# Veason-silverbullet/NNR

Measured on AMD Instinct MI355X. Metric: training impressions/sec on MIND-200k (CNE+SUE, bs=64), higher is better.
Workload: dtype f32

## Files before the change

### include/nnr_hip.h

```cpp
#ifndef NNR_HIP_H
#define NNR_HIP_H
#include <stdint.h>
#include <hip/hip_runtime_api.h>

#ifdef __cplusplus
extern "C" {
#endif

#define NNR_OK 0
#define NNR_ERR_ARG (-1)
#define NNR_ERR_LAUNCH (-2)
#define NNR_ERR_UNSUPPORTED (-3)

int nnr_version(void);

typedef struct nnr_gemm_args {
  const float* A;
  const float* B;
  float* C;
  int M, N, K;
  int lda, ldb, ldc;
  int trans_a, trans_b;
  const int* dyn_dev;
  int dyn_dim;
// ... 17 lines not shown
  int ldres;
  int accumulate;
  int atomic;
  const int* c_idx;
  int split_k;
  const float* rowdot_w;
  float* rowdot_out;
  int batch;
  long strideA, strideB, strideC, stride_aux, stride_res;
  int k_chunk;
  float* colsum_out;
  int tile;
  uint32_t drop_thresh;
  float drop_scale;
  int vec_epi;
  int sched;
  float* slab;
  long slab_floats;
  int slab_mode;
  const float* pre_add;
  int ldpre;
  int gate_bwd;
  const void* B3;
  long b3_stride;
  int ldb3;
} nnr_gemm_args;

int nnr_gemm_f32(const nnr_gemm_args* args, hipStream_t stream);
int nnr_split_bf16x3(const float* w, int rows, int cols, int ld, int ldo, void* out3, long img_stride, hipStream_t stream);

int nnr_seq_plan(uint8_t* mask, const int* ids, int n, int L, const int* perm_in, int* len_out, int* order, int* rank, int* slen,
                 int* bs, int* off, int* row_seq, int* tok, int* prev_f, int* prev_r, hipStream_t stream);

int nnr_seq_plan_pair(uint8_t* mask0, const int* ids0, int n0, uint8_t* mask1, const int* ids1, int n1, int L, const int* perm_in,
                      int* len_out, int* order, int* rank, int* slen, int* bs, int* off, int* row_seq, int* tok, int* prev_f,
                      int* prev_r, hipStream_t stream);

int nnr_cne_pair_map(const int* order_t, const int* order_c, int n0, int n, int* pm_t, int* pm_c, int* tmp, hipStream_t stream);

int nnr_mask_cover(const uint8_t* mask, int n, int L, uint8_t* cover, hipStream_t stream);
int nnr_seq_rowmap(const int* off, const int* rank, const int* len, int n, int L, int* rowmap, hipStream_t stream);

int nnr_lstm_dims(int H, int* UB, int* HP, int* NP);
int nnr_lstm_pack_weights(const float* w_ih_f, const float* w_hh_f, const float* b_ih_f, const float* b_hh_f, const float* w_ih_r,
                          const float* w_hh_r, const float* b_ih_r, const float* b_hh_r, int H, int E, float* w_ihp, float* b_p,
                          float* wf, float* wb, float* w_ihp_t, hipStream_t stream);
int nnr_lstm_unpack_grads(float* dw_ihp, float* db_p, float* dw_hhp, int H, int E, float* dw_ih_f, float* dw_hh_f,
                          float* db_ih_f, float* db_hh_f, float* dw_ih_r, float* dw_hh_r, float* db_ih_r, float* db_hh_r,
                          int accumulate , int zero_src, hipStream_t stream);
typedef struct nnr_lstm_problem {
  const int* bs; const int* off; const int* slen; const int* prev_f; const int* prev_r;
  int n, L;
  float* gates;
  float* cell;
  float* hout;
  float* cn;
  const float* wf;
  const float* wb;
  const float* dh;
  const float* dcn;
  unsigned* sync;
} nnr_lstm_problem;
size_t nnr_lstm_sync_bytes(int n);
size_t nnr_lstm_sync_diag_offset(int n);
int nnr_lstm_set_timeout_counter(unsigned* dev_counter);
int nnr_lstm_fwd(const nnr_lstm_problem* probs, int nprob, int H, hipStream_t stream);
int nnr_lstm_bwd(const nnr_lstm_problem* probs, int nprob, int H, hipStream_t stream);

typedef struct nnr_pool_args {
  const float* x; int ldx; int D; int n; int L;
  int packed;
  const int* off; const int* slen; const int* order;
  const uint8_t* mask; int mask_div;
  const float* score;
  const float* v; int ldv; float scale;
  float* alpha;
  float* out; int ldo; const float* add_in; int ldadd;
  const float* dout; int lddo; const float* dout2; int lddo2;
  float* dx; int lddx; int dx_accumulate;
  float* dscore;
  float* dv; int lddv;
  const float* th; int ldth; int A; const float* w2;
  const float* alpha_b; const float* dout_b; int lddo_b; const float* dscore_b; const float* v_b; int ldv_b; float scale_b;
} nnr_pool_args;
int nnr_attn_pool_fwd(const nnr_pool_args* a, hipStream_t stream);
int nnr_attn_pool_bwd(const nnr_pool_args* a, hipStream_t stream);

int nnr_gate_bwd(const float* dHt, const float* H, const float* G, float* dH, float* dpre, const int* rows_dev, int rows, int cols,
                 hipStream_t stream);
int nnr_packed_seq_sum(const float* x, int D, const int* off, const int* slen, int n, float* out, hipStream_t stream);
int nnr_slot_workspace_floats(int N);
int nnr_tanh_score_bwd(float* th, const float* ds, const float* w2, float* dw2, const int* rows_dev, int rows, int A, float* ws,
                       hipStream_t stream);
int nnr_colsum(const float* x, int ld, const int* rows_dev, int rows, int N, float* out_accum, float* ws, hipStream_t stream);
int nnr_rowdot(const float* x, int ld, const float* w, const int* rows_dev, int rows, int N, float* out,
               hipStream_t stream);
int nnr_small_embed_fwd(const float* table, const int* idx, int n, int dim, float* out, int ldo, float p, uint32_t seed,
                        hipStream_t stream);
int nnr_small_embed_bwd(const int* idx, int n, int dim, const float* dout, int lddo, float* dtable_accum, float p, uint32_t seed,
                        hipStream_t stream);
int nnr_embed_gather(const float* table, const int* idx, long n, const int* n_dev , int dim, float* out,
                     float p, uint32_t seed, hipStream_t stream);
int nnr_embed_scatter(const float* dout, const int* idx, long n, int dim, float* dtable_accum, float p, uint32_t seed,
                      hipStream_t stream);
int nnr_embed_scatter_dyn(const float* dout, const int* idx, long n, const int* n_dev, int dim, float* dtable, float p, uint32_t seed,
                          hipStream_t stream);
size_t nnr_token_sort_workspace_bytes(long cap, int vocab);
int nnr_token_sort(const int* tok, long cap, const int* n_dev, int vocab, unsigned* keys_tmp, int* rows_tmp, unsigned* keys_sorted,
                   int* rows_sorted, void* temp, size_t temp_bytes, hipStream_t stream);
size_t nnr_embed_scatter_sorted_workspace_floats(long cap);
int nnr_embed_scatter_sorted(const float* dout, const unsigned* keys_sorted, const int* rows_sorted, long cap, int vocab, int dim,
                             float* dtable_accum, float p, uint32_t seed, float* partial_ws, hipStream_t stream);
int nnr_transpose2d(const float* in, float* out, long rows, int cols, int accumulate, hipStream_t stream);
typedef struct nnr_transpose_desc { const float* in; float* out; int rows, cols; } nnr_transpose_desc;
int nnr_transpose_batch(const nnr_transpose_desc* descs_dev, int count, hipStream_t stream);
int nnr_add(float* y, const float* x, long n, float alpha, hipStream_t stream);
int nnr_add_atomic(float* y, const float* x, long n, float alpha, hipStream_t stream);
int nnr_add2d(float* y, int ldy, const float* x, int ldx, int rows, int cols, float alpha, int accumulate, hipStream_t stream);
int nnr_expand_rows_fwd(const float* x, float* y, int B, int N, int D, hipStream_t stream);
int nnr_expand_rows_bwd(const float* dy, float* dx, int B, int N, int D, hipStream_t stream);
int nnr_dropout(const float* x, float* y, long n, float p, uint32_t seed, hipStream_t stream);
int nnr_relu_bwd(const float* dy, const float* y, float* dx, long n, hipStream_t stream);
int nnr_gcn_aggregate_fwd(const float* graph, const float* z, const float* bias, const float* resid, float* r_out, float* y, int B, int G,
                          int D, int relu, float p, uint32_t seed, hipStream_t stream);
int nnr_gcn_aggregate_bwd(const float* graph, const float* dy, const float* r, float* ds, float* dx0, float* dz, int B, int G, int D, float p,
                          uint32_t seed, hipStream_t stream);
int nnr_relu_drop_bwd(const float* dy, const float* r, float* ds, float* dx, long n, float p, uint32_t seed, hipStream_t stream);

int nnr_mhsa_fwd(const float* qkv, const uint8_t* mask, int n, int Lq, int heads, int dh, float scale, float* out, float* prob,
                 float drop_p, uint32_t seed, hipStream_t stream);
int nnr_mhsa_bwd(const float* qkv, const uint8_t* mask, const float* prob, const float* dout, int n, int Lq, int heads, int dh,
                 float scale, float* dqkv, float drop_p, uint32_t seed, hipStream_t stream);
int nnr_mhsa_fwd_packed(const float* qkv, const uint8_t* mask, const int* rowmap, int n, int Lq, int heads, int dh, float scale, float* out,
                        float drop_p, uint32_t seed, hipStream_t stream);
int nnr_mhsa_bwd_packed(const float* qkv, const uint8_t* mask, const int* rowmap, const float* dout, int n, int Lq, int heads, int dh, float scale,
                        float* dqkv, float drop_p, uint32_t seed, hipStream_t stream);
int nnr_mhsa_pair_map(const int* off, const int* slen, const int* order, const uint8_t* mask, int n, int L, int* vrowmap, uint8_t* vmask,
                      hipStream_t stream);
int nnr_mhsa_fwd_paired(const float* qkv, const uint8_t* vmask, const int* vrowmap, const int* off, int n, int heads, int dh, float scale,
                        float* out, float drop_p, uint32_t seed, hipStream_t stream);
int nnr_mhsa_bwd_paired(const float* qkv, const uint8_t* vmask, const int* vrowmap, const int* off, const float* dout, int n, int heads, int dh,
                        float scale, float* dqkv, float drop_p, uint32_t seed, hipStream_t stream);

int nnr_sue_x0_fwd(const float* hist, const float* proxy, float* x0, int B, int Hn, int Kc, int D, float p, uint32_t seed,
                   uint8_t* cmask_fix, hipStream_t stream);
int nnr_sue_x0_bwd(const float* dx0, const float* dx0_add, float* dhist, float* dproxy_accum, int B, int Hn, int Kc, int D, float p,
                   uint32_t seed, hipStream_t stream);
int nnr_sue_slice_fwd(const float* gcn, const float* x0, float* gfeat, int B, int Hn, int G, int D, hipStream_t stream);
int nnr_sue_slice_bwd(const float* dgfeat, float* dpad, int B, int Hn, int G, int D, hipStream_t stream);
int nnr_sue_intra_fwd(const float* kf, const float* qc, const float* g, const long* cidx, int B, int N, int Hn, int C, int A, int D,
                      float* alpha, float* feat, hipStream_t stream);
int nnr_sue_intra_bwd(const float* kf, const float* qc, const float* g, const long* cidx, const float* alpha, const float* dfeat, int B,
                      int N, int Hn, int C, int A, int D, float* dg, float* dkf, float* dqc, float* ds_ws ,
                      hipStream_t stream);

int nnr_cand_attn_ws_floats(int B, int N, int H, int A);
int nnr_cand_attn_fwd(const float* P, const float* Q, const float* w2, const float* feat, int ldf, const uint8_t* mask, int B, int N,
                      int H, int A, int D, int act, float* alpha, float* out, hipStream_t stream);
int nnr_cand_attn_bwd(const float* P, const float* Q, const float* w2, const float* feat, int ldf, const uint8_t* mask, const float* alpha,
                      const float* dout, int B, int N, int H, int A, int D, int act, float* dP, float* dQ, float* dfeat,
                      int dfeat_accumulate, float* ws, float* dw2_accum, hipStream_t stream);

int nnr_omap_ws_floats(int B, int N, int H, int D, int K);
int nnr_omap_fwd(const float* hist, int ldf, const float* cand, const uint8_t* mask, const float* W, int B, int N, int H, int D, int K,
                 float* alpha, float* Y, float* beta, float* R, float* gamma, float* out, float* ws, hipStream_t stream);
int nnr_omap_bwd(const float* hist, int ldf, const float* cand, const uint8_t* mask, const float* W, const float* alpha, const float* Y,
                 const float* beta, const float* R, const float* gamma, const float* dout, int B, int N, int H, int D, int K, float* dhist,
                 int dhist_accumulate, float* dcand, float* dW_accum, float* ws, hipStream_t stream);
int nnr_omap_reg_fwd(const float* W, int D, int K, float coef, float* off, float* loss, hipStream_t stream);
int nnr_omap_reg_bwd(const float* W, const float* off, const float* gup, int D, int K, float coef, float* dW_accum, hipStream_t stream);

typedef struct nnr_corpus_tables {
  const int* news_category; const int* news_subCategory;
  const int* title_text; const uint8_t* title_mask; const int* title_entity;
  const int* abstract_text; const uint8_t* abstract_mask; const int* abstract_entity;
  const long* beh_user; const int* beh_history; const uint8_t* beh_history_mask; const int* beh_line;
  const float* graph_table; const uint8_t* cmask_table; const long* cidx_table;
  int T, C, H, G, K1;
} nnr_corpus_tables;
typedef struct nnr_batch_out {
  long* user_id;
  int* u_cat; int* u_sub; int* u_tt; uint8_t* u_tm; int* u_te; int* u_ct; uint8_t* u_cm; int* u_ce;
  uint8_t* u_hmask; float* u_graph; uint8_t* u_cmask; long* u_cidx;
  int* n_cat; int* n_sub; int* n_tt; uint8_t* n_tm; int* n_te; int* n_ct; uint8_t* n_cm; int* n_ce;
} nnr_batch_out;
int nnr_corpus_batch(const nnr_corpus_tables* t, const nnr_batch_out* o, const int* beh_idx, const int* samples, int ld_samples, int B,
                     int S, hipStream_t stream);
int nnr_history_graph(const int* cats, const uint8_t* hmask, int B, int H, int K, int norm, float* graph, uint8_t* cmask, long* cidx,
                      hipStream_t stream);
int nnr_rank_metrics(const float* scores, const uint8_t* labels, const long* offsets, int n_impressions, int* ranks,
                     double* per_impression, hipStream_t stream);

int nnr_logits_loss_fwd(const float* user, const float* cand, int B, int N, int D, float* logits, float* loss, float* dlogits,
                        hipStream_t stream);
int nnr_logits_fwd(const float* user, const float* cand, int B, int N, int D, float* logits, hipStream_t stream);
int nnr_nls_loss(const float* logits, int B, int N, float* loss, float* dlogits, hipStream_t stream);
int nnr_logits_bwd(const float* dlogits, const float* user, const float* cand, int B, int N, int D, float* duser, float* dcand,
                   int dcand_accumulate, hipStream_t stream);
int nnr_layernorm_fwd(const float* u, const float* gamma, const float* beta, float eps, long rows, int D, float* xhat, float* rstd,
                      float* r_out, const float* resid, float* y, float p, uint32_t seed, hipStream_t stream);
int nnr_layernorm_bwd(const float* dv, const float* xhat, const float* rstd, const float* gamma, long rows, int D, float* du,
                      float* dgamma, float* dbeta, hipStream_t stream);
int nnr_sumsq(const float* g, long n, float* out, hipStream_t stream);
int nnr_sumsq_part(const float* g, long n, float* out, const float* add_in, int slot, hipStream_t stream);
int nnr_clip_adam(float* p, const float* g, float* m, float* v, long n, const float* sumsq, float grad_scale, float clip, float lr,
                  float beta1, float beta2, float eps, float weight_decay, int step, hipStream_t stream);

int nnr_adam_skipped_steps(unsigned* host_out, int reset);
int nnr_adam_skipped_peek(unsigned* host_out);

typedef struct nnr_dp_ctx nnr_dp_ctx;
int nnr_dp_unique_id(void* out128);
int nnr_dp_init(const void* uid128, int rank, int world, nnr_dp_ctx** ctx);
int nnr_dp_allreduce(nnr_dp_ctx* ctx, float* flat, size_t n, hipStream_t stream);
int nnr_dp_broadcast(nnr_dp_ctx* ctx, float* flat, size_t n, int root, hipStream_t stream);
int nnr_dp_destroy(nnr_dp_ctx* ctx);
int nnr_dp_emulate_ranks(nnr_dp_ctx* ctx, int ranks);
int nnr_dp_busy(float* buf, long n, int workgroups, int iters, hipStream_t stream);
int nnr_rows_touch(const int* tok, long cap, const int* n_dev, int V, float* flags, hipStream_t stream);
int nnr_rows_compact(const float* flags, int V, int* pos, int* count, hipStream_t stream);
int nnr_rows_pack(const float* dense, const int* pos, int V, int E, float* packed, hipStream_t stream);
int nnr_rows_unpack(const float* packed, const int* pos, int V, int E, float* dense, hipStream_t stream);

int nnr_fusion_rows_fwd(const float* cat_table, const float* sub_table, const int* cat0, const int* sub0, int n0, const int* cat1,
                        const int* sub1, int n1, int cd, int sd, float* out, int ldo, float p, uint32_t seed_cat, uint32_t seed_sub,
                        hipStream_t stream);
int nnr_fusion_rows_bwd(const int* cat0, const int* sub0, int n0, const int* cat1, const int* sub1, int n1, int cd, int sd, const float* dout,
                        int lddo, float* dcat_table_accum, float* dsub_table_accum, float p, uint32_t seed_cat, uint32_t seed_sub,
                        hipStream_t stream);
int nnr_fusion_rows_bwd_det(const int* cat0, const int* sub0, int n0, const int* cat1, const int* sub1, int n1, int cd, int sd, int ncat,
// ... 34 lines not shown
```

### nnr_amd/_lib.py

```python
import ctypes as C
import os
import subprocess

_HERE = os.path.dirname(os.path.abspath(__file__))
LIB_PATH = os.environ.get('NNR_HIP_LIB') or os.path.join(_HERE, 'libnnr_hip.so')
_lib = None

vp, ci, cf, cu32, cl = C.c_void_p, C.c_int, C.c_float, C.c_uint32, C.c_long


class GemmArgs(C.Structure):
    _fields_ = [('A', vp), ('B', vp), ('C', vp), ('M', ci), ('N', ci), ('K', ci), ('lda', ci), ('ldb', ci), ('ldc', ci),
                ('trans_a', ci), ('trans_b', ci), ('dyn_dev', vp), ('dyn_dim', ci), ('a_idx', vp), ('b_idx', vp),
                ('drop_target', ci), ('drop_p', cf), ('drop_seed', cu32), ('drop_cols', ci), ('alpha', cf), ('bias', vp),
                ('rowvec', vp), ('ldrv', ci), ('rowvec_map', vp), ('act', ci), ('aux_out', vp), ('ldaux', ci), ('mul', vp),
                ('ldmul', ci), ('resid', vp), ('ldres', ci), ('accumulate', ci), ('atomic', ci), ('c_idx', vp),
                ('split_k', ci), ('rowdot_w', vp), ('rowdot_out', vp), ('batch', ci), ('strideA', cl), ('strideB', cl),
                ('strideC', cl), ('stride_aux', cl), ('stride_res', cl), ('k_chunk', ci), ('colsum_out', vp), ('tile', ci), ('drop_thresh', cu32),
                ('drop_scale', cf), ('vec_epi', ci), ('sched', ci), ('slab', vp), ('slab_floats', cl), ('slab_mode', ci), ('pre_add', vp), ('ldpre', ci), ('gate_bwd', ci), ('B3', vp), ('b3_stride', cl), ('ldb3', ci)]


class LstmProblem(C.Structure):
    _fields_ = [('bs', vp), ('off', vp), ('slen', vp), ('prev_f', vp), ('prev_r', vp), ('n', ci), ('L', ci), ('gates', vp),
                ('cell', vp), ('hout', vp), ('cn', vp), ('wf', vp), ('wb', vp), ('dh', vp), ('dcn', vp), ('sync', vp)]


class TransposeDesc(C.Structure):
    _fields_ = [('inp', vp), ('out', vp), ('rows', ci), ('cols', ci)]


class CorpusTables(C.Structure):
    _fields_ = [(k, vp) for k in ('news_category', 'news_subCategory', 'title_text', 'title_mask', 'title_entity', 'abstract_text',
                                  'abstract_mask', 'abstract_entity', 'beh_user', 'beh_history', 'beh_history_mask', 'beh_line',
                                  'graph_table', 'cmask_table', 'cidx_table')] + [(k, ci) for k in ('T', 'C', 'H', 'G', 'K1')]


class BatchOut(C.Structure):
    _fields_ = [(k, vp) for k in ('user_id', 'u_cat', 'u_sub', 'u_tt', 'u_tm', 'u_te', 'u_ct', 'u_cm', 'u_ce', 'u_hmask', 'u_graph',
                                  'u_cmask', 'u_cidx', 'n_cat', 'n_sub', 'n_tt', 'n_tm', 'n_te', 'n_ct', 'n_cm', 'n_ce')]


class PoolArgs(C.Structure):
    _fields_ = [('x', vp), ('ldx', ci), ('D', ci), ('n', ci), ('L', ci), ('packed', ci), ('off', vp), ('slen', vp),
                ('order', vp), ('mask', vp), ('mask_div', ci), ('score', vp), ('v', vp), ('ldv', ci), ('scale', cf),
                ('alpha', vp), ('out', vp), ('ldo', ci), ('add_in', vp), ('ldadd', ci), ('dout', vp), ('lddo', ci),
                ('dout2', vp), ('lddo2', ci), ('dx', vp), ('lddx', ci), ('dx_accumulate', ci), ('dscore', vp), ('dv', vp),
                ('lddv', ci), ('th', vp), ('ldth', ci), ('A', ci), ('w2', vp),
                ('alpha_b', vp), ('dout_b', vp), ('lddo_b', ci), ('dscore_b', vp), ('v_b', vp), ('ldv_b', ci), ('scale_b', cf)]


SIGNATURES = {
    'nnr_version': 'i32',
    'nnr_gemm_f32': 'i32 GemmArgs stream',
    'nnr_split_bf16x3': 'i32 ptr i32 i32 i32 i32 ptr i64 stream',
    'nnr_seq_plan': 'i32 ptr ptr i32 i32 ptr ptr ptr ptr ptr ptr ptr ptr ptr ptr ptr stream',
    'nnr_seq_plan_pair': 'i32 ptr ptr i32 ptr ptr i32 i32 ptr ptr ptr ptr ptr ptr ptr ptr ptr ptr ptr stream',
    'nnr_cne_pair_map': 'i32 ptr ptr i32 i32 ptr ptr ptr stream',
    'nnr_mask_cover': 'i32 ptr i32 i32 ptr stream',
    'nnr_seq_rowmap': 'i32 ptr ptr ptr i32 i32 ptr stream',
    'nnr_lstm_dims': 'i32 i32 ptr ptr ptr',
    'nnr_lstm_pack_weights': 'i32 ptr ptr ptr ptr ptr ptr ptr ptr i32 i32 ptr ptr ptr ptr ptr stream',
    'nnr_lstm_unpack_grads': 'i32 ptr ptr ptr i32 i32 ptr ptr ptr ptr ptr ptr ptr ptr i32 i32 stream',
    'nnr_lstm_sync_bytes': 'u64 i32',
    'nnr_lstm_sync_diag_offset': 'u64 i32',
    'nnr_lstm_set_timeout_counter': 'i32 ptr',
    'nnr_lstm_fwd': 'i32 LstmProblem i32 i32 stream',
    'nnr_lstm_bwd': 'i32 LstmProblem i32 i32 stream',
    'nnr_attn_pool_fwd': 'i32 PoolArgs stream',
    'nnr_attn_pool_bwd': 'i32 PoolArgs stream',
    'nnr_gate_bwd': 'i32 ptr ptr ptr ptr ptr ptr i32 i32 stream',
    'nnr_packed_seq_sum': 'i32 ptr i32 ptr ptr i32 ptr stream',
    'nnr_slot_workspace_floats': 'i32 i32',
    'nnr_tanh_score_bwd': 'i32 ptr ptr ptr ptr ptr i32 i32 ptr stream',
    'nnr_colsum': 'i32 ptr i32 ptr i32 i32 ptr ptr stream',
    'nnr_rowdot': 'i32 ptr i32 ptr ptr i32 i32 ptr stream',
    'nnr_small_embed_fwd': 'i32 ptr ptr i32 i32 ptr i32 f32 seed stream',
    'nnr_small_embed_bwd': 'i32 ptr i32 i32 ptr i32 ptr f32 seed stream',
    'nnr_embed_gather': 'i32 ptr ptr i64 ptr i32 ptr f32 seed stream',
    'nnr_embed_scatter': 'i32 ptr ptr i64 i32 ptr f32 seed stream',
    'nnr_embed_scatter_dyn': 'i32 ptr ptr i64 ptr i32 ptr f32 seed stream',
    'nnr_token_sort_workspace_bytes': 'u64 i64 i32',
    'nnr_token_sort': 'i32 ptr i64 ptr i32 ptr ptr ptr ptr ptr u64 stream',
    'nnr_embed_scatter_sorted_workspace_floats': 'u64 i64',
    'nnr_embed_scatter_sorted': 'i32 ptr ptr ptr i64 i32 i32 ptr f32 seed ptr stream',
    'nnr_transpose2d': 'i32 ptr ptr i64 i32 i32 stream',
    'nnr_transpose_batch': 'i32 TransposeDesc i32 stream',
    'nnr_add': 'i32 ptr ptr i64 f32 stream',
    'nnr_add_atomic': 'i32 ptr ptr i64 f32 stream',
    'nnr_add2d': 'i32 ptr i32 ptr i32 i32 i32 f32 i32 stream',
    'nnr_expand_rows_fwd': 'i32 ptr ptr i32 i32 i32 stream',
    'nnr_expand_rows_bwd': 'i32 ptr ptr i32 i32 i32 stream',
    'nnr_dropout': 'i32 ptr ptr i64 f32 seed stream',
    'nnr_relu_bwd': 'i32 ptr ptr ptr i64 stream',
    'nnr_gcn_aggregate_fwd': 'i32 ptr ptr ptr ptr ptr ptr i32 i32 i32 i32 f32 seed stream',
    'nnr_gcn_aggregate_bwd': 'i32 ptr ptr ptr ptr ptr ptr i32 i32 i32 f32 seed stream',
    'nnr_relu_drop_bwd': 'i32 ptr ptr ptr ptr i64 f32 seed stream',
    'nnr_mhsa_fwd': 'i32 ptr ptr i32 i32 i32 i32 f32 ptr ptr f32 seed stream',
    'nnr_mhsa_bwd': 'i32 ptr ptr ptr ptr i32 i32 i32 i32 f32 ptr f32 seed stream',
    'nnr_mhsa_fwd_packed': 'i32 ptr ptr ptr i32 i32 i32 i32 f32 ptr f32 seed stream',
    'nnr_mhsa_bwd_packed': 'i32 ptr ptr ptr ptr i32 i32 i32 i32 f32 ptr f32 seed stream',
    'nnr_mhsa_pair_map': 'i32 ptr ptr ptr ptr i32 i32 ptr ptr stream',
    'nnr_mhsa_fwd_paired': 'i32 ptr ptr ptr ptr i32 i32 i32 f32 ptr f32 seed stream',
    'nnr_mhsa_bwd_paired': 'i32 ptr ptr ptr ptr ptr i32 i32 i32 f32 ptr f32 seed stream',
    'nnr_sue_x0_fwd': 'i32 ptr ptr ptr i32 i32 i32 i32 f32 seed ptr stream',
    'nnr_sue_x0_bwd': 'i32 ptr ptr ptr ptr i32 i32 i32 i32 f32 seed stream',
    'nnr_sue_slice_fwd': 'i32 ptr ptr ptr i32 i32 i32 i32 stream',
    'nnr_sue_slice_bwd': 'i32 ptr ptr i32 i32 i32 i32 stream',
    'nnr_sue_intra_fwd': 'i32 ptr ptr ptr ptr i32 i32 i32 i32 i32 i32 ptr ptr stream',
    'nnr_sue_intra_bwd': 'i32 ptr ptr ptr ptr ptr ptr i32 i32 i32 i32 i32 i32 ptr ptr ptr ptr stream',
    'nnr_cand_attn_ws_floats': 'i32 i32 i32 i32 i32',
    'nnr_cand_attn_fwd': 'i32 ptr ptr ptr ptr i32 ptr i32 i32 i32 i32 i32 i32 ptr ptr stream',
    'nnr_cand_attn_bwd': 'i32 ptr ptr ptr ptr i32 ptr ptr ptr i32 i32 i32 i32 i32 i32 ptr ptr ptr i32 ptr ptr stream',
    'nnr_omap_ws_floats': 'i32 i32 i32 i32 i32 i32',
    'nnr_omap_fwd': 'i32 ptr i32 ptr ptr ptr i32 i32 i32 i32 i32 ptr ptr ptr ptr ptr ptr ptr stream',
    'nnr_omap_bwd': 'i32 ptr i32 ptr ptr ptr ptr ptr ptr ptr ptr ptr i32 i32 i32 i32 i32 ptr i32 ptr ptr ptr stream',
    'nnr_omap_reg_fwd': 'i32 ptr i32 i32 f32 ptr ptr stream',
    'nnr_omap_reg_bwd': 'i32 ptr ptr ptr i32 i32 f32 ptr stream',
    'nnr_corpus_batch': 'i32 CorpusTables BatchOut ptr ptr i32 i32 i32 stream',
    'nnr_history_graph': 'i32 ptr ptr i32 i32 i32 i32 ptr ptr ptr stream',
    'nnr_rank_metrics': 'i32 ptr ptr ptr i32 ptr ptr stream',
    'nnr_logits_loss_fwd': 'i32 ptr ptr i32 i32 i32 ptr ptr ptr stream',
    'nnr_logits_fwd': 'i32 ptr ptr i32 i32 i32 ptr stream',
    'nnr_nls_loss': 'i32 ptr i32 i32 ptr ptr stream',
    'nnr_logits_bwd': 'i32 ptr ptr ptr i32 i32 i32 ptr ptr i32 stream',
    'nnr_layernorm_fwd': 'i32 ptr ptr ptr f32 i64 i32 ptr ptr ptr ptr ptr f32 seed stream',
    'nnr_layernorm_bwd': 'i32 ptr ptr ptr ptr i64 i32 ptr ptr ptr stream',
    'nnr_sumsq': 'i32 ptr i64 ptr stream',
    'nnr_sumsq_part': 'i32 ptr i64 ptr ptr i32 stream',
    'nnr_clip_adam': 'i32 ptr ptr ptr ptr i64 ptr f32 f32 f32 f32 f32 f32 f32 i32 stream',
    'nnr_adam_skipped_steps': 'i32 ptr i32',
    'nnr_adam_skipped_peek': 'i32 ptr',
    'nnr_dp_unique_id': 'i32 ptr',
    'nnr_dp_init': 'i32 ptr i32 i32 handle',
    'nnr_dp_allreduce': 'i32 handle ptr u64 stream',
    'nnr_dp_broadcast': 'i32 handle ptr u64 i32 stream',
    'nnr_dp_destroy': 'i32 handle',
    'nnr_dp_emulate_ranks': 'i32 handle i32',
    'nnr_dp_busy': 'i32 ptr i64 i32 i32 stream',
    'nnr_rows_touch': 'i32 ptr i64 ptr i32 ptr stream',
    'nnr_rows_compact': 'i32 ptr i32 ptr ptr stream',
    'nnr_rows_pack': 'i32 ptr ptr i32 i32 ptr stream',
    'nnr_rows_unpack': 'i32 ptr ptr i32 i32 ptr stream',
    'nnr_fusion_rows_fwd': 'i32 ptr ptr ptr ptr i32 ptr ptr i32 i32 i32 ptr i32 f32 seed seed stream',
    'nnr_fusion_rows_bwd': 'i32 ptr ptr i32 ptr ptr i32 i32 i32 ptr i32 ptr ptr f32 seed seed stream',
    'nnr_fusion_rows_bwd_det': 'i32 ptr ptr i32 ptr ptr i32 i32 i32 i32 i32 ptr i32 ptr ptr f32 seed seed stream',
    'nnr_click_loss': 'i32 ptr ptr i32 i32 i32 ptr ptr ptr ptr ptr ptr stream',
    'nnr_fill_zero': 'i32 ptr u64 stream',
    'nnr_copy_bytes': 'i32 ptr ptr u64 stream',
    'nnr_fill_column_u8': 'i32 ptr i32 i32 i32 i32 stream',
    'nnr_tape_create': 'i32 handle',
    'nnr_tape_destroy': 'i32 handle',
    'nnr_tape_fn_id': 'i32 cstr',
    'nnr_tape_fn_nargs': 'i32 i32',
    'nnr_tape_call': 'i32 handle i32 stream ptr i32 ptr ptr ptr i32 i32 ptr ptr',
    'nnr_tape_wait_stream': 'i32 handle stream stream',
    'nnr_tape_event_record': 'i32 handle u64 stream',
    'nnr_tape_event_wait': 'i32 handle stream u64',
    'nnr_tape_segment': 'i32 handle',
    'nnr_tape_patch': 'i32 handle u64 i32 i32 i64',
    'nnr_tape_finalize': 'i32 handle',
    'nnr_tape_prepare_timing': 'i32 handle i32',
    'nnr_tape_info': 'i32 handle ptr ptr ptr ptr ptr',
    'nnr_tape_replay': 'i32 handle i32 ptr i32 ptr i32 i32',
    'nnr_tape_timings': 'i32 handle i32 ptr i32',
    'nnr_tape_timeline': 'i32 handle i32 ptr ptr ptr i32',
    'nnr_tape_last_error': 'i32 handle ptr ptr cstr i32',
}
SYMBOLS = list(SIGNATURES)
STRUCTS = {'nnr_gemm_args': GemmArgs, 'nnr_lstm_problem': LstmProblem, 'nnr_pool_args': PoolArgs, 'nnr_transpose_desc': TransposeDesc,
           'nnr_corpus_tables': CorpusTables, 'nnr_batch_out': BatchOut}
DEVICE_STRUCTS = {'TransposeDesc'}
_CTYPES = {'i32': ci, 'i64': cl, 'u64': C.c_size_t, 'f32': cf, 'seed': cu32, 'ptr': vp, 'handle': vp, 'cstr': C.c_char_p, 'stream': vp}
_CTYPES.update((c.__name__, vp if c.__name__ in DEVICE_STRUCTS else C.POINTER(c)) for c in STRUCTS.values())


def kinds(name):
    return SIGNATURES[name].split()[1:]


class NnrHipError(RuntimeError):
    pass


def build(force=False):
    if force:
        bdir = os.path.join(_HERE, 'csrc', 'build')
        if os.path.isdir(bdir):
            for f in os.listdir(bdir):
# ... 41 lines not shown
```

### nnr_amd/csrc/gcn.hip

```cpp
#include "common.h"

namespace {

constexpr int GCN_MAXG = 128;

template <int MODE, int MT>
__global__ __launch_bounds__(256) __attribute__((amdgpu_waves_per_eu(3, 8))) void gcn_aggregate_kernel(
    const float* __restrict__ graph, const float* __restrict__ in, const float* __restrict__ bias, const float* __restrict__ aux_in,
    float* __restrict__ out0, float* __restrict__ out1, float* __restrict__ out2, int G, int D, int relu, uint32_t seed, uint32_t thr, float scale) {
  extern __shared__ __attribute__((aligned(16))) float sm[];
  const int ks_n = (G + 3) >> 2, GR = ks_n * 4;
  const int A_LD = GR | 1;
  constexpr int Z_LD = 68;
  float* As = sm;
  float* Zs = sm + ((GR * A_LD + 3) & ~3);
  const int b = blockIdx.y, tid = threadIdx.x, lane = tid & 63, w = tid >> 6;
  const int r16 = lane & 15, kk = lane >> 4;
  const float* A = graph + (long)b * G * G;
  if ((G & 3) == 0) {
    const int g4 = G >> 2;
    for (int i = tid; i < G * g4; i += 256) {
      const int row = i / g4, c = (i - row * g4) * 4;
      const f32x4 v = *reinterpret_cast<const f32x4*>(A + row * G + c);
#pragma unroll
      for (int e = 0; e < 4; ++e) As[row * A_LD + c + e] = v[e];
    }
  } else {
    for (int i = tid; i < GR * A_LD; i += 256) {
      const int row = i / A_LD, col = i - row * A_LD;
      As[i] = (row < G && col < G) ? A[row * G + col] : 0.f;
    }
  }
  const int c0 = blockIdx.x * 64;
  const int c4 = (tid & 15) * 4, rr = tid >> 4;
  const bool cok = c0 + c4 < D;
  const long base = (long)b * G * D;
#pragma unroll
  for (int pass = 0; pass < MT; ++pass) {
    const int row = pass * 16 + rr;
    f32x4 v = {0.f, 0.f, 0.f, 0.f};
    if (row < G && cok) {
      const long idx = base + (long)row * D + c0 + c4;
      v = *reinterpret_cast<const f32x4*>(in + idx);
      if (MODE == 1 && aux_in) {
        if (thr) {
          bool kp[4];
          nnr_keep4(seed, (uint64_t)idx, thr, kp);
#pragma unroll
          for (int e = 0; e < 4; ++e) v[e] = kp[e] ? v[e] * scale : 0.f;
        }
        if (out1) *reinterpret_cast<f32x4*>(out1 + idx) = v;
        const f32x4 rv = *reinterpret_cast<const f32x4*>(aux_in + idx);
#pragma unroll
        for (int e = 0; e < 4; ++e) v[e] = rv[e] > 0.f ? v[e] : 0.f;
        *reinterpret_cast<f32x4*>(out0 + idx) = v;
      }
    }
    if (row < GR) *reinterpret_cast<f32x4*>(&Zs[row * Z_LD + c4]) = v;
  }
  __syncthreads();
  float bf[MT * 4];
#pragma unroll
  for (int ks = 0; ks < MT * 4; ++ks) bf[ks] = ks < ks_n ? Zs[(4 * ks + kk) * Z_LD + w * 16 + r16] : 0.f;
  f32x4 acc[MT];
  int arow[MT];
#pragma unroll
  for (int m = 0; m < MT; ++m) {
    acc[m] = f32x4{0.f, 0.f, 0.f, 0.f};
    arow[m] = min(m * 16 + r16, GR - 1);
  }
#pragma unroll
  for (int ks = 0; ks < MT * 4; ++ks) {
    if (ks < ks_n) {
#pragma unroll
      for (int m = 0; m < MT; ++m) {
        const float a = MODE == 0 ? As[arow[m] * A_LD + 4 * ks + kk] : As[(4 * ks + kk) * A_LD + arow[m]];
        acc[m] = __builtin_amdgcn_mfma_f32_16x16x4f32(a, bf[ks], acc[m], 0, 0, 0);
      }
    }
  }
  __syncthreads();
#pragma unroll
  for (int m = 0; m < MT; ++m)
#pragma unroll
    for (int e = 0; e < 4; ++e)
      if (m * 16 + 4 * kk + e < GR) Zs[(m * 16 + 4 * kk + e) * Z_LD + w * 16 + r16] = acc[m][e];
  __syncthreads();
  if (!cok) return;
  f32x4 bv = {0.f, 0.f, 0.f, 0.f};
  if (MODE == 0 && bias) bv = *reinterpret_cast<const f32x4*>(bias + c0 + c4);
#pragma unroll
  for (int pass = 0; pass < MT; ++pass) {
    const int row = pass * 16 + rr;
    if (row < G) {
      const long idx = base + (long)row * D + c0 + c4;
      f32x4 x = *reinterpret_cast<const f32x4*>(&Zs[row * Z_LD + c4]);
      if (MODE == 0) {
        x += bv;
        if (relu) {
#pragma unroll
          for (int e = 0; e < 4; ++e) x[e] = fmaxf(x[e], 0.f);
        }
        if (out1) *reinterpret_cast<f32x4*>(out1 + idx) = x;
        if (aux_in) x += *reinterpret_cast<const f32x4*>(aux_in + idx);
        if (thr) {
          bool kp[4];
          nnr_keep4(seed, (uint64_t)idx, thr, kp);
#pragma unroll
          for (int e = 0; e < 4; ++e) x[e] = kp[e] ? x[e] * scale : 0.f;
        }
        *reinterpret_cast<f32x4*>(out0 + idx) = x;
      } else {
        *reinterpret_cast<f32x4*>(out2 + idx) = x;
      }
    }
  }
}


}

extern "C" int nnr_gcn_aggregate_fwd(const float* graph, const float* z, const float* bias, const float* resid, float* r_out, float* y, int B,
                                     int G, int D, int relu, float p, uint32_t seed, hipStream_t stream) {
  if (!graph || !z || !y || B <= 0 || G <= 0 || D <= 0) return NNR_ERR_ARG;
  if (G > GCN_MAXG || (D & 3)) return NNR_ERR_UNSUPPORTED;
  const float sc = p > 0.f ? 1.f / (1.f - p) : 1.f;
  const int gp = (G + 15) / 16 * 16, gr = (G + 3) / 4 * 4;
#define GCN_CASE(MT_) case MT_: hipLaunchKernelGGL((gcn_aggregate_kernel<0, MT_>), dim3((D + 63) / 64, B), dim3(256), (size_t)(((gr * (gr | 1) + 3) & ~3) + gr * 68) * sizeof(float), \
                                                   stream, graph, z, bias, resid, y, r_out, nullptr, G, D, relu, seed, nnr_drop_thresh(p), sc); break;
  switch (gp / 16) { GCN_CASE(1) GCN_CASE(2) GCN_CASE(3) GCN_CASE(4) GCN_CASE(5) GCN_CASE(6) GCN_CASE(7) GCN_CASE(8) }
#undef GCN_CASE
  NNR_CHECK_LAUNCH();
  return NNR_OK;
}

extern "C" int nnr_gcn_aggregate_bwd(const float* graph, const float* dy, const float* r, float* ds, float* dx0, float* dz, int B, int G, int D,
                                     float p, uint32_t seed, hipStream_t stream) {
  if (!graph || !dy || !dz || B <= 0 || G <= 0 || D <= 0 || (r && !ds)) return NNR_ERR_ARG;
  if (G > GCN_MAXG || (D & 3)) return NNR_ERR_UNSUPPORTED;
  const float sc = p > 0.f ? 1.f / (1.f - p) : 1.f;
  const int gp = (G + 15) / 16 * 16, gr = (G + 3) / 4 * 4;
#define GCN_CASE(MT_) case MT_: hipLaunchKernelGGL((gcn_aggregate_kernel<1, MT_>), dim3((D + 63) / 64, B), dim3(256), (size_t)(((gr * (gr | 1) + 3) & ~3) + gr * 68) * sizeof(float), \
                                                   stream, graph, dy, nullptr, r, ds, dx0, dz, G, D, 0, seed, nnr_drop_thresh(p), sc); break;
  switch (gp / 16) { GCN_CASE(1) GCN_CASE(2) GCN_CASE(3) GCN_CASE(4) GCN_CASE(5) GCN_CASE(6) GCN_CASE(7) GCN_CASE(8) }
#undef GCN_CASE
  NNR_CHECK_LAUNCH();
  return NNR_OK;
}
```

### nnr_amd/csrc/gemm.hip

```cpp
#include "common.h"
#include <stdlib.h>
#include <type_traits>

namespace {

template <int BK>
__device__ __forceinline__ int swz(int r16) {
  return BK == 16 ? ((4 - (r16 >> 2)) & 3) : BK == 32 ? ((r16 >> 1) & 7) : (r16 & 15);
}

template <int TM, int TN>
__device__ __forceinline__ void gemm_epilogue(const nnr_gemm_args& g, f32x4 (&acc)[TM][TN], float* lds, float* __restrict__ C, int m0,
                                              int n0, int M, int N, int z) {
  constexpr int BN = 16 * TN, E_LD = BN + 4;
  const int tid = threadIdx.x, lane = tid & 63, w = tid >> 6;
  const int r = lane & 15, kk = lane >> 4;
  const uint32_t dthr = g.drop_thresh;
  const float dscale = g.drop_scale;
  const bool use_atomic = !g.slab_mode && (g.atomic || g.split_k > 1 || g.k_chunk > 0);
  float* aux = g.aux_out;
  const float* res = g.resid;
  const float* mulp = g.mul;
  if (g.batch > 1 && g.split_k <= 1 && g.k_chunk <= 0) {
    if (aux) aux += (long)z * g.stride_aux;
// ... 797 lines not shown
  dim3 grid(nbm * nbn, 1, g.batch > 1 ? g.batch : 1), block(256);
  hipLaunchKernelGGL((gemm_nt_pipe2_kernel<TM, TN, NS, OCC>), grid, block, 0, s, g);
  NNR_CHECK_LAUNCH();
  return NNR_OK;
}

template <int TM, int TN, int BK, int NS, int OCC, int PRIO = 0>
int launch_pipe(const nnr_gemm_args& g0, hipStream_t s) {
  constexpr int BM = 64 * TM, BN = 16 * TN;
  nnr_gemm_args g = g0;
  g.sched = kNtRagged;
  const int nbm = (g.M + BM - 1) / BM, nbn = (g.N + BN - 1) / BN;
  dim3 grid(nbm * nbn, 1, g.batch > 1 ? g.batch : 1), block(256);
  hipLaunchKernelGGL((gemm_nt_pipe_kernel<TM, TN, BK, NS, OCC, PRIO>), grid, block, 0, s, g);
  NNR_CHECK_LAUNCH();
  return NNR_OK;
}

static bool pipe_ok(const nnr_gemm_args& g) {
  auto al = [](const void* p) { return ((uintptr_t)p & 15) == 0; };
  return !g.trans_a && !g.trans_b && !g.b_idx && g.split_k <= 1 && g.k_chunk <= 0 && !g.rowdot_w && !g.colsum_out &&
         (g.drop_target == 0 || g.drop_target == 3 || g.drop_target == 4) && (g.K & 3) == 0 && (g.lda & 3) == 0 && (g.ldb & 3) == 0 &&
         al(g.A) && al(g.B) && (g.batch <= 1 || (((g.strideA | g.strideB) & 3) == 0)) && (g.dyn_dim == 0 || g.dyn_dim == 1);
}

typedef __bf16 bf16x8_t __attribute__((ext_vector_type(8)));
__device__ __forceinline__ void split3_bf16(float x, __bf16& h1, __bf16& h2, __bf16& h3) {
  const unsigned u = __builtin_bit_cast(unsigned, x), mag = u & 0x7fffffffu;
  const bool big = mag >= 0x7f7f8000u, nonfinite = mag >= 0x7f800000u;
  h1 = (__bf16)x;
  if (big) h1 = __builtin_bit_cast(__bf16, (unsigned short)((u >> 16) | (mag > 0x7f800000u ? 0x40u : 0u)));
  const float r1 = nonfinite ? 0.f : x - (float)h1;
  h2 = (__bf16)r1;
  const float r2 = r1 - (float)h2;
  h3 = (__bf16)r2;
}
__global__ void split_bf16x3_kernel(const float* __restrict__ w, int rows, int cols, int ld, int ldo, __bf16* __restrict__ out, long img_stride) {
  const long total = (long)rows * ldo;
  for (long i = blockIdx.x * (long)blockDim.x + threadIdx.x; i < total; i += (long)gridDim.x * blockDim.x) {
    const int r = (int)(i / ldo), c = (int)(i - (long)r * ldo);
    __bf16 a, b, d;
    split3_bf16(c < cols ? w[(long)r * ld + c] : 0.f, a, b, d);
    out[i] = a; out[img_stride + i] = b; out[2 * img_stride + i] = d;
  }
}
__device__ __forceinline__ int bx3_swzA(int r) { return ((r >> 1) & 1) | (((r >> 3) & 1) << 2); }
__device__ __forceinline__ int bx3_swzB(int r) { return (r >> 1) & 3; }

typedef unsigned u32x4_t __attribute__((ext_vector_type(4)));
__device__ __forceinline__ unsigned hi16_pair(float odd, float even) {
  return __builtin_amdgcn_perm(__float_as_uint(odd), __float_as_uint(even), 0x07060302u);
}
__device__ __forceinline__ void split3_trunc8(const f32x4& x0, const f32x4& x1, bf16x8_t& a1, bf16x8_t& a2, bf16x8_t& a3) {
  const float xs[8] = {x0[0], x0[1], x0[2], x0[3], x1[0], x1[1], x1[2], x1[3]};
  unsigned w1[4], w2[4], w3[4];
#pragma unroll
  for (int p = 0; p < 4; ++p) {
    const float xe = xs[2 * p], xo = xs[2 * p + 1];
    const unsigned h1 = hi16_pair(xo, xe);
    const float re = xe - __uint_as_float(h1 << 16), ro = xo - __uint_as_float(h1 & 0xffff0000u);
    const unsigned h2 = hi16_pair(ro, re);
    const float se = re - __uint_as_float(h2 << 16), so = ro - __uint_as_float(h2 & 0xffff0000u);
    w1[p] = h1; w2[p] = h2; w3[p] = hi16_pair(so, se);
  }
  a1 = __builtin_bit_cast(bf16x8_t, u32x4_t{w1[0], w1[1], w1[2], w1[3]});
  a2 = __builtin_bit_cast(bf16x8_t, u32x4_t{w2[0], w2[1], w2[2], w2[3]});
  a3 = __builtin_bit_cast(bf16x8_t, u32x4_t{w3[0], w3[1], w3[2], w3[3]});
}

template <int TM, int TN, int NS>
__global__ __launch_bounds__(256, (NS * (64 * TM * 128 + 3 * 16 * TN * 64) > 80 * 1024 ? 1 : 2)) void gemm_nt_bx3_kernel(nnr_gemm_args g) {
  constexpr int BM = 64 * TM, BN = 16 * TN, BK = 32;
  constexpr int A_BYTES = BM * BK * 4, B_IMG_BYTES = BN * BK * 2, STAGE_BYTES = A_BYTES + 3 * B_IMG_BYTES;
  constexpr int NIA = A_BYTES / 1024, NIB1 = B_IMG_BYTES / 1024;
  static_assert(A_BYTES % 1024 == 0 && B_IMG_BYTES % 1024 == 0 && NIA % 4 == 0, "tile shape");
  constexpr int E_LD = BN + 4;
  constexpr int LDS_BYTES = NS * STAGE_BYTES > 64 * E_LD * 4 ? NS * STAGE_BYTES : 64 * E_LD * 4;
  __shared__ __attribute__((aligned(1024))) unsigned char lds_raw[LDS_BYTES];
  const int tid = threadIdx.x, lane = tid & 63, w = __builtin_amdgcn_readfirstlane(tid >> 6), r = lane & 15, q = lane >> 4;
  int M = g.M;
  if (g.dyn_dim == 1) M = min(M, *g.dyn_dev);
  const int N = g.N, K = g.K;
  const int nbm = (M + BM - 1) / BM, nbn = (N + BN - 1) / BN, nblk = nbm * nbn;
  if ((int)blockIdx.x >= nblk) return;
  int v;
  {
    const int b = blockIdx.x, qq = nblk >> 3, rem = nblk & 7, x = b & 7, slot = b >> 3;
    v = x * qq + min(x, rem) + slot;
  }
  const int bm = v / nbn, bn = v - bm * nbn, m0 = bm * BM, n0 = bn * BN;
  const int S = (K + BK - 1) / BK;
  const unsigned lds_base = (unsigned)(uintptr_t)lds_raw;
  const float* zero = nnr_zero_page;
  asm volatile("" : "+s"(zero));
  constexpr int NA = NIA / 4, NBW = (3 * NIB1 + 3) / 4;
  static_assert(NA <= 8 && NBW <= 8, "tile shape");
  unsigned voffA[8], voffB[8];
  int akc[NA], bkc[NBW];
#pragma unroll
  for (int i = 0; i < 8; ++i) voffA[i] = voffB[i] = 0;
#pragma unroll
  for (int i = 0; i < NA; ++i) {
    const int row = (w + 4 * i) * 8 + lane / 8, c = (lane % 8) ^ bx3_swzA(row & 15);
    akc[i] = 4 * c;
    voffA[i] = (unsigned)(((long)min(row, M - 1 - m0) * g.lda + 4 * c) * 4);
  }
#pragma unroll
  for (int j = 0; j < NBW; ++j) {
    const int idx = min(w + 4 * j, 3 * NIB1 - 1);
    const int img = idx / NIB1, jj = idx - img * NIB1, row = jj * 16 + lane / 4, c = (lane % 4) ^ bx3_swzB(row & 15);
    bkc[j] = 8 * c;
    voffB[j] = (unsigned)(((long)img * g.b3_stride + (long)min(row, N - 1 - n0) * g.ldb3 + 8 * c) * 2);
  }
  const float* Abase = g.A + (long)m0 * g.lda;
  const char* Bbase = reinterpret_cast<const char*>(reinterpret_cast<const __bf16*>(g.B3) + (long)n0 * g.ldb3);
  const bool nb_hi = ((3 * NIB1) % 4 == 0) || (w < (3 * NIB1) % 4);
  const bool ktail = (K % BK) != 0;
  auto issue = [&](int s) __attribute__((always_inline)) {
    const int k0 = s * BK;
    const unsigned sb = lds_base + (unsigned)((s % NS) * STAGE_BYTES) + (unsigned)(w * 1024);
    if (!(ktail && s == S - 1)) {
      lds_dma16_block<NA>(Abase + k0, sb, voffA);
      const float* bb = reinterpret_cast<const float*>(Bbase + 2L * k0);
      if (nb_hi) lds_dma16_block<NBW>(bb, sb + A_BYTES, voffB);
      else if constexpr (NBW > 1) lds_dma16_block<NBW - 1>(bb, sb + A_BYTES, voffB);
      return;
    }
#pragma unroll
    for (int i = 0; i < NA; ++i)
      lds_dma16((k0 + akc[i] < K) ? reinterpret_cast<const float*>(reinterpret_cast<const char*>(Abase + k0) + voffA[i]) : zero, sb + (unsigned)(i * 4096));
#pragma unroll
    for (int j = 0; j < NBW; ++j)
      if (j < NBW - 1 || nb_hi)
        lds_dma16((k0 + bkc[j] < K) ? reinterpret_cast<const float*>(Bbase + 2L * k0 + voffB[j]) : zero, sb + A_BYTES + (unsigned)(j * 4096));
  };
  f32x4 acc_hi[TM][TN], acc_lo[TM][TN];
#pragma unroll
  for (int m = 0; m < TM; ++m)
#pragma unroll
    for (int n = 0; n < TN; ++n) acc_hi[m][n] = acc_lo[m][n] = f32x4{0.f, 0.f, 0.f, 0.f};
#pragma unroll
  for (int s = 0; s < NS - 1; ++s)
    if (s < S) issue(s);
  for (int s = 0; s < S; ++s) {
    if (nb_hi) wait_stages<NA + NBW, NS - 2>(S - 1 - s);
    else wait_stages<NA + NBW - 1, NS - 2>(S - 1 - s);
    __builtin_amdgcn_s_barrier();
    if (s + NS - 1 < S) issue(s + NS - 1);
    const unsigned char* st = lds_raw + (s % NS) * STAGE_BYTES;
    const float* As = reinterpret_cast<const float*>(st);
    const __bf16* Bi = reinterpret_cast<const __bf16*>(st + A_BYTES);
    bf16x8_t bf[3][TN];
#pragma unroll
    for (int img = 0; img < 3; ++img)
#pragma unroll
      for (int n = 0; n < TN; ++n)
        bf[img][n] = *reinterpret_cast<const bf16x8_t*>(Bi + img * (BN * BK) + (n * 16 + r) * BK + ((q ^ bx3_swzB(r)) * 8));
#pragma unroll
    for (int m = 0; m < TM; ++m) {
      const float* arow = As + ((w * TM + m) * 16 + r) * BK;
      const f32x4 x0 = *reinterpret_cast<const f32x4*>(arow + 4 * ((2 * q) ^ bx3_swzA(r)));
      const f32x4 x1 = *reinterpret_cast<const f32x4*>(arow + 4 * ((2 * q + 1) ^ bx3_swzA(r)));
      bf16x8_t a1, a2, a3;
      split3_trunc8(x0, x1, a1, a2, a3);
#pragma unroll
      for (int n = 0; n < TN; ++n) {
        acc_hi[m][n] = __builtin_amdgcn_mfma_f32_16x16x32_bf16(a1, bf[0][n], acc_hi[m][n], 0, 0, 0);
        acc_lo[m][n] = __builtin_amdgcn_mfma_f32_16x16x32_bf16(a3, bf[0][n], acc_lo[m][n], 0, 0, 0);
        acc_lo[m][n] = __builtin_amdgcn_mfma_f32_16x16x32_bf16(a1, bf[2][n], acc_lo[m][n], 0, 0, 0);
        acc_lo[m][n] = __builtin_amdgcn_mfma_f32_16x16x32_bf16(a2, bf[1][n], acc_lo[m][n], 0, 0, 0);
        acc_lo[m][n] = __builtin_amdgcn_mfma_f32_16x16x32_bf16(a2, bf[0][n], acc_lo[m][n], 0, 0, 0);
        acc_lo[m][n] = __builtin_amdgcn_mfma_f32_16x16x32_bf16(a1, bf[1][n], acc_lo[m][n], 0, 0, 0);
      }
    }
  }
#pragma unroll
  for (int m = 0; m < TM; ++m)
#pragma unroll
    for (int n = 0; n < TN; ++n) acc_hi[m][n] += acc_lo[m][n];
  __syncthreads();
  gemm_epilogue<TM, TN>(g, acc_hi, reinterpret_cast<float*>(lds_raw), g.C, m0, n0, M, N, 0);
}

static bool bx3_ok(const nnr_gemm_args& g) {
  auto al = [](const void* p) { return ((uintptr_t)p & 15) == 0; };
  return pipe_ok(g) && !g.a_idx && g.batch <= 1 && g.B3 && al(g.B3) && (g.ldb3 & 7) == 0 && g.ldb3 >= g.K && ((g.b3_stride * 2) & 15) == 0;
}
template <int TM, int TN, int NS>
int launch_bx3(const nnr_gemm_args& g, hipStream_t s) {
  constexpr int BM = 64 * TM, BN = 16 * TN;
  const int nbm = (g.M + BM - 1) / BM, nbn = (g.N + BN - 1) / BN;
  hipLaunchKernelGGL((gemm_nt_bx3_kernel<TM, TN, NS>), dim3(nbm * nbn), dim3(256), 0, s, g);
  NNR_CHECK_LAUNCH();
  return NNR_OK;
}

__device__ __forceinline__ int tn_eff_slices(int split_k, int sched, int K, int nblk, int slots) {
  const int deal_mode = sched & 3;
  const int want_wg = ((sched >> 2) & 63) ? ((sched >> 2) & 63) * 64 : 512;
  const int slice_stages = (sched >> 8) ? (sched >> 8) : 96;
  const int ktiles = (K + 15) / 16;
  const int want = (want_wg + nblk - 1) / nblk;
  int eff = max(1, min(min(split_k, max(want, ktiles / slice_stages)), max(1, ktiles / 12)));
  if (deal_mode != 2) {
    const int W = eff * nblk, wv = W / slots;
    const int target = W < slots ? slots : (((W - wv * slots) * 2 < slots) ? wv * slots : (wv + 1) * slots);
    eff = max(1, min(target / nblk, min(split_k, max(1, ktiles / 12))));
  }
  return eff;
}

template <int TM, int TN, int NS, int OCC, int PRIO = 0>
__global__ __launch_bounds__(256, OCC) void gemm_tn_pipe_kernel(nnr_gemm_args g) {
  if (PRIO == 1) set_prio_dyn((blockIdx.x + gridDim.x * blockIdx.z) >> 8);
  constexpr int BK = 16, BM = 64 * TM, BN = 16 * TN;
  constexpr int PA = BM, PB = BN <= 64 ? 64 : (BN <= 128 ? 128 : 256);
  constexpr int RA = 256 / PA, RB = 256 / PB;
  constexpr int NIA = BK / RA, NIB = BK / RB, NI = NIA + NIB;
  constexpr int NPW = (NI + 3) / 4;
  constexpr int STAGE = BK * (PA + PB);
  constexpr int E_LD = BN + 4;
  constexpr int LDS_FLOATS = (NS * STAGE > 64 * E_LD) ? NS * STAGE : 64 * E_LD;
  static_assert(BN <= 256 && NI % 4 == 0, "tile shape");
  __shared__ __attribute__((aligned(1024))) float lds[LDS_FLOATS];

  const int tid = threadIdx.x, lane = tid & 63, w = __builtin_amdgcn_readfirstlane(tid >> 6);
  const int r = lane & 15, kk = lane >> 4;
  const int M = g.M, N = g.N;
  int K = g.K;
  if (g.dyn_dim == 2) K = min(K, *g.dyn_dev);
  const int nbm = (M + BM - 1) / BM, nbn = (N + BN - 1) / BN;
  const int nblk = nbm * nbn;
  int v, z = 0;
  int kbeg = 0, kend = K;
  if (g.split_k > 1) {
    const int deal_mode = g.sched & 3;
    const int ktiles = (K + BK - 1) / BK;
    const int eff = tn_eff_slices(g.split_k, g.sched, K, nblk, OCC * 256);
    if (deal_mode) {
      const int W = eff * nblk, per = (W + 7) >> 3;
      const int L = blockIdx.x, x = L & 7, slot = L >> 3;
      const int lin = x * per + slot;
      if (slot >= per || lin >= W) return;
      z = lin / nblk;
      v = lin - z * nblk;
    } else {
      z = blockIdx.x / nblk;
      v = blockIdx.x - z * nblk;
      if (z >= eff) return;
    }
    const int per_k = (ktiles + eff - 1) / eff;
    kbeg = z * per_k * BK;
    kend = min(K, kbeg + per_k * BK);
    if (kbeg >= kend) return;
  } else {
    const int b = blockIdx.x, q = nblk >> 3, rem = nblk & 7, x = b & 7, slot = b >> 3;
    v = x * q + min(x, rem) + slot;
  }
  const int bm = v / nbn, bn = v - bm * nbn;
  const int m0 = bm * BM, n0 = bn * BN;
  const float* __restrict__ A = g.A;
  const float* __restrict__ B = g.B;
  const int* __restrict__ bidx = g.b_idx;
  const float* zero = nnr_zero_page;
  asm volatile("" : "+s"(zero));

  long coloff[NPW];
  int krow[NPW];
#pragma unroll
  for (int i = 0; i < NPW; ++i) {
    const int q = w + 4 * i;
    if (q < NIA) {
      const int kl = q * RA + lane / (PA / 4), p4 = lane % (PA / 4);
      const int col = (4 * p4) ^ (16 * ((kl >> 2) & 1));
      krow[i] = kl;
// ... 661 lines not shown
```

### nnr_amd/csrc/misc.hip

```cpp
#include "common.h"

namespace {

constexpr int EW_BLOCKS = 2048;
__host__ __device__ inline int ew_grid(long n, int per_block) {
  long b = (n + per_block - 1) / per_block;
  return (int)(b < 1 ? 1 : (b > EW_BLOCKS ? EW_BLOCKS : b));
}
__device__ __forceinline__ int dyn_rows(const int* dev, int rows) { return dev ? min(rows, *dev) : rows; }

__global__ void gate_bwd_kernel(const float* __restrict__ dHt, const float* __restrict__ H, const float* __restrict__ G,
                                float* __restrict__ dH, float* __restrict__ dpre, const int* rows_dev, int rows, int cols) {
  const long n4 = (long)dyn_rows(rows_dev, rows) * cols / 4;
  for (long i = blockIdx.x * (long)blockDim.x + threadIdx.x; i < n4; i += (long)gridDim.x * blockDim.x) {
    const f32x4 d = reinterpret_cast<const f32x4*>(dHt)[i], h = reinterpret_cast<const f32x4*>(H)[i],
                g = reinterpret_cast<const f32x4*>(G)[i];
    reinterpret_cast<f32x4*>(dH)[i] = d * g;
    reinterpret_cast<f32x4*>(dpre)[i] = d * h * g * (1.f - g);
  }
}

__global__ __launch_bounds__(256) void packed_seq_sum_kernel(const float* __restrict__ x, int D, const int* __restrict__ off,
                                                             const int* __restrict__ slen, int n, float* __restrict__ out) {
  __shared__ f32x4 part[128];
// ... 241 lines not shown
    }
    __syncthreads();
    for (int j = ty; j < 32; j += 8) {
      const int c = c0 + j, r = r0 + tx;
      if (r < d.rows && c < d.cols) d.out[(long)c * d.rows + r] = tile[tx][j];
    }
    __syncthreads();
  }
}

__global__ void add_kernel(float* __restrict__ y, const float* __restrict__ x, long n, float alpha) {
  for (long i = blockIdx.x * (long)blockDim.x + threadIdx.x; i < n; i += (long)gridDim.x * blockDim.x) y[i] += alpha * x[i];
}
__global__ void add_atomic_kernel(float* __restrict__ y, const float* __restrict__ x, long n, float alpha) {
  for (long i = blockIdx.x * (long)blockDim.x + threadIdx.x; i < n; i += (long)gridDim.x * blockDim.x) atomicAdd(&y[i], alpha * x[i]);
}
__global__ void add2d_kernel(float* __restrict__ y, int ldy, const float* __restrict__ x, int ldx, int rows, int cols,
                             float alpha, int accumulate) {
  const long total = (long)rows * cols;
  for (long i = blockIdx.x * (long)blockDim.x + threadIdx.x; i < total; i += (long)gridDim.x * blockDim.x) {
    const int r = i / cols, c = i - (long)r * cols;
    const float v = alpha * x[(long)r * ldx + c];
    float* p = y + (long)r * ldy + c;
    *p = accumulate ? *p + v : v;
  }
}
__global__ void expand_rows_kernel(const float* __restrict__ x, float* __restrict__ y, int B, int N, int D) {
  const long total = (long)B * N * D;
  for (long i = blockIdx.x * (long)blockDim.x + threadIdx.x; i < total; i += (long)gridDim.x * blockDim.x) {
    const long row = i / D;
    const int c = (int)(i - row * D);
    y[i] = x[(row / N) * D + c];
  }
}
__global__ void expand_rows_bwd_kernel(const float* __restrict__ dy, float* __restrict__ dx, int B, int N, int D) {
  const long total = (long)B * D;
  for (long i = blockIdx.x * (long)blockDim.x + threadIdx.x; i < total; i += (long)gridDim.x * blockDim.x) {
    const long b = i / D;
    const int c = (int)(i - b * D);
    const float* p = dy + b * N * D + c;
    float acc = p[0];
    for (int j = 1; j < N; ++j) acc += p[(long)j * D];
    dx[i] = acc;
  }
}

__global__ void sue_x0_kernel(const float* __restrict__ hist, const float* __restrict__ proxy, float* __restrict__ x0, int B,
                              int Hn, int Kc, int D, const float* __restrict__ dx0, const float* __restrict__ dx0_add,
                              float* __restrict__ dhist, float* __restrict__ dproxy, uint8_t* __restrict__ cmask_fix, uint32_t seed,
                              uint32_t thr, float scale) {
  const int G = Hn + Kc;
  const long total = (long)B * G * D;
  if (cmask_fix)
    for (long b = blockIdx.x * (long)blockDim.x + threadIdx.x; b < B; b += (long)gridDim.x * blockDim.x) cmask_fix[b * (Kc + 1) + Kc] = 1;
  for (long i = blockIdx.x * (long)blockDim.x + threadIdx.x; i < total; i += (long)gridDim.x * blockDim.x) {
    const int c = i % D; const long q = i / D; const int j = q % G; const int b = q / G;
    const float up = dx0 ? (dx0_add ? dx0[i] + dx0_add[i] : dx0[i]) : 0.f;
    if (j < Hn) {
      if (x0) x0[i] = hist[((long)b * Hn + j) * D + c];
      if (dhist) dhist[((long)b * Hn + j) * D + c] = up;
    } else {
      const int k = j - Hn;
      if (x0) {
        const float m = nnr_keep(seed, (uint64_t)((long)b * Kc + k) * D + c, thr) ? scale : 0.f;
        x0[i] = proxy[(long)k * D + c] * m;
      }
    }
  }
  if (dproxy) {
    for (long t = blockIdx.x * (long)blockDim.x + threadIdx.x; t < (long)Kc * D; t += (long)gridDim.x * blockDim.x) {
      const int c = t % D, k = t / D;
      float acc = 0.f;
      for (int b = 0; b < B; ++b) {
        const long i = ((long)b * G + Hn + k) * D + c;
        const float up = dx0_add ? dx0[i] + dx0_add[i] : dx0[i];
        const float m = nnr_keep(seed, (uint64_t)((long)b * Kc + k) * D + c, thr) ? scale : 0.f;
        acc += up * m;
      }
      atomicAdd(&dproxy[t], acc);
    }
  }
}

__global__ void sue_slice_kernel(const float* __restrict__ gcn, const float* __restrict__ x0, float* __restrict__ gfeat,
                                 const float* __restrict__ dgfeat, float* __restrict__ dpad, int B, int Hn, int G, int D) {
  const long total = (long)B * G * D;
  for (long i = blockIdx.x * (long)blockDim.x + threadIdx.x; i < total; i += (long)gridDim.x * blockDim.x) {
    const int c = i % D; const long q = i / D; const int j = q % G; const int b = q / G;
    if (gfeat) { if (j < Hn) gfeat[((long)b * Hn + j) * D + c] = gcn[i] + x0[i]; }
    if (dpad) dpad[i] = (j < Hn) ? dgfeat[((long)b * Hn + j) * D + c] : 0.f;
  }
}

__global__ void relu_drop_bwd_kernel(const float* __restrict__ dy, const float* __restrict__ r, float* __restrict__ ds,
                                     float* __restrict__ dx, long n, int cols, uint32_t seed, uint32_t thr, float scale) {
  for (long i = blockIdx.x * (long)blockDim.x + threadIdx.x; i < n; i += (long)gridDim.x * blockDim.x) {
    const float m = nnr_keep(seed, (uint64_t)i, thr) ? scale : 0.f;
    const float g = dy[i] * m;
    ds[i] = (r[i] > 0.f) ? g : 0.f;
    if (dx) dx[i] = g;
  }
}

__global__ void dropout_kernel(const float* __restrict__ x, float* __restrict__ y, long n, uint32_t seed, uint32_t thr,
                               float scale) {
  for (long i = blockIdx.x * (long)blockDim.x + threadIdx.x; i < n; i += (long)gridDim.x * blockDim.x)
    y[i] = nnr_keep(seed, (uint64_t)i, thr) ? x[i] * scale : 0.f;
}

__global__ void relu_bwd_kernel(const float* __restrict__ dy, const float* __restrict__ y, float* __restrict__ dx, long n) {
  for (long i = blockIdx.x * (long)blockDim.x + threadIdx.x; i < n; i += (long)gridDim.x * blockDim.x)
    dx[i] = (y[i] > 0.f) ? dy[i] : 0.f;
}

constexpr int SUE_MAXH = 64, SUE_MAXC = 32;
__device__ __forceinline__ void sue_members(const int* cid, int Hn, int C, int* ccnt, int* cstart, int* order) {
  const int tid = threadIdx.x;
  if (tid < C) {
    int n = 0;
    for (int j = 0; j < Hn; ++j) n += (cid[j] == tid);
    ccnt[tid] = n;
  }
  __syncthreads();
  if (tid == 0) {
    int acc = 0;
    for (int c = 0; c < C; ++c) { cstart[c] = acc; acc += ccnt[c]; }
  }
  __syncthreads();
  if (tid < C) {
    int k = cstart[tid];
    for (int j = 0; j < Hn; ++j) if (cid[j] == tid) order[k++] = j;
  }
  __syncthreads();
}

__device__ __forceinline__ bool sue_xcd_map(int id, int B, int per_user, int* b, int* w) {
  const int x = id & 7, slot = id >> 3;
  *b = (slot / per_user) * 8 + x;
  *w = slot % per_user;
  return *b < B;
}
__global__ __launch_bounds__(256) void sue_intra_fwd_kernel(const float* __restrict__ kf, const float* __restrict__ qc,
                                                            const float* __restrict__ g, const long* __restrict__ cidx,
                                                            int B, int N, int Hn, int C, int A, int D, float inv_scale,
                                                            float* __restrict__ alpha, float* __restrict__ feat) {
  __shared__ float sc[SUE_MAXH], al[SUE_MAXH], cmax[SUE_MAXC], csum[SUE_MAXC];
  __shared__ int cid[SUE_MAXH], order[SUE_MAXH], ccnt[SUE_MAXC], cstart[SUE_MAXC];
  int b, wi;
  if (!sue_xcd_map(blockIdx.x, B, N * ((D + 255) / 256), &b, &wi)) return;
  const int slice = wi / N, bn = b * N + (wi - slice * N);
  const int tid = threadIdx.x, lane = tid & 63, w = tid >> 6;
  for (int j = tid; j < Hn; j += 256) cid[j] = (int)cidx[(long)b * Hn + j];
  const float* q = qc + (long)bn * A;
  for (int j0 = w; j0 < Hn; j0 += 16) {
    float p[4] = {0.f, 0.f, 0.f, 0.f};
    const float* k[4];
#pragma unroll
    for (int u = 0; u < 4; ++u) k[u] = kf + ((long)b * Hn + min(j0 + 4 * u, Hn - 1)) * A;
    for (int x = lane; x < A; x += 64) {
      const float qv = q[x];
      float kv[4];
#pragma unroll
      for (int u = 0; u < 4; ++u) kv[u] = k[u][x];
#pragma unroll
      for (int u = 0; u < 4; ++u) p[u] += kv[u] * qv;
    }
// ... 329 lines not shown
  const float mean = wave_sum(s) / (float)D;
  float q = 0.f;
#pragma unroll
  for (int i = 0; i < LN_MAXPL; ++i) {
    const int c = lane + 64 * i;
    const float d = c < D ? v[i] - mean : 0.f;
    q += d * d;
  }
  const float rstd = 1.f / sqrtf(wave_sum(q) / (float)D + eps);
  if (lane == 0) rstd_out[row] = rstd;
#pragma unroll
  for (int i = 0; i < LN_MAXPL; ++i) {
    const int c = lane + 64 * i;
    if (c < D) {
      const float xh = (v[i] - mean) * rstd;
      const float r = fmaxf(xh * gamma[c] + beta[c], 0.f);
      xhat[row * D + c] = xh;
      r_out[row * D + c] = r;
      float o = r + (resid ? resid[row * D + c] : 0.f);
      if (thr) o = nnr_keep(seed, (uint64_t)(row * D + c), thr) ? o * scale : 0.f;
      y[row * D + c] = o;
    }
  }
}

__global__ __launch_bounds__(256) void ln_bwd_kernel(const float* __restrict__ dv, const float* __restrict__ xhat, const float* __restrict__ rstd,
                                                     const float* __restrict__ gamma, long rows, int D, float* __restrict__ du,
                                                     float* __restrict__ dgamma, float* __restrict__ dbeta) {
  __shared__ float red[2][LN_MAXPL * 64];
  const int lane = threadIdx.x & 63, w = threadIdx.x >> 6;
  for (int i = threadIdx.x; i < 2 * LN_MAXPL * 64; i += 256) (&red[0][0])[i] = 0.f;
  __syncthreads();
  float ag[LN_MAXPL], ab[LN_MAXPL];
#pragma unroll
  for (int i = 0; i < LN_MAXPL; ++i) ag[i] = ab[i] = 0.f;
  for (int k = 0; k < 4; ++k) {
    const long row = (long)blockIdx.x * 16 + w * 4 + k;
    if (row >= rows) break;
    float g[LN_MAXPL], xh[LN_MAXPL];
    float s1 = 0.f, s2 = 0.f;
#pragma unroll
    for (int i = 0; i < LN_MAXPL; ++i) {
      const int c = lane + 64 * i;
      const float d = c < D ? dv[row * D + c] : 0.f;
      xh[i] = c < D ? xhat[row * D + c] : 0.f;
      g[i] = c < D ? d * gamma[c] : 0.f;
      s1 += g[i];
      s2 += g[i] * xh[i];
      ag[i] += d * xh[i];
      ab[i] += d;
    }
    s1 = wave_sum(s1) / (float)D;
    s2 = wave_sum(s2) / (float)D;
    const float rs = rstd[row];
#pragma unroll
    for (int i = 0; i < LN_MAXPL; ++i) {
      const int c = lane + 64 * i;
      if (c < D) du[row * D + c] = rs * (g[i] - s1 - xh[i] * s2);
    }
  }
#pragma unroll
  for (int i = 0; i < LN_MAXPL; ++i) {
    atomicAdd(&red[0][lane + 64 * i], ag[i]);
    atomicAdd(&red[1][lane + 64 * i], ab[i]);
  }
  __syncthreads();
  for (int c = threadIdx.x; c < D; c += 256) {
    atomicAdd(&dgamma[c], red[0][c]);
    atomicAdd(&dbeta[c], red[1][c]);
  }
}

}

#define EW_LAUNCH(kern, n, ...)                                                             \
  do {                                                                                      \
    hipLaunchKernelGGL(kern, dim3(ew_grid((n), 256)), dim3(256), 0, stream, __VA_ARGS__);   \
    NNR_CHECK_LAUNCH();                                                                     \
    return NNR_OK;                                                                          \
  } while (0)

extern "C" int nnr_version(void) { return 1; }

extern "C" int nnr_gate_bwd(const float* dHt, const float* H, const float* G, float* dH, float* dpre, const int* rows_dev,
                            int rows, int cols, hipStream_t stream) {
  if (cols & 3) return NNR_ERR_UNSUPPORTED;
  EW_LAUNCH(gate_bwd_kernel, (long)rows * cols / 4, dHt, H, G, dH, dpre, rows_dev, rows, cols);
}

extern "C" int nnr_packed_seq_sum(const float* x, int D, const int* off, const int* slen, int n, float* out, hipStream_t stream) {
  if (D & 3) return NNR_ERR_UNSUPPORTED;
  hipLaunchKernelGGL(packed_seq_sum_kernel, dim3(n), dim3(256), 0, stream, x, D, off, slen, n, out);
  NNR_CHECK_LAUNCH();
  return NNR_OK;
}

extern "C" int nnr_slot_workspace_floats(int N) { return NNR_SLOTS * N; }

extern "C" int nnr_tanh_score_bwd(float* th, const float* ds, const float* w2, float* dw2, const int* rows_dev, int rows, int A,
                                  float* ws, hipStream_t stream) {
  const int rpb = 64;
  int blocks = (rows + rpb - 1) / rpb;
  if (ws) blocks = blocks > NNR_SLOTS ? NNR_SLOTS : (blocks < 1 ? 1 : blocks);
  hipLaunchKernelGGL(tanh_score_bwd_kernel, dim3(blocks), dim3(256), 0, stream, th, ds, w2, dw2, rows_dev, rows, A, rpb, ws);
  NNR_CHECK_LAUNCH();
  if (ws) {
    hipLaunchKernelGGL(slot_reduce_kernel, dim3((A + 7) / 8), dim3(256), 0, stream, (const float*)ws, blocks, A, dw2);
    NNR_CHECK_LAUNCH();
  }
  return NNR_OK;
}

extern "C" int nnr_rowdot(const float* x, int ld, const float* w, const int* rows_dev, int rows, int N, float* out, hipStream_t stream) {
  if (!x || !w || !out || rows <= 0) return rows <= 0 ? NNR_OK : NNR_ERR_ARG;
  if ((N & 3) || (ld & 3) || ((uintptr_t)x & 15) || ((uintptr_t)w & 15)) return NNR_ERR_UNSUPPORTED;
  const int blocks = (rows + 3) / 4;
  hipLaunchKernelGGL(rowdot_kernel, dim3(blocks > 8192 ? 8192 : blocks), dim3(256), 0, stream, x, ld, w, rows_dev, rows, N, out);
  NNR_CHECK_LAUNCH();
  return NNR_OK;
}

extern "C" int nnr_colsum(const float* x, int ld, const int* rows_dev, int rows, int N, float* out, float* ws, hipStream_t stream) {
  if (rows <= 0 || N <= 0) return NNR_OK;
  int rpb = rows / 512;
  rpb = rpb < 8 ? 8 : (rpb > 128 ? 128 : rpb);
  int blocks = (rows + rpb - 1) / rpb;
  if (ws) blocks = blocks > NNR_SLOTS ? NNR_SLOTS : blocks;
  hipLaunchKernelGGL(colsum_kernel, dim3(blocks, (N + 255) / 256), dim3(256), 0, stream, x, ld, rows_dev, rows, N, out, rpb, ws);
  NNR_CHECK_LAUNCH();
  if (ws) {
    hipLaunchKernelGGL(slot_reduce_kernel, dim3((N + 7) / 8), dim3(256), 0, stream, (const float*)ws, blocks, N, out);
    NNR_CHECK_LAUNCH();
  }
  return NNR_OK;
}

extern "C" int nnr_small_embed_fwd(const float* table, const int* idx, int n, int dim, float* out, int ldo, float p, uint32_t seed,
                                   hipStream_t stream) {
  const float sc = p > 0.f ? 1.f / (1.f - p) : 1.f;
  EW_LAUNCH(small_embed_kernel, (long)n * dim, table, idx, n, dim, out, ldo, (float*)nullptr, (const float*)nullptr, 0, seed,
            nnr_drop_thresh(p), sc);
}
extern "C" int nnr_small_embed_bwd(const int* idx, int n, int dim, const float* dout, int lddo, float* dtable, float p, uint32_t seed,
                                   hipStream_t stream) {
  const float sc = p > 0.f ? 1.f / (1.f - p) : 1.f;
  if (n <= 0) return NNR_OK;
  const int rpw = n >= 16 * 1024 ? 16 : (n >= 2048 ? 8 : 4);
  hipLaunchKernelGGL(small_embed_bwd_kernel, dim3((n + 4 * rpw - 1) / (4 * rpw)), dim3(256), 0, stream, idx, n, dim, dout, lddo, dtable, seed,
                     nnr_drop_thresh(p), sc, rpw);
  NNR_CHECK_LAUNCH();
  return NNR_OK;
}


extern "C" int nnr_embed_gather(const float* table, const int* idx, long n, const int* n_dev, int dim, float* out, float p, uint32_t seed,
                                hipStream_t stream) {
  if (dim & 3) return NNR_ERR_UNSUPPORTED;
  const float sc = p > 0.f ? 1.f / (1.f - p) : 1.f;
  hipLaunchKernelGGL(embed_gather_kernel, dim3(ew_grid((n + 3) / 4, 4)), dim3(256), 0, stream, table, idx, n, n_dev, dim, out, seed,
                     nnr_drop_thresh(p), sc);
  NNR_CHECK_LAUNCH();
  return NNR_OK;
}
static int embed_scatter_launch(const float* dout, const int* idx, long n, const int* n_dev, int dim, float* dtable, float p, uint32_t seed,
                                hipStream_t stream) {
  const float sc = p > 0.f ? 1.f / (1.f - p) : 1.f;
  const long want = (n + 3) / 4;
  hipLaunchKernelGGL(embed_scatter_kernel, dim3((int)(want < 1 ? 1 : (want > 1024 ? 1024 : want))), dim3(256), 0, stream, dout, idx, n, n_dev, dim, dtable,
                     seed, nnr_drop_thresh(p), sc);
  NNR_CHECK_LAUNCH();
  return NNR_OK;
}
extern "C" int nnr_embed_scatter(const float* dout, const int* idx, long n, int dim, float* dtable, float p, uint32_t seed, hipStream_t stream) {
  return embed_scatter_launch(dout, idx, n, nullptr, dim, dtable, p, seed, stream);
}
extern "C" int nnr_embed_scatter_dyn(const float* dout, const int* idx, long n, const int* n_dev, int dim, float* dtable, float p, uint32_t seed,
                                     hipStream_t stream) {
  return embed_scatter_launch(dout, idx, n, n_dev, dim, dtable, p, seed, stream);
}
extern "C" int nnr_transpose2d(const float* in, float* out, long rows, int cols, int accumulate, hipStream_t stream) {
  EW_LAUNCH(transpose2d_kernel, rows * cols, in, out, rows, cols, accumulate);
}

extern "C" int nnr_transpose_batch(const nnr_transpose_desc* descs_dev, int count, hipStream_t stream) {
  if (count <= 0) return NNR_OK;
  if (!descs_dev) return NNR_ERR_ARG;
  hipLaunchKernelGGL(transpose_batch_kernel, dim3(64, count), dim3(256), 0, stream, descs_dev);
  NNR_CHECK_LAUNCH();
  return NNR_OK;
}

extern "C" int nnr_add(float* y, const float* x, long n, float alpha, hipStream_t stream) { EW_LAUNCH(add_kernel, n, y, x, n, alpha); }
extern "C" int nnr_add_atomic(float* y, const float* x, long n, float alpha, hipStream_t stream) {
  EW_LAUNCH(add_atomic_kernel, n, y, x, n, alpha);
}
extern "C" int nnr_add2d(float* y, int ldy, const float* x, int ldx, int rows, int cols, float alpha, int accumulate,
                         hipStream_t stream) {
  EW_LAUNCH(add2d_kernel, (long)rows * cols, y, ldy, x, ldx, rows, cols, alpha, accumulate);
}

extern "C" int nnr_expand_rows_fwd(const float* x, float* y, int B, int N, int D, hipStream_t stream) {
  if (!x || !y || B <= 0 || N <= 0 || D <= 0) return NNR_ERR_ARG;
  EW_LAUNCH(expand_rows_kernel, (long)B * N * D, x, y, B, N, D);
}
extern "C" int nnr_expand_rows_bwd(const float* dy, float* dx, int B, int N, int D, hipStream_t stream) {
  if (!dy || !dx || B <= 0 || N <= 0 || D <= 0) return NNR_ERR_ARG;
  EW_LAUNCH(expand_rows_bwd_kernel, (long)B * D, dy, dx, B, N, D);
}

extern "C" int nnr_sue_x0_fwd(const float* hist, const float* proxy, float* x0, int B, int Hn, int Kc, int D, float p, uint32_t seed,
                              uint8_t* cmask_fix, hipStream_t stream) {
  const float sc = p > 0.f ? 1.f / (1.f - p) : 1.f;
  EW_LAUNCH(sue_x0_kernel, (long)B * (Hn + Kc) * D, hist, proxy, x0, B, Hn, Kc, D, (const float*)nullptr, (const float*)nullptr, (float*)nullptr,
            (float*)nullptr, cmask_fix, seed, nnr_drop_thresh(p), sc);
}
extern "C" int nnr_sue_x0_bwd(const float* dx0, const float* dx0_add, float* dhist, float* dproxy, int B, int Hn, int Kc, int D, float p,
                              uint32_t seed, hipStream_t stream) {
  const float sc = p > 0.f ? 1.f / (1.f - p) : 1.f;
  EW_LAUNCH(sue_x0_kernel, (long)B * (Hn + Kc) * D, (const float*)nullptr, (const float*)nullptr, (float*)nullptr, B, Hn, Kc, D, dx0, dx0_add,
            dhist, dproxy, (uint8_t*)nullptr, seed, nnr_drop_thresh(p), sc);
}
extern "C" int nnr_sue_slice_fwd(const float* gcn, const float* x0, float* gfeat, int B, int Hn, int G, int D, hipStream_t stream) {
  EW_LAUNCH(sue_slice_kernel, (long)B * G * D, gcn, x0, gfeat, (const float*)nullptr, (float*)nullptr, B, Hn, G, D);
}
extern "C" int nnr_sue_slice_bwd(const float* dgfeat, float* dpad, int B, int Hn, int G, int D, hipStream_t stream) {
  EW_LAUNCH(sue_slice_kernel, (long)B * G * D, (const float*)nullptr, (const float*)nullptr, (float*)nullptr, dgfeat, dpad, B, Hn, G, D);
}

extern "C" int nnr_relu_drop_bwd(const float* dy, const float* r, float* ds, float* dx, long n, float p, uint32_t seed,
                                 hipStream_t stream) {
  const float sc = p > 0.f ? 1.f / (1.f - p) : 1.f;
  EW_LAUNCH(relu_drop_bwd_kernel, n, dy, r, ds, dx, n, 0, seed, nnr_drop_thresh(p), sc);
}
extern "C" int nnr_dropout(const float* x, float* y, long n, float p, uint32_t seed, hipStream_t stream) {
  const float sc = p > 0.f ? 1.f / (1.f - p) : 1.f;
  EW_LAUNCH(dropout_kernel, n, x, y, n, seed, nnr_drop_thresh(p), sc);
}

extern "C" int nnr_layernorm_fwd(const float* u, const float* gamma, const float* beta, float eps, long rows, int D, float* xhat, float* rstd,
                                 float* r_out, const float* resid, float* y, float p, uint32_t seed, hipStream_t stream) {
  if (D > LN_MAXPL * 64 || rows <= 0) return D > LN_MAXPL * 64 ? NNR_ERR_UNSUPPORTED : NNR_OK;
  const float sc = p > 0.f ? 1.f / (1.f - p) : 1.f;
  hipLaunchKernelGGL(ln_fwd_kernel, dim3((unsigned)((rows + 3) / 4)), dim3(256), 0, stream, u, gamma, beta, eps, rows, D, xhat, rstd, r_out, resid, y,
                     seed, nnr_drop_thresh(p), sc);
  NNR_CHECK_LAUNCH();
  return NNR_OK;
}
extern "C" int nnr_layernorm_bwd(const float* dv, const float* xhat, const float* rstd, const float* gamma, long rows, int D, float* du,
                                 float* dgamma, float* dbeta, hipStream_t stream) {
  if (D > LN_MAXPL * 64 || rows <= 0) return D > LN_MAXPL * 64 ? NNR_ERR_UNSUPPORTED : NNR_OK;
  hipLaunchKernelGGL(ln_bwd_kernel, dim3((unsigned)((rows + 15) / 16)), dim3(256), 0, stream, dv, xhat, rstd, gamma, rows, D, du, dgamma, dbeta);
  NNR_CHECK_LAUNCH();
  return NNR_OK;
}
extern "C" int nnr_relu_bwd(const float* dy, const float* y, float* dx, long n, hipStream_t stream) {
  EW_LAUNCH(relu_bwd_kernel, n, dy, y, dx, n);
}

extern "C" int nnr_sue_intra_fwd(const float* kf, const float* qc, const float* g, const long* cidx, int B, int N, int Hn, int C, int A,
                                 int D, float* alpha, float* feat, hipStream_t stream) {
  if (Hn > SUE_MAXH || C > SUE_MAXC) return NNR_ERR_UNSUPPORTED;
  hipLaunchKernelGGL(sue_intra_fwd_kernel, dim3((B + 7) / 8 * 8 * N * ((D + 255) / 256)), dim3(256), 0, stream, kf, qc, g, cidx, B, N, Hn, C, A, D,
                     1.f / sqrtf((float)A), alpha, feat);
  NNR_CHECK_LAUNCH();
  return NNR_OK;
}
extern "C" int nnr_sue_intra_bwd(const float* kf, const float* qc, const float* g, const long* cidx, const float* alpha,
                                 const float* dfeat, int B, int N, int Hn, int C, int A, int D, float* dg, float* dkf, float* dqc,
                                 float* ds_ws, hipStream_t stream) {
  if (Hn > SUE_MAXH || C > SUE_MAXC || N > 8) return NNR_ERR_UNSUPPORTED;
  if (!ds_ws) return NNR_ERR_ARG;
  hipLaunchKernelGGL(sue_intra_bwd_ds_kernel, dim3((B + 7) / 8 * 8 * N), dim3(256), 0, stream, kf, g, cidx, alpha, dfeat, B, N, Hn, C, A, D,
                     1.f / sqrtf((float)A), ds_ws, dqc);
  NNR_CHECK_LAUNCH();
  hipLaunchKernelGGL(sue_intra_bwd_dg_kernel, dim3(B, (D + 255) / 256 + 1, C >= 3 ? 3 : 1), dim3(256), 0, stream, qc, cidx, alpha, dfeat, ds_ws, N, Hn, C,
                     A, D, dg, dkf);
  NNR_CHECK_LAUNCH();
  return NNR_OK;
}

extern "C" int nnr_logits_loss_fwd(const float* user, const float* cand, int B, int N, int D, float* logits, float* loss, float* dlogits,
                                   hipStream_t stream) {
  hipLaunchKernelGGL(logits_kernel, dim3((B * N + 3) / 4), dim3(256), 0, stream, user, cand, B * N, D, logits);
  NNR_CHECK_LAUNCH();
  hipLaunchKernelGGL(loss_kernel, dim3(1), dim3(256), 0, stream, logits, B, N, loss, dlogits);
  NNR_CHECK_LAUNCH();
  return NNR_OK;
}
extern "C" int nnr_logits_fwd(const float* user, const float* cand, int B, int N, int D, float* logits, hipStream_t stream) {
  hipLaunchKernelGGL(logits_kernel, dim3((B * N + 3) / 4), dim3(256), 0, stream, user, cand, B * N, D, logits);
  NNR_CHECK_LAUNCH();
  return NNR_OK;
}
extern "C" int nnr_nls_loss(const float* logits, int B, int N, float* loss, float* dlogits, hipStream_t stream) {
  hipLaunchKernelGGL(loss_kernel, dim3(1), dim3(256), 0, stream, logits, B, N, loss, dlogits);
  NNR_CHECK_LAUNCH();
  return NNR_OK;
}
extern "C" int nnr_logits_bwd(const float* dlogits, const float* user, const float* cand, int B, int N, int D, float* duser, float* dcand,
                              int dcand_accumulate, hipStream_t stream) {
  EW_LAUNCH(logits_bwd_kernel, (long)B * N * D, dlogits, user, cand, (long)B * N, D, duser, dcand, dcand_accumulate);
}

// ... 52 lines not shown
```

### nnr_amd/csrc/pool.hip

```cpp
#include "common.h"
#include <stdlib.h>

namespace {

constexpr int MAXT = 2;
constexpr int MAXV_ALL = 5;

struct PoolArgs {
  const float* x; int ldx; int D; int n; int L;
  int packed;
  const int* off; const int* slen; const int* order;
  const uint8_t* mask; int mask_div;
  const float* score;
  const float* v; int ldv; float scale;
  float* alpha;
  float* out; int ldo; const float* add_in; int ldadd;
  const float* dout; int lddo; const float* dout2; int lddo2;
  float* dx; int lddx; int dx_accumulate;
  float* dscore;
  float* dv; int lddv;
  const float* th; int ldth; int A; const float* w2;
  const float* alpha_b; const float* dout_b; int lddo_b; const float* dscore_b; const float* v_b; int ldv_b; float scale_b;
};

__device__ __forceinline__ long item_row(const PoolArgs& a, int s, int t) {
  return a.packed ? (long)a.off[t] + s : (long)s * a.L + t;
}

template <bool BWD, int NV, int UR>
__device__ __forceinline__ void pool_stream_body(const PoolArgs& a, const int s, float* __restrict__ tok, f32x4 (*__restrict__ part)[64 * NV]) {
  constexpr int MAXV = NV;
  constexpr int NWV = 4;
  const int lane = threadIdx.x & 63, w = threadIdx.x >> 6;
  if (s >= a.n) return;
  const int len = a.packed ? a.slen[s] : a.L;
  const int oidx = a.packed ? a.order[s] : s;
  const int nv = (a.D + 3) >> 2;
  const bool dot = a.v != nullptr;

  f32x4 q[MAXV];
  if (dot) {
#pragma unroll
    for (int j = 0; j < MAXV; ++j) {
      const int c = lane + 64 * j;
      q[j] = (c < nv) ? *reinterpret_cast<const f32x4*>(a.v + (long)oidx * a.ldv + 4 * c) : f32x4{0.f, 0.f, 0.f, 0.f};
    }
  }
  auto load_rows = [&](int t0, f32x4 (&xv)[UR][MAXV]) __attribute__((always_inline)) {
#pragma unroll
    for (int u = 0; u < UR; ++u) {
      const int t = min(t0 + u, len - 1);
      const float* xr = a.x + item_row(a, s, t) * a.ldx;
#pragma unroll
      for (int j = 0; j < MAXV; ++j) {
        const int c = lane + 64 * j;
        xv[u][j] = (c < nv) ? *reinterpret_cast<const f32x4*>(xr + 4 * c) : f32x4{0.f, 0.f, 0.f, 0.f};
      }
    }
  };
  auto reduce_vec = [&](f32x4 (&v)[MAXV]) __attribute__((always_inline)) {
#pragma unroll
    for (int j = 0; j < MAXV; ++j) part[w][lane + 64 * j] = v[j];
    __syncthreads();
#pragma unroll
    for (int j = 0; j < MAXV; ++j) v[j] = part[0][lane + 64 * j] + part[1][lane + 64 * j] + part[2][lane + 64 * j] + part[3][lane + 64 * j];
  };

  if (!BWD) {
    float sc[MAXT];
    if (dot) {
      for (int t0 = w * UR; t0 < len; t0 += NWV * UR) {
        f32x4 xv[UR][MAXV];
        load_rows(t0, xv);
#pragma unroll
        for (int u = 0; u < UR; ++u) {
          const int t = t0 + u;
          float p = 0.f;
#pragma unroll
          for (int j = 0; j < MAXV; ++j) p += xv[u][j][0] * q[j][0] + xv[u][j][1] * q[j][1] + xv[u][j][2] * q[j][2] + xv[u][j][3] * q[j][3];
          p = wave_sum(p) * a.scale;
          if (t < len && lane == 0) tok[t] = p;
        }
      }
      __syncthreads();
#pragma unroll
      for (int k = 0; k < MAXT; ++k) {
        const int t = lane + 64 * k;
        sc[k] = (t < len) ? tok[t] : -INFINITY;
      }
    } else if (a.th) {
      const int na = a.A >> 2;
      const f32x4 wv = (lane < na) ? *reinterpret_cast<const f32x4*>(a.w2 + 4 * lane) : f32x4{0.f, 0.f, 0.f, 0.f};
      for (int t0 = w; t0 < len; t0 += 4 * NWV) {
        f32x4 tv[4];
#pragma unroll
        for (int u = 0; u < 4; ++u) {
          const int t = min(t0 + u * NWV, len - 1);
          tv[u] = (lane < na) ? *reinterpret_cast<const f32x4*>(a.th + item_row(a, s, t) * a.ldth + 4 * lane) : f32x4{0.f, 0.f, 0.f, 0.f};
        }
#pragma unroll
        for (int u = 0; u < 4; ++u) {
          const int t = t0 + u * NWV;
          float p = tv[u][0] * wv[0] + tv[u][1] * wv[1] + tv[u][2] * wv[2] + tv[u][3] * wv[3];
          p = wave_sum(p);
          if (t < len && lane == 0) tok[t] = p;
        }
      }
      __syncthreads();
#pragma unroll
      for (int k = 0; k < MAXT; ++k) {
        const int t = lane + 64 * k;
        sc[k] = (t < len) ? tok[t] : -INFINITY;
// ... 80 lines not shown
#pragma unroll
      for (int u = 0; u < UR; ++u) {
        const int t = t0 + u;
        float p = 0.f;
#pragma unroll
        for (int j = 0; j < MAXV; ++j) p += xv[u][j][0] * go[j][0] + xv[u][j][1] * go[j][1] + xv[u][j][2] * go[j][2] + xv[u][j][3] * go[j][3];
        p = wave_sum(p);
        if (t < len && lane == 0) tok[t] = p;
      }
    }
    __syncthreads();
#pragma unroll
    for (int k = 0; k < MAXT; ++k) {
      const int t = lane + 64 * k;
      da[k] = (t < len) ? tok[t] : 0.f;
    }
    float dsum = 0.f;
#pragma unroll
    for (int k = 0; k < MAXT; ++k) dsum += al[k] * da[k];
    dsum = wave_sum(dsum);
    float ds[MAXT];
#pragma unroll
    for (int k = 0; k < MAXT; ++k) {
      const int t = lane + 64 * k;
      ds[k] = al[k] * (da[k] - dsum);
      if (a.mask && t < len && !a.mask[(long)((a.packed ? oidx : s) / a.mask_div) * a.L + t]) ds[k] = 0.f;
      if (w == 0 && t < len && a.dscore) a.dscore[item_row(a, s, t)] = ds[k];
    }
    f32x4 dvacc[MAXV];
#pragma unroll
    for (int j = 0; j < MAXV; ++j) dvacc[j] = f32x4{0.f, 0.f, 0.f, 0.f};
    if (!a.dx && !(dot && a.dv)) return;
    const bool two = a.alpha_b != nullptr;
    f32x4 go2[MAXV], q2[MAXV];
    float al2[MAXT], ds2[MAXT];
#pragma unroll
    for (int j = 0; j < MAXV; ++j) {
      const int c = lane + 64 * j;
      go2[j] = q2[j] = f32x4{0.f, 0.f, 0.f, 0.f};
      if (two && c < nv) {
        go2[j] = *reinterpret_cast<const f32x4*>(a.dout_b + (long)oidx * a.lddo_b + 4 * c);
        q2[j] = *reinterpret_cast<const f32x4*>(a.v_b + (long)oidx * a.ldv_b + 4 * c);
      }
    }
#pragma unroll
    for (int k = 0; k < MAXT; ++k) {
      const int t = lane + 64 * k;
      al2[k] = (two && t < len) ? a.alpha_b[item_row(a, s, t)] : 0.f;
      ds2[k] = (two && t < len) ? a.dscore_b[item_row(a, s, t)] * a.scale_b : 0.f;
    }
    for (int t0 = w * UR; t0 < len; t0 += NWV * UR) {
      f32x4 xv[UR][MAXV], old[UR][MAXV];
      long rows[UR];
#pragma unroll
      for (int u = 0; u < UR; ++u) {
        const int t = min(t0 + u, len - 1);
        rows[u] = item_row(a, s, t);
#pragma unroll
        for (int j = 0; j < MAXV; ++j) {
          const int c = lane + 64 * j;
          xv[u][j] = (dot && c < nv) ? *reinterpret_cast<const f32x4*>(a.x + rows[u] * a.ldx + 4 * c) : f32x4{0.f, 0.f, 0.f, 0.f};
          old[u][j] = (a.dx && a.dx_accumulate && c < nv) ? *reinterpret_cast<const f32x4*>(a.dx + rows[u] * a.lddx + 4 * c)
                                                          : f32x4{0.f, 0.f, 0.f, 0.f};
        }
      }
#pragma unroll
      for (int u = 0; u < UR; ++u) {
        const int t = t0 + u;
        if (t >= len) continue;
        const float alt = __shfl(t < 64 ? al[0] : al[1], t & 63, 64);
        const float dst = __shfl(t < 64 ? ds[0] : ds[1], t & 63, 64) * a.scale;
        const float alt2 = __shfl(t < 64 ? al2[0] : al2[1], t & 63, 64);
        const float dst2 = __shfl(t < 64 ? ds2[0] : ds2[1], t & 63, 64);
#pragma unroll
        for (int j = 0; j < MAXV; ++j) {
          const int c = lane + 64 * j;
          if (c < nv) {
            const f32x4 prev = two ? (alt2 * go2[j] + dst2 * q2[j]) : old[u][j];
            f32x4 g = alt * go[j] + prev;
            if (dot) {
              g += dst * q[j];
              dvacc[j] += dst * xv[u][j];
            }
            if (a.dx) *reinterpret_cast<f32x4*>(a.dx + rows[u] * a.lddx + 4 * c) = g;
          }
        }
      }
    }
    if (dot && a.dv) {
      reduce_vec(dvacc);
      if (w == 0) {
#pragma unroll
        for (int j = 0; j < MAXV; ++j) {
          const int c = lane + 64 * j;
          if (c < nv) *reinterpret_cast<f32x4*>(a.dv + (long)oidx * a.lddv + 4 * c) = dvacc[j];
        }
      }
    }
  }
}

template <bool BWD, int NV, int UR>
__global__ __launch_bounds__(256) void pool_kernel(PoolArgs a) {
  __shared__ float tok[64 * MAXT];
  __shared__ f32x4 part[4][64 * NV];
  pool_stream_body<BWD, NV, UR>(a, blockIdx.x, tok, part);
}

__device__ __forceinline__ float lane_get(float v, int i) { return __builtin_bit_cast(float, __builtin_amdgcn_readlane(__builtin_bit_cast(int, v), i)); }

template <bool BWD, int NV, int NW, int R>
__device__ __forceinline__ void pool_team_body(const PoolArgs& a, const int s, const int wt, float* __restrict__ tok, f32x4 (*__restrict__ part)[64 * NV]) {
  const int lane = threadIdx.x & 63;
  const int len = a.slen[s];
  const int oidx = a.order[s];
  const int nv = (a.D + 3) >> 2;
  const bool dot = a.v != nullptr;
  const long mrow = (long)(oidx / a.mask_div) * a.L;
  const int tl = wt + NW * lane;
  const bool livel = lane < R && tl < len;
  const int rowl = a.off[min(tl, a.L)] + s;
  f32x4 x[R][NV];
#pragma unroll
  for (int i = 0; i < R; ++i) {
    const bool live = wt + NW * i < len;
    const long row = __builtin_amdgcn_readlane(rowl, i);
#pragma unroll
    for (int j = 0; j < NV; ++j) {
      const int c = lane + 64 * j;
      x[i][j] = (live && c < nv) ? *reinterpret_cast<const f32x4*>(a.x + row * a.ldx + 4 * c) : f32x4{0.f, 0.f, 0.f, 0.f};
    }
  }
  f32x4 q[NV];
#pragma unroll
  for (int j = 0; j < NV; ++j) {
    const int c = lane + 64 * j;
    q[j] = (dot && c < nv) ? *reinterpret_cast<const f32x4*>(a.v + (long)oidx * a.ldv + 4 * c) : f32x4{0.f, 0.f, 0.f, 0.f};
  }
  auto dotq = [&](const f32x4 (&xi)[NV], const f32x4 (&y)[NV]) __attribute__((always_inline)) {
    float p = 0.f;
#pragma unroll
    for (int j = 0; j < NV; ++j) p += xi[j][0] * y[j][0] + xi[j][1] * y[j][1] + xi[j][2] * y[j][2] + xi[j][3] * y[j][3];
    return wave_sum(p);
  };
  auto reduce_vec = [&](f32x4 (&v)[NV]) __attribute__((always_inline)) {
    if constexpr (NW > 1) {
#pragma unroll
      for (int j = 0; j < NV; ++j) part[wt][lane + 64 * j] = v[j];
      __syncthreads();
#pragma unroll
      for (int j = 0; j < NV; ++j) v[j] = part[0][lane + 64 * j] + part[1][lane + 64 * j] + part[2][lane + 64 * j] + part[3][lane + 64 * j];
    }
  };

  if constexpr (!BWD) {
    float pv = 0.f;
    if (dot) {
#pragma unroll
      for (int i = 0; i < R; ++i) {
        const float d = dotq(x[i], q) * a.scale;
        pv = (lane == i) ? d : pv;
      }
    } else if (a.th) {
      const int na = a.A >> 2;
      const f32x4 wv = (lane < na) ? *reinterpret_cast<const f32x4*>(a.w2 + 4 * lane) : f32x4{0.f, 0.f, 0.f, 0.f};
      f32x4 tv[R];
#pragma unroll
      for (int i = 0; i < R; ++i) {
        const long row = __builtin_amdgcn_readlane(rowl, i);
        tv[i] = (wt + NW * i < len && lane < na) ? *reinterpret_cast<const f32x4*>(a.th + row * a.ldth + 4 * lane) : f32x4{0.f, 0.f, 0.f, 0.f};
      }
#pragma unroll
      for (int i = 0; i < R; ++i) {
        const float d = wave_sum(tv[i][0] * wv[0] + tv[i][1] * wv[1] + tv[i][2] * wv[2] + tv[i][3] * wv[3]);
        pv = (lane == i) ? d : pv;
      }
    } else {
      pv = livel ? a.score[rowl] : 0.f;
    }
    if (a.mask && livel && !a.mask[mrow + tl]) pv = -1e9f;
    float alv;
    if constexpr (NW == 1) {
      const float m = wave_max(livel ? pv : -INFINITY);
      const float e = livel ? expf(pv - m) : 0.f;
      alv = e * (1.f / wave_sum(e));
    } else {
      if (livel) tok[tl] = pv;
      __syncthreads();
      const float sc = (lane < len) ? tok[lane] : -INFINITY;
// ... 61 lines not shown
      go2[j] = q2[j] = dvacc[j] = f32x4{0.f, 0.f, 0.f, 0.f};
      if (two && c < nv) {
        go2[j] = *reinterpret_cast<const f32x4*>(a.dout_b + (long)oidx * a.lddo_b + 4 * c);
        q2[j] = *reinterpret_cast<const f32x4*>(a.v_b + (long)oidx * a.ldv_b + 4 * c);
      }
    }
    const float al2v = (two && livel) ? a.alpha_b[rowl] : 0.f;
    const float ds2v = (two && livel) ? a.dscore_b[rowl] * a.scale_b : 0.f;
    const float dstv = dsv * a.scale;
#pragma unroll
    for (int i = 0; i < R; ++i) {
      if (wt + NW * i >= len) continue;
      const long row = __builtin_amdgcn_readlane(rowl, i);
      const float al = lane_get(alv, i), dst = lane_get(dstv, i), al2 = lane_get(al2v, i), ds2 = lane_get(ds2v, i);
#pragma unroll
      for (int j = 0; j < NV; ++j) {
        const int c = lane + 64 * j;
        if (c < nv) {
          f32x4 prev = f32x4{0.f, 0.f, 0.f, 0.f};
          if (two) prev = al2 * go2[j] + ds2 * q2[j];
          else if (a.dx && a.dx_accumulate) prev = *reinterpret_cast<const f32x4*>(a.dx + row * a.lddx + 4 * c);
          f32x4 g = al * go[j] + prev;
          if (dot) {
            g += dst * q[j];
            dvacc[j] += dst * x[i][j];
          }
          if (a.dx) *reinterpret_cast<f32x4*>(a.dx + row * a.lddx + 4 * c) = g;
        }
      }
    }
    if (dot && a.dv) {
      reduce_vec(dvacc);
      if (wt == 0) {
#pragma unroll
        for (int j = 0; j < NV; ++j) {
          const int c = lane + 64 * j;
          if (c < nv) *reinterpret_cast<f32x4*>(a.dv + (long)oidx * a.lddv + 4 * c) = dvacc[j];
        }
      }
    }
  }
}

template <bool BWD, int NV, int R>
__global__ __launch_bounds__(256, (R >= 16 ? 2 : 3)) void pool_packed_kernel(PoolArgs a) {
  __shared__ float tok[64 * MAXT];
  __shared__ f32x4 part[4][64 * NV];
  const int w = __builtin_amdgcn_readfirstlane(threadIdx.x >> 6);
  const int b = blockIdx.x;
  const int nstream = a.L > 4 * R ? a.off[4 * R + 1] - a.off[4 * R] : 0;
  const int ncoop = a.L > R ? a.off[R + 1] - a.off[R] : 0;
  if (b < nstream) {
    pool_stream_body<BWD, NV, 4>(a, b, tok, part);
  } else if (b < ncoop) {
    pool_team_body<BWD, NV, 4, R>(a, b, w, tok, part);
  } else {
    const int s = ncoop + 4 * (b - ncoop) + w;
    if (s < a.n) pool_team_body<BWD, NV, 1, R>(a, s, 0, tok, part);
  }
}

}

static int pool_check(const nnr_pool_args* p) {
  if (!p || !p->x || p->n <= 0) return NNR_ERR_ARG;
  if ((p->D & 3) || p->D > 4 * 64 * MAXV_ALL || (p->ldx & 3)) return NNR_ERR_UNSUPPORTED;
  if (p->L > 64 * MAXT) return NNR_ERR_UNSUPPORTED;
  if (p->packed && (!p->off || !p->slen || !p->order)) return NNR_ERR_ARG;
  if (!p->v && !p->score && !p->alpha && !p->th) return NNR_ERR_ARG;
  if (p->th && (!p->w2 || p->A <= 0 || p->A > 256 || (p->A & 3) || (p->ldth & 3))) return NNR_ERR_UNSUPPORTED;
  return NNR_OK;
}

static PoolArgs to_args(const nnr_pool_args* p) {
  PoolArgs a;
  a.x = p->x; a.ldx = p->ldx; a.D = p->D; a.n = p->n; a.L = p->L; a.packed = p->packed;
  a.off = p->off; a.slen = p->slen; a.order = p->order; a.mask = p->mask; a.mask_div = p->mask_div > 0 ? p->mask_div : 1;
  a.score = p->score; a.v = p->v; a.ldv = p->ldv; a.scale = p->v ? p->scale : 1.f;
  a.alpha = p->alpha; a.out = p->out; a.ldo = p->ldo; a.add_in = p->add_in; a.ldadd = p->ldadd;
  a.dout = p->dout; a.lddo = p->lddo; a.dout2 = p->dout2; a.lddo2 = p->lddo2;
  a.dx = p->dx; a.lddx = p->lddx; a.dx_accumulate = p->dx_accumulate; a.dscore = p->dscore; a.dv = p->dv; a.lddv = p->lddv;
  a.th = p->th; a.ldth = p->ldth; a.A = p->A; a.w2 = p->w2;
  a.alpha_b = p->alpha_b; a.dout_b = p->dout_b; a.lddo_b = p->lddo_b; a.dscore_b = p->dscore_b; a.v_b = p->v_b; a.ldv_b = p->ldv_b; a.scale_b = p->scale_b;
  return a;
}

template <bool BWD>
static int pool_launch(const nnr_pool_args* p, hipStream_t stream) {
  const PoolArgs a = to_args(p);
  const dim3 grid(p->n), block(256);
  const int nv = (p->D + 3) / 4;
  if (p->packed && nv <= 128 && p->L <= 128) {
    if (nv <= 64) hipLaunchKernelGGL((pool_packed_kernel<BWD, 1, 8>), grid, block, 0, stream, a);
    else hipLaunchKernelGGL((pool_packed_kernel<BWD, 2, 8>), grid, block, 0, stream, a);
    NNR_CHECK_LAUNCH();
    return NNR_OK;
  }
  if (nv <= 64) hipLaunchKernelGGL((pool_kernel<BWD, 1, 4>), grid, block, 0, stream, a);
  else if (nv <= 128) hipLaunchKernelGGL((pool_kernel<BWD, 2, 4>), grid, block, 0, stream, a);
  else if (nv <= 256) hipLaunchKernelGGL((pool_kernel<BWD, 4, 2>), grid, block, 0, stream, a);
  else hipLaunchKernelGGL((pool_kernel<BWD, 5, 2>), grid, block, 0, stream, a);
  NNR_CHECK_LAUNCH();
  return NNR_OK;
}

extern "C" int nnr_attn_pool_fwd(const nnr_pool_args* p, hipStream_t stream) {
  int rc = pool_check(p);
  if (rc != NNR_OK) return rc;
  if (!p->out || (!p->v && !p->score && !p->th)) return NNR_ERR_ARG;
  return pool_launch<false>(p, stream);
}

extern "C" int nnr_attn_pool_bwd(const nnr_pool_args* p, hipStream_t stream) {
  int rc = pool_check(p);
  if (rc != NNR_OK) return rc;
  if (!p->dout || !p->alpha) return NNR_ERR_ARG;
  if (p->alpha_b && (!p->dout_b || !p->dscore_b || !p->v_b || !p->dx || p->dx_accumulate || (p->lddo_b & 3) || (p->ldv_b & 3))) return NNR_ERR_ARG;
  return pool_launch<true>(p, stream);
}
```

### nnr_amd/csrc/tape.hip

```cpp
#include <cstring>
#include <string>
#include <tuple>
#include <utility>
#include <vector>
#include "common.h"

namespace {

typedef int (*thunk_t)(const uint64_t* slots, hipStream_t stream);

template <typename T> inline T slot_as(const uint64_t* s) { T v; std::memcpy(&v, s, sizeof(T)); return v; }

template <auto Fn> struct Thunk;
template <typename... P, int (*Fn)(P...)> struct Thunk<Fn> {
  static constexpr int nargs = (int)sizeof...(P) - 1;
  template <size_t... I> static int apply(const uint64_t* s, hipStream_t st, std::index_sequence<I...>) {
    using Tup = std::tuple<P...>;
    static_assert(std::is_same<std::tuple_element_t<sizeof...(P) - 1, Tup>, hipStream_t>::value, "entry point must end with hipStream_t");
    return Fn(slot_as<std::tuple_element_t<I, Tup>>(s + I)..., st);
  }
  static int call(const uint64_t* s, hipStream_t st) { return apply(s, st, std::make_index_sequence<sizeof...(P) - 1>{}); }
};

struct Entry { const char* name; thunk_t thunk; int nargs; };
#define R(fn) { #fn, &Thunk<&fn>::call, Thunk<&fn>::nargs }
const Entry REGISTRY[] = {
  R(nnr_gemm_f32), R(nnr_seq_plan), R(nnr_seq_plan_pair), R(nnr_cne_pair_map), R(nnr_lstm_pack_weights), R(nnr_lstm_unpack_grads),
  R(nnr_lstm_fwd), R(nnr_lstm_bwd), R(nnr_attn_pool_fwd), R(nnr_attn_pool_bwd), R(nnr_gate_bwd), R(nnr_packed_seq_sum),
  R(nnr_tanh_score_bwd), R(nnr_colsum), R(nnr_rowdot), R(nnr_small_embed_fwd), R(nnr_small_embed_bwd), R(nnr_embed_gather),
  R(nnr_embed_scatter), R(nnr_embed_scatter_dyn), R(nnr_transpose2d), R(nnr_transpose_batch), R(nnr_add), R(nnr_add_atomic), R(nnr_add2d), R(nnr_expand_rows_fwd), R(nnr_expand_rows_bwd),
  R(nnr_dropout), R(nnr_relu_bwd), R(nnr_gcn_aggregate_fwd), R(nnr_gcn_aggregate_bwd), R(nnr_relu_drop_bwd), R(nnr_mhsa_fwd), R(nnr_mhsa_bwd),
  R(nnr_sue_x0_fwd), R(nnr_sue_x0_bwd), R(nnr_sue_slice_fwd), R(nnr_sue_slice_bwd), R(nnr_sue_intra_fwd), R(nnr_sue_intra_bwd),
  R(nnr_corpus_batch), R(nnr_history_graph), R(nnr_logits_loss_fwd), R(nnr_logits_fwd), R(nnr_nls_loss), R(nnr_logits_bwd),
  R(nnr_layernorm_fwd), R(nnr_layernorm_bwd), R(nnr_sumsq), R(nnr_sumsq_part), R(nnr_clip_adam), R(nnr_dp_allreduce), R(nnr_dp_broadcast), R(nnr_dp_busy), R(nnr_split_bf16x3), R(nnr_mhsa_fwd_packed), R(nnr_mhsa_bwd_packed), R(nnr_mhsa_pair_map), R(nnr_mhsa_fwd_paired), R(nnr_mhsa_bwd_paired), R(nnr_mask_cover), R(nnr_seq_rowmap),
  R(nnr_fill_zero), R(nnr_copy_bytes), R(nnr_fill_column_u8), R(nnr_fusion_rows_fwd), R(nnr_fusion_rows_bwd), R(nnr_click_loss), R(nnr_rank_metrics),
  R(nnr_token_sort), R(nnr_embed_scatter_sorted), R(nnr_fusion_rows_bwd_det),
  R(nnr_rows_touch), R(nnr_rows_compact), R(nnr_rows_pack), R(nnr_rows_unpack),
  R(nnr_cand_attn_fwd), R(nnr_cand_attn_bwd),
  R(nnr_omap_fwd), R(nnr_omap_bwd), R(nnr_omap_reg_fwd), R(nnr_omap_reg_bwd),
};
#undef R
constexpr int NREG = (int)(sizeof(REGISTRY) / sizeof(REGISTRY[0]));

enum { OP_CALL = 0, OP_RECORD = 1, OP_WAIT = 2 };
struct Op { int kind, a, b; };
struct Call { int fn, stream, nslots, tag; size_t slot_off; };
struct BlobRef { size_t slot; size_t blob_off; };
struct Patch { size_t byte_off; int kind; int width; int64_t addend; };
constexpr int MAX_TIMING_SETS = 64;

}

struct nnr_tape {
  std::vector<uint64_t> arena;
  std::vector<Call> calls;
  std::vector<Op> ops;
  std::vector<size_t> seg_begin;
  std::vector<hipStream_t> streams;
  std::vector<hipEvent_t> events;
  std::vector<uint64_t> event_keys;
  std::vector<BlobRef> blob_refs;
  std::vector<Patch> patches;
  std::vector<std::vector<hipEvent_t>> tset;
  int ntagged = 0;
  bool final = false;
  int last_rc = 0, last_failed_call = -1;
};

namespace {
int stream_index(nnr_tape* t, hipStream_t s) {
  for (size_t i = 0; i < t->streams.size(); ++i) if (t->streams[i] == s) return (int)i;
  t->streams.push_back(s);
  return (int)t->streams.size() - 1;
}
int new_event(nnr_tape* t, uint64_t key) {
  hipEvent_t e;
  if (hipEventCreateWithFlags(&e, hipEventDisableTiming) != hipSuccess) return -1;
  t->events.push_back(e);
  t->event_keys.push_back(key);
  return (int)t->events.size() - 1;
}
}

extern "C" int nnr_tape_create(nnr_tape** out) {
  if (!out) return NNR_ERR_ARG;
  *out = new nnr_tape();
  (*out)->seg_begin.push_back(0);
  return NNR_OK;
}

extern "C" int nnr_tape_destroy(nnr_tape* t) {
  if (!t) return NNR_OK;
  for (hipEvent_t e : t->events) (void)hipEventDestroy(e);
  for (auto& set : t->tset) for (hipEvent_t e : set) (void)hipEventDestroy(e);
  delete t;
  return NNR_OK;
}

extern "C" int nnr_tape_fn_id(const char* name) {
  for (int i = 0; i < NREG; ++i) if (std::strcmp(REGISTRY[i].name, name) == 0) return i;
  return -1;
}
extern "C" int nnr_tape_fn_nargs(int fn) { return (fn >= 0 && fn < NREG) ? REGISTRY[fn].nargs : -1; }

extern "C" int nnr_tape_call(nnr_tape* t, int fn, hipStream_t stream, const uint64_t* slots, int nslots, const int* blob_slot,
                             const void* const* blob_ptr, const size_t* blob_bytes, int nblobs, int tag, size_t* slot_off_out,
                             size_t* blob_off_out) {
  if (!t || t->final || fn < 0 || fn >= NREG || nslots != REGISTRY[fn].nargs || (nslots > 0 && !slots)) return NNR_ERR_ARG;
  if (nblobs < 0 || (nblobs > 0 && (!blob_slot || !blob_ptr || !blob_bytes))) return NNR_ERR_ARG;
  for (int i = 0; i < nblobs; ++i)
    if (blob_slot[i] < 0 || blob_slot[i] >= nslots || !blob_ptr[i]) return NNR_ERR_ARG;
  Call c;
  c.fn = fn; c.stream = stream_index(t, stream); c.nslots = nslots; c.tag = tag; c.slot_off = t->arena.size();
  t->arena.insert(t->arena.end(), slots, slots + nslots);
  for (int i = 0; i < nblobs; ++i) {
// ... 197 lines not shown
```

### nnr_amd/ops.py

```python
import ctypes as C
import math
import os
import weakref

import torch

from . import _lib as L
from . import profile as _prof
from . import tape as _tape

ACT_NONE, ACT_RELU, ACT_TANH, ACT_SIGMOID = 0, 1, 2, 3
K_CHUNK = 1024


class _NoSpan:
    def __enter__(self):
        return self

    def __exit__(self, *a):
        return False


_NOSPAN = _NoSpan()

# ... 658 lines not shown


def _timeout_counter(dev):
    key = dev.index if dev.index is not None else torch.cuda.current_device()
    t = _TMO.get(key)
    if t is None:
        t = torch.zeros(1, dtype=torch.int32, device=dev)
        _TMO[key] = t
        L.check(L.lib().nnr_lstm_set_timeout_counter(t.data_ptr()), 'nnr_lstm_set_timeout_counter')
    return t


def dp_busy(buf, workgroups, iters):
    L.check(L.lib().nnr_dp_busy(_p(buf), buf.numel(), workgroups, iters, _s()), 'nnr_dp_busy')


def lstm_sync_timeouts(reset=False):
    n = sum(int(t.item()) for t in _TMO.values())
    if reset:
        for t in _TMO.values():
            t.zero_()
    return n


def lstm_last_launch_timeouts():
    return sum(int(t[off // 4].item()) for t, off in LAST_LSTM_SYNC)


_SYNC_WS = {}


def _sync_workspace(dev, n, slot):
    key = (dev.index, n, slot, torch._C._cuda_getCurrentRawStream(_DEV_INDEX[0] if _DEV_INDEX else torch.cuda.current_device()))
    ws = _SYNC_WS.get(key)
    if ws is None:
        ws = _SYNC_WS[key] = torch.zeros(L.lib().nnr_lstm_sync_bytes(n) // 4, dtype=torch.int32, device=dev)
    tape_keep(ws)
    return ws


def _lstm_probs(items, H=0, backward=False):
    arr = (L.LstmProblem * len(items))()
    del LAST_LSTM_SYNC[:]
    for a, it in zip(arr, items):
        pl = it['plan']
        if LSTM_PAIR and H == 200:
            _timeout_counter(it['gates'].device)
            it['sync'] = _sync_workspace(it['gates'].device, pl.n, (it.get('name'), len(LAST_LSTM_SYNC), backward))
            LAST_LSTM_SYNC.append((it['sync'], L.lib().nnr_lstm_sync_diag_offset(pl.n)))
        a.sync = _p(it.get('sync'))
        a.bs, a.off, a.slen, a.prev_f, a.prev_r = _p(pl.bs), _p(pl.off), _p(pl.slen), _p(pl.prev_f), _p(pl.prev_r)
        a.n, a.L = pl.n, pl.L
        a.gates, a.cell, a.hout, a.cn = _p(it['gates']), _p(it['cell']), _p(it.get('hout')), _p(it.get('cn'))
        a.wf, a.wb = _p(it['w'].wf), _p(it['w'].wb)
        a.dh, a.dcn = _p(it.get('dh')), _p(it.get('dcn'))
    return arr


def _lstm_flops(items, H):
    totals = [it['plan'].total for it in items]

    def flops(vals=None):
        tok = sum(float(vals[t.data_ptr()]) if vals is not None else float(t.item()) for t in totals)
        return tok * 2 * (2.0 * H * 4 * H)
    flops.dyn = totals
    flops.scale = 4.0 * H / max(4 * H, -(-H // 16) * 64)
    return flops


def lstm_fwd(items, H):
    arr = _lstm_probs(items, H)
    with _prof.span('lstm_fwd', _lstm_flops(items, H)):
        L.check(L.lib().nnr_lstm_fwd(arr, len(items), H, _s()), 'nnr_lstm_fwd')


def lstm_bwd(items, H):
    arr = _lstm_probs(items, H, backward=True)
    with _prof.span('lstm_bwd', _lstm_flops(items, H)):
        L.check(L.lib().nnr_lstm_bwd(arr, len(items), H, _s()), 'nnr_lstm_bwd')


def _pool_args(x, ldx, D, n, Lx, plan=None, mask=None, mask_div=1, score=None, v=None, ldv=0, scale=1.0, alpha=None, out=None,
               ldo=0, add_in=None, ldadd=0, dout=None, lddo=0, dout2=None, lddo2=0, dx=None, lddx=0, dx_accumulate=False,
               dscore=None, dv=None, lddv=0, th=None, w2=None, alpha_b=None, dout_b=None, lddo_b=0, dscore_b=None, v_b=None, ldv_b=0, scale_b=1.0):
    a = L.PoolArgs()
    a.x, a.ldx, a.D, a.n, a.L = _p(x), ldx, D, n, Lx
    a.packed = int(plan is not None)
    if plan is not None:
        a.off, a.slen, a.order = _p(plan.off), _p(plan.slen), _p(plan.order)
    if mask is not None:
        a.mask = _p(mask.view(torch.uint8) if mask.dtype == torch.bool else mask)
    a.mask_div = mask_div
    a.score, a.v, a.ldv, a.scale, a.alpha = _p(score), _p(v), ldv, float(scale), _p(alpha)
    a.out, a.ldo, a.add_in, a.ldadd = _p(out), ldo, _p(add_in), ldadd
    a.dout, a.lddo, a.dout2, a.lddo2 = _p(dout), lddo, _p(dout2), lddo2
    a.dx, a.lddx, a.dx_accumulate, a.dscore, a.dv, a.lddv = _p(dx), lddx, int(dx_accumulate), _p(dscore), _p(dv), lddv
    if th is not None:
        a.th, a.ldth, a.A, a.w2 = _p(th), th.stride(0), th.shape[1], _p(w2)
    if alpha_b is not None:
        a.alpha_b, a.dout_b, a.lddo_b, a.dscore_b, a.v_b, a.ldv_b, a.scale_b = _p(alpha_b), _p(dout_b), lddo_b, _p(dscore_b), _p(v_b), ldv_b, float(scale_b)
    return a


def _pool_span(family, kw, per_token_arrays):
    if not _prof.active():
        return _NOSPAN
    plan, D, n, Lx = kw.get('plan'), kw['D'], kw['n'], kw['Lx']
    th = kw.get('th')
    per_row = 4.0 * (D * per_token_arrays + (th.shape[1] if th is not None else 0) + 2)
    return _hbm_span(family, per_row, n * Lx, dyn=plan.total if plan is not None else None, fixed=4.0 * n * D * 3)


def pool_fwd(**kw):
    with _pool_span('pool_fwd', kw, 1):
        L.check(L.lib().nnr_attn_pool_fwd(C.byref(_pool_args(**kw)), _s()), 'nnr_attn_pool_fwd')


def pool_bwd(**kw):
    with _pool_span('pool_bwd', kw, (3 if kw.get('dx_accumulate') else 2) if kw.get('dx') is not None else 1):
        L.check(L.lib().nnr_attn_pool_bwd(C.byref(_pool_args(**kw)), _s()), 'nnr_attn_pool_bwd')


def add_(y, x, alpha=1.0):
    assert y.is_contiguous() and x.is_contiguous() and y.numel() == x.numel()
    L.check(L.lib().nnr_add(_p(y), _p(x), y.numel(), alpha, _s()), 'nnr_add')
    return y


def add_atomic_(y, x, alpha=1.0):
    assert y.is_contiguous() and x.is_contiguous() and y.numel() == x.numel()
    L.check(L.lib().nnr_add_atomic(_p(y), _p(x), y.numel(), alpha, _s()), 'nnr_add_atomic')
    return y


def expand_rows(x, N):
    B, D = x.shape
    y = torch.empty((B, N, D), device=x.device, dtype=torch.float32)
    L.check(L.lib().nnr_expand_rows_fwd(_p(x), _p(y), B, N, D, _s()), 'nnr_expand_rows_fwd')
    return y


def expand_rows_bwd(dy):
    B, N, D = dy.shape
    dx = torch.empty((B, D), device=dy.device, dtype=torch.float32)
    L.check(L.lib().nnr_expand_rows_bwd(_p(dy), _p(dx), B, N, D, _s()), 'nnr_expand_rows_bwd')
    return dx


def add2d(y, ldy, x, ldx, rows, cols, alpha=1.0, accumulate=False):
    L.check(L.lib().nnr_add2d(_p(y), ldy, _p(x), ldx, rows, cols, alpha, accumulate, _s()), 'nnr_add2d')


def gate_bwd(dHt, H, G, dH, dpre, plan, cols):
    with _hbm_span('gate_bwd', 5 * 4.0 * cols, plan.cap, dyn=plan.total):
        return _gate_bwd(dHt, H, G, dH, dpre, plan, cols)


def _gate_bwd(dHt, H, G, dH, dpre, plan, cols):
    L.check(L.lib().nnr_gate_bwd(_p(dHt), _p(H), _p(G), _p(dH), _p(dpre), _p(plan.total), plan.cap, cols, _s()), 'nnr_gate_bwd')


def packed_seq_sum(x, D, plan, out):
    L.check(L.lib().nnr_packed_seq_sum(_p(x), D, _p(plan.off), _p(plan.slen), plan.n, _p(out), _s()), 'nnr_packed_seq_sum')


def tanh_score_bwd(th, ds, w2, dw2, plan, A):
    rows = plan.cap if plan is not None else th.shape[0]
    ws = _slot_ws(th.device, A)
    L.check(L.lib().nnr_tanh_score_bwd(_p(th), _p(ds), _p(w2), _p(dw2), _p(plan.total) if plan is not None else None, rows, A, _p(ws),
                                       _s()), 'nnr_tanh_score_bwd')


def small_embed_fwd(table, idx, out_view, ldo, p, seed):
    n, dim = idx.numel(), table.shape[1]
    L.check(L.lib().nnr_small_embed_fwd(_p(table), _p(idx), n, dim, _p(out_view), ldo, p, seed, _s()), 'nnr_small_embed_fwd')


def small_embed_bwd(idx, dim, dout_view, lddo, dtable, p, seed):
    L.check(L.lib().nnr_small_embed_bwd(_p(idx), idx.numel(), dim, _p(dout_view), lddo, _p(dtable), p, seed, _s()), 'nnr_small_embed_bwd')


def dropout(x, p, seed, out=None):
    if out is None:
        out = torch.empty_like(x)
    L.check(L.lib().nnr_dropout(_p(x), _p(out), x.numel(), p, seed, _s()), 'nnr_dropout')
    return out


def layernorm_fwd(u, gamma, beta, eps, xhat, rstd, r_out, resid, y, p, seed):
    rows, D = u.numel() // u.shape[-1], u.shape[-1]
    L.check(L.lib().nnr_layernorm_fwd(_p(u), _p(gamma), _p(beta), eps, rows, D, _p(xhat), _p(rstd), _p(r_out), _p(resid), _p(y), p, seed, _s()),
                                      'nnr_layernorm_fwd')


def layernorm_bwd(dv, xhat, rstd, gamma, du, dgamma, dbeta):
    rows, D = dv.numel() // dv.shape[-1], dv.shape[-1]
    L.check(L.lib().nnr_layernorm_bwd(_p(dv), _p(xhat), _p(rstd), _p(gamma), rows, D, _p(du), _p(dgamma), _p(dbeta), _s()), 'nnr_layernorm_bwd')


def relu_bwd(dy, y, dx=None):
    if dx is None:
        dx = torch.empty_like(dy)
    L.check(L.lib().nnr_relu_bwd(_p(dy), _p(y), _p(dx), dy.numel(), _s()), 'nnr_relu_bwd')
    return dx


def relu_drop_bwd(dy, r, ds, dx, p, seed):
    L.check(L.lib().nnr_relu_drop_bwd(_p(dy), _p(r), _p(ds), _p(dx), dy.numel(), p, seed, _s()), 'nnr_relu_drop_bwd')


def gcn_aggregate_fwd(graph, z, bias, resid, r_out, y, B, G, D, relu, p, seed):
    arrays = 3 + (1 if resid is not None else 0)
    with _hbm_span('gcn_aggregate_fwd', 4.0 * (G * D * arrays + G * G), B):
        L.check(L.lib().nnr_gcn_aggregate_fwd(_p(graph), _p(z), _p(bias), _p(resid), _p(r_out), _p(y), B, G, D, relu, p, seed, _s()),
                                              'nnr_gcn_aggregate_fwd')


def gcn_aggregate_bwd(graph, dy, r, ds, dx0, dz, B, G, D, p, seed):
    arrays = 4 + (1 if dx0 is not None else 0)
    with _hbm_span('gcn_aggregate_bwd', 4.0 * (G * D * arrays + G * G), B):
        L.check(L.lib().nnr_gcn_aggregate_bwd(_p(graph), _p(dy), _p(r), _p(ds), _p(dx0), _p(dz), B, G, D, p, seed, _s()), 'nnr_gcn_aggregate_bwd')


def sue_x0_fwd(hist, proxy, x0, B, Hn, Kc, D, p, seed, cmask_fix=None):
    if cmask_fix is not None:
        assert cmask_fix.is_contiguous() and cmask_fix.element_size() == 1 and tuple(cmask_fix.shape) == (B, Kc + 1)
    L.check(L.lib().nnr_sue_x0_fwd(_p(hist), _p(proxy), _p(x0), B, Hn, Kc, D, p, seed, _p(cmask_fix), _s()), 'nnr_sue_x0_fwd')


def sue_x0_bwd(dx0, dhist, dproxy, B, Hn, Kc, D, p, seed, dx0_add=None):
    L.check(L.lib().nnr_sue_x0_bwd(_p(dx0), _p(dx0_add), _p(dhist), _p(dproxy), B, Hn, Kc, D, p, seed, _s()), 'nnr_sue_x0_bwd')


def sue_slice_fwd(gcn, x0, gfeat, B, Hn, G, D):
    L.check(L.lib().nnr_sue_slice_fwd(_p(gcn), _p(x0), _p(gfeat), B, Hn, G, D, _s()), 'nnr_sue_slice_fwd')


def sue_slice_bwd(dgfeat, dpad, B, Hn, G, D):
    L.check(L.lib().nnr_sue_slice_bwd(_p(dgfeat), _p(dpad), B, Hn, G, D, _s()), 'nnr_sue_slice_bwd')


def sue_intra_fwd(kf, qc, g, cidx, B, N, Hn, Cn, A, D, alpha, feat):
    with _hbm_span('sue_intra_fwd', 4.0 * (Hn * A + N * A + Hn * D + N * Hn + N * Cn * D) + 8.0 * Hn, B):
        return _sue_intra_fwd(kf, qc, g, cidx, B, N, Hn, Cn, A, D, alpha, feat)


def _sue_intra_fwd(kf, qc, g, cidx, B, N, Hn, Cn, A, D, alpha, feat):
    L.check(L.lib().nnr_sue_intra_fwd(_p(kf), _p(qc), _p(g), _p(cidx), B, N, Hn, Cn, A, D, _p(alpha), _p(feat), _s()), 'nnr_sue_intra_fwd')


def sue_intra_bwd(kf, qc, g, cidx, alpha, dfeat, B, N, Hn, Cn, A, D, dg, dkf, dqc):
    ws = torch.empty(B * N * Hn, device=kf.device, dtype=torch.float32)
    with _hbm_span('sue_intra_bwd', 4.0 * (N * Cn * D + 2 * Hn * D + 2 * Hn * A + 2 * N * A + N * Hn) + 8.0 * Hn, B):
        return _sue_intra_bwd(kf, qc, g, cidx, alpha, dfeat, B, N, Hn, Cn, A, D, dg, dkf, dqc, ws)


def _sue_intra_bwd(kf, qc, g, cidx, alpha, dfeat, B, N, Hn, Cn, A, D, dg, dkf, dqc, ws):
    L.check(L.lib().nnr_sue_intra_bwd(_p(kf), _p(qc), _p(g), _p(cidx), _p(alpha), _p(dfeat), B, N, Hn, Cn, A, D, _p(dg), _p(dkf), _p(dqc),
                                      _p(ws), _s()), 'nnr_sue_intra_bwd')


def _u8(mask):
    return None if mask is None else (mask.view(torch.uint8) if mask.dtype == torch.bool else mask)


def cand_attn_fwd(P, Q, w2, feat, mask, B, N, H, A, D, act, alpha, out):
    with _hbm_span('cand_attn_fwd', 4.0 * (N * A + H * A + H * D + N * H + N * D) + 1.0 * H, B, fixed=4.0 * A):
        L.check(L.lib().nnr_cand_attn_fwd(_p(P), _p(Q), _p(w2), _p(feat), feat.stride(1), _p(_u8(mask)), B, N, H, A, D, act, _p(alpha), _p(out),
                                          _s()), 'nnr_cand_attn_fwd')


def cand_attn_bwd(P, Q, w2, feat, mask, alpha, dout, B, N, H, A, D, act, dP, dQ, dfeat, dw2, accumulate=False):
    ws = torch.empty(L.lib().nnr_cand_attn_ws_floats(B, N, H, A), device=P.device, dtype=torch.float32)
    with _hbm_span('cand_attn_bwd', 4.0 * (2 * N * A + 2 * H * A + (3 if accumulate else 2) * H * D + 3 * N * H + N * D + 2 * N * A) + 1.0 * H, B,
                   fixed=8.0 * A):
        L.check(L.lib().nnr_cand_attn_bwd(_p(P), _p(Q), _p(w2), _p(feat), feat.stride(1), _p(_u8(mask)), _p(alpha), _p(dout), B, N, H, A, D, act,
                                          _p(dP), _p(dQ), _p(dfeat), accumulate, _p(ws), _p(dw2), _s()), 'nnr_cand_attn_bwd')


def omap_ws(B, N, H, D, K, device):
    n = L.lib().nnr_omap_ws_floats(B, N, H, D, K)
    if n < 0:
        raise L.NnrHipError('nnr_omap_ws_floats failed with code %d (B %d, N %d, H %d, D %d, K %d)' % (n, B, N, H, D, K))
    return torch.empty(n, device=device, dtype=torch.float32)


def omap_fwd(hist, cand, mask, W, B, N, H, D, K, alpha, Y, beta, R, gamma, out):
    ws = omap_ws(B, N, H, D, K, hist.device)
    with _hbm_span('omap_fwd', 4.0 * (2 * H * D + 2 * H * H + 2 * H * D + N * D + 2 * K * D + N * D + 2 * H * K + N * K) + 1.0 * H, B,
                   fixed=4.0 * D * K):
        L.check(L.lib().nnr_omap_fwd(_p(hist), hist.stride(1), _p(cand), _p(_u8(mask)), _p(W), B, N, H, D, K, _p(alpha), _p(Y), _p(beta), _p(R),
                                     _p(gamma), _p(out), _p(ws), _s()), 'nnr_omap_fwd')


def omap_bwd(hist, cand, mask, W, alpha, Y, beta, R, gamma, dout, B, N, H, D, K, dhist, dcand, dW, accumulate=False):
    ws = omap_ws(B, N, H, D, K, hist.device)
    with _hbm_span('omap_bwd', 4.0 * (2 * H * D + 2 * H * D + 2 * H * H + 2 * H * H + 2 * N * D + K * D + 3 * K * D + N * D +
                                      (2 if accumulate else 1) * H * D + 2 * D * K + 3 * H * K) + 1.0 * H, B, fixed=12.0 * D * K):
        L.check(L.lib().nnr_omap_bwd(_p(hist), hist.stride(1), _p(cand), _p(_u8(mask)), _p(W), _p(alpha), _p(Y), _p(beta), _p(R), _p(gamma), _p(dout),
                                     B, N, H, D, K, _p(dhist), accumulate, _p(dcand), _p(dW), _p(ws), _s()), 'nnr_omap_bwd')


def omap_reg_fwd(W, coef, off, loss):
    D, K = W.shape
    L.check(L.lib().nnr_omap_reg_fwd(_p(W), D, K, coef, _p(off), _p(loss), _s()), 'nnr_omap_reg_fwd')


def omap_reg_bwd(W, off, gup, coef, dW):
    D, K = W.shape
    L.check(L.lib().nnr_omap_reg_bwd(_p(W), _p(off), _p(gup), D, K, coef, _p(dW), _s()), 'nnr_omap_reg_bwd')


def logits_loss_fwd(user, cand, B, N, D, logits, loss, dlogits):
    L.check(L.lib().nnr_logits_loss_fwd(_p(user), _p(cand), B, N, D, _p(logits), _p(loss), _p(dlogits), _s()), 'nnr_logits_loss_fwd')
# ... 251 lines not shown
```

### nnr_amd/user_encoders.py

```python
import math

import torch
import torch.nn as nn

from . import ops
from .layers import Attention, ScaledDotProduct_CandidateAttention, MultiHeadAttention, GCN, grad_of, _CandAttnFn
from .news_encoders import NewsEncoder


class UserEncoder(nn.Module):

    def __init__(self, news_encoder: NewsEncoder, config):
        super().__init__()
        self.news_embedding_dim = news_encoder.news_embedding_dim
        self.news_encoder = news_encoder
        self.auxiliary_loss = None
        self._seed_base = int(getattr(config, 'seed', 0)) * 104723 + 29
        self._calls = 0

    def _next_seed(self):
        self._calls += 1
        return (self._seed_base + 15485863 * self._calls) & 0x7FFFFFFF

    def forward(self, user_title_text, user_title_mask, user_title_entity, user_content_text, user_content_mask, user_content_entity,
                user_category, user_subCategory, user_history_mask, user_history_graph, user_history_category_mask,
                user_history_category_indices, user_embedding, candidate_news_representation):
        raise Exception('Function forward must be implemented at sub-class')


class _SUEFunction(torch.autograd.Function):
    @staticmethod
    def forward(ctx, hist, cand, mod, graph, cmask, cidx):
        out, saved = sue_forward(mod, hist.contiguous(), cand.contiguous(), graph, cmask, cidx)
        ctx.mod, ctx.saved = mod, saved
        return out

    @staticmethod
    def backward(ctx, dout):
        dhist, dcand = sue_backward(ctx.mod, ctx.saved, dout.contiguous())
        ctx.saved = None
        return dhist, dcand, None, None, None, None


_SIDE = {}
ops.STREAM_CACHES.append(_SIDE)


def _sue_side(dev):
    if ops.ONE_STREAM[0]:
        return None
    key = (dev.type, dev.index)
    if key not in _SIDE:
        _SIDE[key] = ops.new_stream(dev)
    return _SIDE[key]


def gcn_forward(gcn, x0, graph, seed0, training):
    B, G, D = x0.shape
    f32 = dict(device=x0.device, dtype=torch.float32)
    Lg = gcn.num_layers
    xs, rs, lns = [x0], [], []
    x = x0
    for l, layer in enumerate(gcn.gcn_layers):
        y = torch.empty((B, G, D), **f32)
        r = torch.empty((B, G, D), **f32)
        pl = (gcn.dropout_rate if training else 0.0) if l + 1 < Lg else 0.0
        z = ops.linear_fwd(x.view(B * G, D), layer.W.weight)
        if getattr(layer, 'layer_norm', False):
            u = torch.empty((B, G, D), **f32)
            ops.gemm(graph, z, u, M=G, N=D, K=G, lda=G, ldb=D, ldc=D, trans_b=True, bias=layer.W.bias, batch=B, strideA=G * G, strideB=G * D,
                     strideC=G * D, tile=2)
            xhat = torch.empty((B, G, D), **f32)
            rstd = torch.empty(B * G, **f32)
            ln = layer.layer_normalization
            ops.layernorm_fwd(u, ln.weight, ln.bias, ln.eps, xhat, rstd, r, x if gcn.residual else None, y, pl, seed0 + l)
            lns.append((xhat, rstd))
        elif G <= 128 and D % 4 == 0:
            ops.gcn_aggregate_fwd(graph, z, layer.W.bias, x if gcn.residual else None, r, y, B, G, D, True, pl, seed0 + l)
            lns.append(None)
        else:
            ops.gemm(graph, z, y, M=G, N=D, K=G, lda=G, ldb=D, ldc=D, trans_b=True, bias=layer.W.bias, act=ops.ACT_RELU, aux_out=r,
                     ldaux=D, resid=x if gcn.residual else None, ldres=D, drop=(3, pl, seed0 + l, D), batch=B, strideA=G * G,
                     strideB=G * D, strideC=G * D, stride_aux=G * D, stride_res=G * D, tile=2)
            lns.append(None)
        xs.append(y)
        rs.append(r)
        x = y
    return x, dict(xs=xs, rs=rs, lns=lns, seed0=seed0, training=training)


def gcn_backward(gcn, gsv, dy, graph, leaf):
    B, G, D = dy.shape
    f32 = dict(device=dy.device, dtype=torch.float32)
    Lg = gcn.num_layers
    for l in range(Lg - 1, -1, -1):
        layer = gcn.gcn_layers[l]
        pl = (gcn.dropout_rate if gsv['training'] else 0.0) if l + 1 < Lg else 0.0
        dS = torch.empty((B, G, D), **f32)
        dx = torch.empty((B, G, D), **f32)
        if G <= 128 and D % 4 == 0 and gsv['lns'][l] is None:
            dz = torch.empty((B, G, D), **f32)
            ops.gcn_aggregate_bwd(graph, dy, gsv['rs'][l], dS, dx if gcn.residual else None, dz, B, G, D, pl, gsv['seed0'] + l)
            ops.linear_bwd_data(dz.view(B * G, D), layer.W.weight, out=dx.view(B * G, D), accumulate=bool(gcn.residual))
            leaf(lambda dS=dS, dz=dz, l=l, layer=layer: (ops.bias_grad(dS.view(B * G, D), grad_of(layer.W.bias)),
                                                         ops.linear_bwd_weight(dz.view(B * G, D), gsv['xs'][l].view(B * G, D), grad_of(layer.W.weight))), dS, dz)
            dy = dx
            continue
        ops.relu_drop_bwd(dy, gsv['rs'][l], dS, dx, pl, gsv['seed0'] + l)
        if not gcn.residual:
            ops.fill_zero(dx)
        if gsv['lns'][l] is not None:
            xhat, rstd = gsv['lns'][l]
            ln = layer.layer_normalization
            du = torch.empty((B, G, D), **f32)
            ops.layernorm_bwd(dS, xhat, rstd, ln.weight, du, grad_of(ln.weight), grad_of(ln.bias))
            dS = du
        dz = torch.empty((B, G, D), **f32)
        ops.gemm(graph, dS, dz, M=G, N=D, K=G, lda=G, ldb=D, ldc=D, trans_a=True, trans_b=True, batch=B, strideA=G * G, strideB=G * D,
                 strideC=G * D, tile=2)
        ops.linear_bwd_data(dz.view(B * G, D), layer.W.weight, out=dx.view(B * G, D), accumulate=True)
        leaf(lambda dS=dS, dz=dz, l=l, layer=layer: (ops.bias_grad(dS.view(B * G, D), grad_of(layer.W.bias)),
                                                     ops.linear_bwd_weight(dz.view(B * G, D), gsv['xs'][l].view(B * G, D), grad_of(layer.W.weight))), dS, dz)
        dy = dx
    return dy


class _GCNFunction(torch.autograd.Function):

    @staticmethod
    def forward(ctx, feature, gcn, graph):
        seed = (getattr(gcn, '_calls', 0) * 7919 + 101) & 0x7FFFFFFF
        gcn.__dict__['_calls'] = getattr(gcn, '_calls', 0) + 1
        out, gsv = gcn_forward(gcn, feature.contiguous(), graph.contiguous(), seed, gcn.training)
        ctx.gcn, ctx.gsv, ctx.graph = gcn, gsv, graph.contiguous()
        return out

    @staticmethod
    def backward(ctx, dy):
        with ops.leaf_scope(dy.device, enable=False) as leaf:
            dx = gcn_backward(ctx.gcn, ctx.gsv, dy.contiguous(), ctx.graph, leaf)
        ctx.gsv = None
        return dx, None, None


CAPTURE = [None]


def sue_forward(mod, hist, cand, graph, cmask, cidx):
    B, Hn, D = hist.shape
    N = cand.shape[1]
    Kc = mod.proxy_node_embedding.shape[0]
    G, Cn, A = Hn + Kc, Kc + 1, mod.attention_dim
    dev = hist.device
    f32 = dict(device=dev, dtype=torch.float32)
    p = mod.dropout_rate if mod.training else 0.0
    seed = mod._next_seed()
    sv = dict(B=B, Hn=Hn, D=D, N=N, Kc=Kc, G=G, Cn=Cn, A=A, p=p, seed=seed, hist=hist, cand=cand, cidx=cidx, cmask=cmask,
              graph=graph)
    x0 = torch.empty((B, G, D), **f32)
    cand2 = cand.view(B * N, D)
    ia = mod.interClusterAttention
    qc = torch.empty((B * N, A), **f32)
    qv = torch.empty((B * N, A), **f32)
    v = torch.empty((B * N, D), **f32)

    def cand_side():
        ops.linear_fwd(cand2, mod.intraCluster_Q.weight, mod.intraCluster_Q.bias, out=qc)
        ops.linear_fwd(cand2, ia.Q.weight, ia.Q.bias, out=qv)
        ops.gemm(qv, ia.K.weight, v, M=B * N, N=D, K=A, lda=A, ldb=D, ldc=D, trans_b=True)
    side = _sue_side(dev)
    side_ev = None
    if side is not None:
        side.wait_stream(torch.cuda.current_stream(dev))
        with torch.cuda.stream(side):
            cand_side()
            side_ev = torch.cuda.Event()
            side_ev.record()
    fix = cmask if (cmask.is_cuda and cmask.dim() == 2 and cmask.is_contiguous() and tuple(cmask.shape) == (B, Kc + 1)) else None
    if fix is None:
        if cmask.is_cuda and cmask.dim() == 2 and cmask.is_contiguous() and cmask.element_size() == 1:
            ops.fill_column_u8(cmask, -1, 1)
        else:
            cmask[:, -1] = 1
    ops.sue_x0_fwd(hist, mod.proxy_node_embedding, x0, B, Hn, Kc, D, p, seed + 1, cmask_fix=fix)
    x, gsv = gcn_forward(mod.gcn, x0, graph, seed + 10, mod.training)
    sv['gcn'] = gsv
    gfeat = torch.empty((B, Hn, D), **f32)
    ops.sue_slice_fwd(x, x0, gfeat, B, Hn, G, D)
    kf = ops.linear_fwd(gfeat.view(B * Hn, D), mod.intraCluster_K.weight)
    if side is None:
        cand_side()
    else:
        torch.cuda.current_stream(dev).wait_event(side_ev)
    alpha_i = torch.empty((B, N, Hn), **f32)
    feat = torch.empty((B * N * Cn, D), **f32)
    ops.sue_intra_fwd(kf, qc, gfeat, cidx, B, N, Hn, Cn, A, D, alpha_i, feat)
    rc = torch.empty((B * N * Cn, D), **f32)
    f2 = torch.empty((B * N * Cn, D), **f32)
    ops.gemm(feat, mod.clusterFeatureAffine.weight, f2, M=B * N * Cn, N=D, K=D, lda=D, ldb=D, ldc=D, bias=mod.clusterFeatureAffine.bias,
             act=ops.ACT_RELU, aux_out=rc, ldaux=D, resid=feat, ldres=D, drop=(3, p, seed + 2, D))
    alpha_o = torch.empty(B * N * Cn, **f32)
    out = torch.empty((B * N, D), **f32)
    ops.pool_fwd(x=f2, ldx=D, D=D, n=B * N, Lx=Cn, mask=cmask, mask_div=N, v=v, ldv=D, scale=1.0 / math.sqrt(A), alpha=alpha_o, out=out,
                 ldo=D)
    sv.update(gfeat=gfeat, kf=kf, qc=qc, alpha_i=alpha_i, feat=feat, rc=rc, f2=f2, qv=qv, v=v, alpha_o=alpha_o)
    if CAPTURE[0] is not None:
        CAPTURE[0].append(sv)
    return out.view(B, N, D), sv


def sue_backward(mod, sv, dout, dhist_out=None, dcand_accum=None):
    B, Hn, D, N, Kc, G, Cn, A, p, seed = (sv[k] for k in ('B', 'Hn', 'D', 'N', 'Kc', 'G', 'Cn', 'A', 'p', 'seed'))
    dev = dout.device
    f32 = dict(device=dev, dtype=torch.float32)
    cand2 = sv['cand'].view(B * N, D)
    dout = dout.view(B * N, D)
    ia = mod.interClusterAttention
    hook = mod.__dict__.get('_grads_ready_hook')
    exchange = getattr(hook, '__self__', None)
    need_now = (exchange is not None and exchange.active()) or not ops._DEFER.get('step_joins')
    with ops.leaf_scope(dev, defer_join=not need_now) as leaf:
        res = _sue_backward_body(mod, sv, dout, leaf, B, Hn, D, N, Kc, G, Cn, A, p, seed, dev, f32, cand2, ia, dhist_out, dcand_accum)
    if hook is not None:
        hook()
    return res


def _sue_backward_body(mod, sv, dout, leaf, B, Hn, D, N, Kc, G, Cn, A, p, seed, dev, f32, cand2, ia, dhist_out=None, dcand_accum=None):
    df2 = torch.empty((B * N * Cn, D), **f32)
    dv = torch.empty((B * N, D), **f32)
    ops.pool_bwd(x=sv['f2'], ldx=D, D=D, n=B * N, Lx=Cn, mask=sv['cmask'], mask_div=N, v=sv['v'], ldv=D, scale=1.0 / math.sqrt(A),
                 alpha=sv['alpha_o'], dout=dout, lddo=D, dx=df2, lddx=D, dv=dv, lddv=D)
    dqv = torch.empty((B * N, A), **f32)
    dcand = dcand_accum if dcand_accum is not None else torch.empty((B * N, D), **f32)
    main = torch.cuda.current_stream(dev)
    side = _sue_side(dev)

    def on_side(fn):
        if side is None:
            return fn()
        side.wait_stream(main)
        with torch.cuda.stream(side):
            return fn()

    def inter_q():
        ops.gemm(dv, ia.K.weight, dqv, M=B * N, N=A, K=D, lda=D, ldb=D, ldc=A)
        leaf(lambda: (ops.linear_bwd_weight(sv['qv'], dv, grad_of(ia.K.weight)),
                      ops.linear_bwd_weight(dqv, cand2, grad_of(ia.Q.weight), db=grad_of(ia.Q.bias))), dv, dqv)
        ops.linear_bwd_data(dqv, ia.Q.weight, out=dcand, accumulate=dcand_accum is not None)
    on_side(inter_q)
    dS = torch.empty((B * N * Cn, D), **f32)
    dfeat = torch.empty((B * N * Cn, D), **f32)
    ops.relu_drop_bwd(df2, sv['rc'], dS, dfeat, p, seed + 2)
    ops.linear_bwd_data(dS, mod.clusterFeatureAffine.weight, out=dfeat, accumulate=True)
    dS_aff = dS
    leaf(lambda: ops.linear_bwd_weight(dS_aff, sv['feat'], grad_of(mod.clusterFeatureAffine.weight), db=grad_of(mod.clusterFeatureAffine.bias)), dS_aff)
    dg = torch.empty((B, Hn, D), **f32)
    dkf = torch.empty((B * Hn, A), **f32)
    dqc = torch.empty((B * N, A), **f32)
    ops.sue_intra_bwd(sv['kf'], sv['qc'], sv['gfeat'], sv['cidx'], sv['alpha_i'], dfeat, B, N, Hn, Cn, A, D, dg, dkf, dqc)
    ops.linear_bwd_data(dkf, mod.intraCluster_K.weight, out=dg.view(B * Hn, D), accumulate=True)
    on_side(lambda: ops.linear_bwd_data(dqc, mod.intraCluster_Q.weight, out=dcand, accumulate=True))
    leaf(lambda: (ops.linear_bwd_weight(dkf, sv['gfeat'].view(B * Hn, D), grad_of(mod.intraCluster_K.weight)),
                  ops.linear_bwd_weight(dqc, cand2, grad_of(mod.intraCluster_Q.weight), db=grad_of(mod.intraCluster_Q.bias))), dkf, dqc)
    dpad = torch.empty((B, G, D), **f32)
    ops.sue_slice_bwd(dg, dpad, B, Hn, G, D)
    dy = gcn_backward(mod.gcn, sv['gcn'], dpad, sv['graph'], leaf)
    dhist = torch.empty((B, Hn, D), **f32) if dhist_out is None else dhist_out
    ops.sue_x0_bwd(dy, dhist, grad_of(mod.proxy_node_embedding), B, Hn, Kc, D, p, seed + 1, dx0_add=dpad)
    if side is not None:
        main.wait_stream(side)
    return dhist, dcand.view(B, N, D)


class SUE(UserEncoder):

    def __init__(self, news_encoder: NewsEncoder, config):
        super().__init__(news_encoder, config)
        self.attention_dim = max(config.attention_dim, self.news_embedding_dim // 4)
        self.proxy_node_embedding = nn.Parameter(torch.zeros([config.category_num, self.news_embedding_dim]))
        self.gcn = GCN(in_dim=self.news_embedding_dim, out_dim=self.news_embedding_dim, hidden_dim=self.news_embedding_dim,
                       num_layers=config.gcn_layer_num, dropout=config.dropout_rate / 2, residual=not config.no_gcn_residual,
                       layer_norm=config.gcn_layer_norm)
        self.intraCluster_K = nn.Linear(self.news_embedding_dim, self.attention_dim, bias=False)
        self.intraCluster_Q = nn.Linear(self.news_embedding_dim, self.attention_dim, bias=True)
        self.clusterFeatureAffine = nn.Linear(self.news_embedding_dim, self.news_embedding_dim, bias=True)
        self.interClusterAttention = ScaledDotProduct_CandidateAttention(self.news_embedding_dim, self.news_embedding_dim, self.attention_dim)
        self.dropout_rate = float(config.dropout_rate)
        self.category_num = config.category_num + 1
        self.max_history_num = config.max_history_num
        self.attention_scalar = math.sqrt(float(self.attention_dim))

    def initialize(self):
        self.gcn.initialize()
        nn.init.zeros_(self.proxy_node_embedding)
        nn.init.xavier_uniform_(self.intraCluster_K.weight)
        nn.init.xavier_uniform_(self.intraCluster_Q.weight)
        nn.init.zeros_(self.intraCluster_Q.bias)
        nn.init.xavier_uniform_(self.clusterFeatureAffine.weight, gain=nn.init.calculate_gain('relu'))
        nn.init.zeros_(self.clusterFeatureAffine.bias)
        self.interClusterAttention.initialize()

    def forward(self, user_title_text, user_title_mask, user_title_entity, user_content_text, user_content_mask, user_content_entity,
                user_category, user_subCategory, user_history_mask, user_history_graph, user_history_category_mask,
                user_history_category_indices, user_embedding, candidate_news_representation):
        history_embedding = self.news_encoder(user_title_text, user_title_mask, user_title_entity, user_content_text, user_content_mask,
                                              user_content_entity, user_category, user_subCategory, user_embedding)
        return self.encode_user(history_embedding, user_history_mask, user_history_graph, user_history_category_mask,
                                user_history_category_indices, candidate_news_representation)

    def encode_user(self, history_embedding, user_history_mask, user_history_graph, user_history_category_mask,
                    user_history_category_indices, candidate_news_representation):
        graph = user_history_graph.contiguous()
        cidx = user_history_category_indices.contiguous()
        assert cidx.dtype == torch.int64 and graph.dtype == torch.float32
        return _SUEFunction.apply(history_embedding, candidate_news_representation, self, graph, user_history_category_mask, cidx)

class MHSA(UserEncoder):

    def __init__(self, news_encoder: NewsEncoder, config):
        super().__init__(news_encoder, config)
        self.head_num, self.head_dim, self.max_history_num = config.head_num, config.head_dim, config.max_history_num
        self.multiheadAttention = MultiHeadAttention(config.head_num, self.news_embedding_dim, config.max_history_num,
                                                     config.max_history_num, config.head_dim, config.head_dim)
        self.affine = nn.Linear(config.head_num * config.head_dim, self.news_embedding_dim, bias=True)
        self.attention = Attention(self.news_embedding_dim, config.attention_dim)

    def initialize(self):
        self.multiheadAttention.initialize()
        nn.init.xavier_uniform_(self.affine.weight, gain=nn.init.calculate_gain('relu'))
        nn.init.zeros_(self.affine.bias)
        self.attention.initialize()

    def forward(self, user_title_text, user_title_mask, user_title_entity, user_content_text, user_content_mask, user_content_entity,
                user_category, user_subCategory, user_history_mask, user_history_graph, user_history_category_mask,
                user_history_category_indices, user_embedding, candidate_news_representation):
        history_embedding = self.news_encoder(user_title_text, user_title_mask, user_title_entity, user_content_text, user_content_mask,
                                              user_content_entity, user_category, user_subCategory, user_embedding)
        return self.encode_user(history_embedding, user_history_mask, user_history_graph, user_history_category_mask,
                                user_history_category_indices, candidate_news_representation)

    def encode_user(self, history_embedding, user_history_mask, user_history_graph, user_history_category_mask,
                    user_history_category_indices, candidate_news_representation):
        from . import functional as Fn
        news_num = candidate_news_representation.size(1)
        B, Hn, D = history_embedding.shape
        qkv = Fn.QKVFn.apply(history_embedding.reshape(B * Hn, D), self.multiheadAttention, None)
        h = Fn.MhsaCoreFn.apply(qkv, user_history_mask.contiguous(), B, Hn, self.head_num, self.head_dim)
        h = Fn.LinearFn.apply(h, self.affine.weight, self.affine.bias, ops.ACT_RELU, 0.5 if self.training else 0.0, self._next_seed())
        user = self.attention(h.view(B, Hn, D))
        return Fn.ExpandFn.apply(user, news_num)

# ... 136 lines not shown
```

Baseline: 6741.

## Fold SUE slice into GCN kernels, fuse relu-dropout into pool bwd, persistent bx3 GEMM

```diff
diff --git a/include/nnr_hip.h b/include/nnr_hip.h
--- a/include/nnr_hip.h
+++ b/include/nnr_hip.h
@@ -123,6 +123,7 @@
   float* dv; int lddv;
   const float* th; int ldth; int A; const float* w2;
   const float* alpha_b; const float* dout_b; int lddo_b; const float* dscore_b; const float* v_b; int ldv_b; float scale_b;
+  const float* relu_r; float* drelu; float drop_p; uint32_t drop_seed;
 } nnr_pool_args;
 int nnr_attn_pool_fwd(const nnr_pool_args* a, hipStream_t stream);
 int nnr_attn_pool_bwd(const nnr_pool_args* a, hipStream_t stream);
@@ -164,8 +165,13 @@
 int nnr_relu_bwd(const float* dy, const float* y, float* dx, long n, hipStream_t stream);
 int nnr_gcn_aggregate_fwd(const float* graph, const float* z, const float* bias, const float* resid, float* r_out, float* y, int B, int G,
                           int D, int relu, float p, uint32_t seed, hipStream_t stream);
+int nnr_gcn_aggregate_fwd_slice(const float* graph, const float* z, const float* bias, const float* resid, float* r_out, float* y,
+                                const float* x0, float* gfeat, int B, int G, int Hn, int D, int relu, float p, uint32_t seed,
+                                hipStream_t stream);
 int nnr_gcn_aggregate_bwd(const float* graph, const float* dy, const float* r, float* ds, float* dx0, float* dz, int B, int G, int D, float p,
                           uint32_t seed, hipStream_t stream);
+int nnr_gcn_aggregate_bwd_compact(const float* graph, const float* dy, const float* r, float* ds, float* dx0, float* dz, int B, int G,
+                                  int in_rows, int D, float p, uint32_t seed, hipStream_t stream);
 int nnr_relu_drop_bwd(const float* dy, const float* r, float* ds, float* dx, long n, float p, uint32_t seed, hipStream_t stream);
 
 int nnr_mhsa_fwd(const float* qkv, const uint8_t* mask, int n, int Lq, int heads, int dh, float scale, float* out, float* prob,
@@ -187,6 +193,8 @@
                    uint8_t* cmask_fix, hipStream_t stream);
 int nnr_sue_x0_bwd(const float* dx0, const float* dx0_add, float* dhist, float* dproxy_accum, int B, int Hn, int Kc, int D, float p,
                    uint32_t seed, hipStream_t stream);
+int nnr_sue_x0_bwd_compact(const float* dx0, const float* dgfeat, float* dhist, float* dproxy_accum, int B, int Hn, int Kc, int D, float p,
+                           uint32_t seed, hipStream_t stream);
 int nnr_sue_slice_fwd(const float* gcn, const float* x0, float* gfeat, int B, int Hn, int G, int D, hipStream_t stream);
 int nnr_sue_slice_bwd(const float* dgfeat, float* dpad, int B, int Hn, int G, int D, hipStream_t stream);
 int nnr_sue_intra_fwd(const float* kf, const float* qc, const float* g, const long* cidx, int B, int N, int Hn, int C, int A, int D,
diff --git a/nnr_amd/_lib.py b/nnr_amd/_lib.py
--- a/nnr_amd/_lib.py
+++ b/nnr_amd/_lib.py
@@ -46,7 +46,8 @@
                 ('alpha', vp), ('out', vp), ('ldo', ci), ('add_in', vp), ('ldadd', ci), ('dout', vp), ('lddo', ci),
                 ('dout2', vp), ('lddo2', ci), ('dx', vp), ('lddx', ci), ('dx_accumulate', ci), ('dscore', vp), ('dv', vp),
                 ('lddv', ci), ('th', vp), ('ldth', ci), ('A', ci), ('w2', vp),
-                ('alpha_b', vp), ('dout_b', vp), ('lddo_b', ci), ('dscore_b', vp), ('v_b', vp), ('ldv_b', ci), ('scale_b', cf)]
+                ('alpha_b', vp), ('dout_b', vp), ('lddo_b', ci), ('dscore_b', vp), ('v_b', vp), ('ldv_b', ci), ('scale_b', cf),
+                ('relu_r', vp), ('drelu', vp), ('drop_p', cf), ('drop_seed', cu32)]
 
 
 SIGNATURES = {
@@ -94,6 +95,8 @@
     'nnr_relu_bwd': 'i32 ptr ptr ptr i64 stream',
     'nnr_gcn_aggregate_fwd': 'i32 ptr ptr ptr ptr ptr ptr i32 i32 i32 i32 f32 seed stream',
     'nnr_gcn_aggregate_bwd': 'i32 ptr ptr ptr ptr ptr ptr i32 i32 i32 f32 seed stream',
+    'nnr_gcn_aggregate_fwd_slice': 'i32 ptr ptr ptr ptr ptr ptr ptr ptr i32 i32 i32 i32 i32 f32 seed stream',
+    'nnr_gcn_aggregate_bwd_compact': 'i32 ptr ptr ptr ptr ptr ptr i32 i32 i32 i32 f32 seed stream',
     'nnr_relu_drop_bwd': 'i32 ptr ptr ptr ptr i64 f32 seed stream',
     'nnr_mhsa_fwd': 'i32 ptr ptr i32 i32 i32 i32 f32 ptr ptr f32 seed stream',
     'nnr_mhsa_bwd': 'i32 ptr ptr ptr ptr i32 i32 i32 i32 f32 ptr f32 seed stream',
@@ -104,6 +107,7 @@
     'nnr_mhsa_bwd_paired': 'i32 ptr ptr ptr ptr ptr i32 i32 i32 f32 ptr f32 seed stream',
     'nnr_sue_x0_fwd': 'i32 ptr ptr ptr i32 i32 i32 i32 f32 seed ptr stream',
     'nnr_sue_x0_bwd': 'i32 ptr ptr ptr ptr i32 i32 i32 i32 f32 seed stream',
+    'nnr_sue_x0_bwd_compact': 'i32 ptr ptr ptr ptr i32 i32 i32 i32 f32 seed stream',
     'nnr_sue_slice_fwd': 'i32 ptr ptr ptr i32 i32 i32 i32 stream',
     'nnr_sue_slice_bwd': 'i32 ptr ptr i32 i32 i32 i32 stream',
     'nnr_sue_intra_fwd': 'i32 ptr ptr ptr ptr i32 i32 i32 i32 i32 i32 ptr ptr stream',
diff --git a/nnr_amd/csrc/gcn.hip b/nnr_amd/csrc/gcn.hip
--- a/nnr_amd/csrc/gcn.hip
+++ b/nnr_amd/csrc/gcn.hip
@@ -7,7 +7,8 @@
 template <int MODE, int MT>
 __global__ __launch_bounds__(256) __attribute__((amdgpu_waves_per_eu(3, 8))) void gcn_aggregate_kernel(
     const float* __restrict__ graph, const float* __restrict__ in, const float* __restrict__ bias, const float* __restrict__ aux_in,
-    float* __restrict__ out0, float* __restrict__ out1, float* __restrict__ out2, int G, int D, int relu, uint32_t seed, uint32_t thr, float scale) {
+    float* __restrict__ out0, float* __restrict__ out1, float* __restrict__ out2, int G, int D, int relu, uint32_t seed, uint32_t thr, float scale,
+    const float* __restrict__ x0, float* __restrict__ gfeat, int in_rows) {
   extern __shared__ __attribute__((aligned(16))) float sm[];
   const int ks_n = (G + 3) >> 2, GR = ks_n * 4;
   const int A_LD = GR | 1;
@@ -41,7 +42,11 @@
     f32x4 v = {0.f, 0.f, 0.f, 0.f};
     if (row < G && cok) {
       const long idx = base + (long)row * D + c0 + c4;
-      v = *reinterpret_cast<const f32x4*>(in + idx);
+      if (MODE == 1 && in_rows < G) {
+        if (row < in_rows) v = *reinterpret_cast<const f32x4*>(in + ((long)b * in_rows + row) * D + c0 + c4);
+      } else {
+        v = *reinterpret_cast<const f32x4*>(in + idx);
+      }
       if (MODE == 1 && aux_in) {
         if (thr) {
           bool kp[4];
@@ -110,6 +115,8 @@
           for (int e = 0; e < 4; ++e) x[e] = kp[e] ? x[e] * scale : 0.f;
         }
         *reinterpret_cast<f32x4*>(out0 + idx) = x;
+        if (gfeat && row < in_rows)
+          *reinterpret_cast<f32x4*>(gfeat + ((long)b * in_rows + row) * D + c0 + c4) = x + *reinterpret_cast<const f32x4*>(x0 + idx);
       } else {
         *reinterpret_cast<f32x4*>(out2 + idx) = x;
       }
@@ -120,14 +127,35 @@
 
 }
 
-extern "C" int nnr_gcn_aggregate_fwd(const float* graph, const float* z, const float* bias, const float* resid, float* r_out, float* y, int B,
-                                     int G, int D, int relu, float p, uint32_t seed, hipStream_t stream) {
-  if (!graph || !z || !y || B <= 0 || G <= 0 || D <= 0) return NNR_ERR_ARG;
+extern "C" int nnr_gcn_aggregate_fwd_slice(const float* graph, const float* z, const float* bias, const float* resid, float* r_out, float* y,
+                                           const float* x0, float* gfeat, int B, int G, int Hn, int D, int relu, float p, uint32_t seed,
+                                           hipStream_t stream) {
+  if (!graph || !z || !y || B <= 0 || G <= 0 || D <= 0 || (gfeat && (!x0 || Hn <= 0 || Hn > G))) return NNR_ERR_ARG;
+  if (!gfeat) Hn = G;
   if (G > GCN_MAXG || (D & 3)) return NNR_ERR_UNSUPPORTED;
   const float sc = p > 0.f ? 1.f / (1.f - p) : 1.f;
   const int gp = (G + 15) / 16 * 16, gr = (G + 3) / 4 * 4;
 #define GCN_CASE(MT_) case MT_: hipLaunchKernelGGL((gcn_aggregate_kernel<0, MT_>), dim3((D + 63) / 64, B), dim3(256), (size_t)(((gr * (gr | 1) + 3) & ~3) + gr * 68) * sizeof(float), \
-                                                   stream, graph, z, bias, resid, y, r_out, nullptr, G, D, relu, seed, nnr_drop_thresh(p), sc); break;
+                                                   stream, graph, z, bias, resid, y, r_out, nullptr, G, D, relu, seed, nnr_drop_thresh(p), sc, x0, gfeat, Hn); break;
+  switch (gp / 16) { GCN_CASE(1) GCN_CASE(2) GCN_CASE(3) GCN_CASE(4) GCN_CASE(5) GCN_CASE(6) GCN_CASE(7) GCN_CASE(8) }
+#undef GCN_CASE
+  NNR_CHECK_LAUNCH();
+  return NNR_OK;
+}
+
+extern "C" int nnr_gcn_aggregate_fwd(const float* graph, const float* z, const float* bias, const float* resid, float* r_out, float* y, int B,
+                                     int G, int D, int relu, float p, uint32_t seed, hipStream_t stream) {
+  return nnr_gcn_aggregate_fwd_slice(graph, z, bias, resid, r_out, y, nullptr, nullptr, B, G, G, D, relu, p, seed, stream);
+}
+
+extern "C" int nnr_gcn_aggregate_bwd_compact(const float* graph, const float* dy, const float* r, float* ds, float* dx0, float* dz, int B, int G,
+                                             int in_rows, int D, float p, uint32_t seed, hipStream_t stream) {
+  if (!graph || !dy || !dz || B <= 0 || G <= 0 || D <= 0 || (r && !ds) || in_rows <= 0 || in_rows > G) return NNR_ERR_ARG;
+  if (G > GCN_MAXG || (D & 3)) return NNR_ERR_UNSUPPORTED;
+  const float sc = p > 0.f ? 1.f / (1.f - p) : 1.f;
+  const int gp = (G + 15) / 16 * 16, gr = (G + 3) / 4 * 4;
+#define GCN_CASE(MT_) case MT_: hipLaunchKernelGGL((gcn_aggregate_kernel<1, MT_>), dim3((D + 63) / 64, B), dim3(256), (size_t)(((gr * (gr | 1) + 3) & ~3) + gr * 68) * sizeof(float), \
+                                                   stream, graph, dy, nullptr, r, ds, dx0, dz, G, D, 0, seed, nnr_drop_thresh(p), sc, nullptr, nullptr, in_rows); break;
   switch (gp / 16) { GCN_CASE(1) GCN_CASE(2) GCN_CASE(3) GCN_CASE(4) GCN_CASE(5) GCN_CASE(6) GCN_CASE(7) GCN_CASE(8) }
 #undef GCN_CASE
   NNR_CHECK_LAUNCH();
@@ -136,14 +164,5 @@
 
 extern "C" int nnr_gcn_aggregate_bwd(const float* graph, const float* dy, const float* r, float* ds, float* dx0, float* dz, int B, int G, int D,
                                      float p, uint32_t seed, hipStream_t stream) {
-  if (!graph || !dy || !dz || B <= 0 || G <= 0 || D <= 0 || (r && !ds)) return NNR_ERR_ARG;
-  if (G > GCN_MAXG || (D & 3)) return NNR_ERR_UNSUPPORTED;
-  const float sc = p > 0.f ? 1.f / (1.f - p) : 1.f;
-  const int gp = (G + 15) / 16 * 16, gr = (G + 3) / 4 * 4;
-#define GCN_CASE(MT_) case MT_: hipLaunchKernelGGL((gcn_aggregate_kernel<1, MT_>), dim3((D + 63) / 64, B), dim3(256), (size_t)(((gr * (gr | 1) + 3) & ~3) + gr * 68) * sizeof(float), \
-                                                   stream, graph, dy, nullptr, r, ds, dx0, dz, G, D, 0, seed, nnr_drop_thresh(p), sc); break;
-  switch (gp / 16) { GCN_CASE(1) GCN_CASE(2) GCN_CASE(3) GCN_CASE(4) GCN_CASE(5) GCN_CASE(6) GCN_CASE(7) GCN_CASE(8) }
-#undef GCN_CASE
-  NNR_CHECK_LAUNCH();
-  return NNR_OK;
+  return nnr_gcn_aggregate_bwd_compact(graph, dy, r, ds, dx0, dz, B, G, G, D, p, seed, stream);
 }
diff --git a/nnr_amd/csrc/gemm.hip b/nnr_amd/csrc/gemm.hip
--- a/nnr_amd/csrc/gemm.hip
+++ b/nnr_amd/csrc/gemm.hip
@@ -903,17 +903,19 @@
   if (g.dyn_dim == 1) M = min(M, *g.dyn_dev);
   const int N = g.N, K = g.K;
   const int nbm = (M + BM - 1) / BM, nbn = (N + BN - 1) / BN, nblk = nbm * nbn;
-  if ((int)blockIdx.x >= nblk) return;
-  int v;
-  {
-    const int b = blockIdx.x, qq = nblk >> 3, rem = nblk & 7, x = b & 7, slot = b >> 3;
-    v = x * qq + min(x, rem) + slot;
-  }
-  const int bm = v / nbn, bn = v - bm * nbn, m0 = bm * BM, n0 = bn * BN;
   const int S = (K + BK - 1) / BK;
   const unsigned lds_base = (unsigned)(uintptr_t)lds_raw;
   const float* zero = nnr_zero_page;
   asm volatile("" : "+s"(zero));
+  const bool nb_hi = ((3 * NIB1) % 4 == 0) || (w < (3 * NIB1) % 4);
+  const bool ktail = (K % BK) != 0;
+  for (int vb = blockIdx.x; vb < nblk; vb += gridDim.x) {
+  int v;
+  {
+    const int b = vb, qq = nblk >> 3, rem = nblk & 7, x = b & 7, slot = b >> 3;
+    v = x * qq + min(x, rem) + slot;
+  }
+  const int bm = v / nbn, bn = v - bm * nbn, m0 = bm * BM, n0 = bn * BN;
   constexpr int NA = NIA / 4, NBW = (3 * NIB1 + 3) / 4;
   static_assert(NA <= 8 && NBW <= 8, "tile shape");
   unsigned voffA[8], voffB[8];
@@ -935,8 +937,6 @@
   }
   const float* Abase = g.A + (long)m0 * g.lda;
   const char* Bbase = reinterpret_cast<const char*>(reinterpret_cast<const __bf16*>(g.B3) + (long)n0 * g.ldb3);
-  const bool nb_hi = ((3 * NIB1) % 4 == 0) || (w < (3 * NIB1) % 4);
-  const bool ktail = (K % BK) != 0;
   auto issue = [&](int s) __attribute__((always_inline)) {
     const int k0 = s * BK;
     const unsigned sb = lds_base + (unsigned)((s % NS) * STAGE_BYTES) + (unsigned)(w * 1024);
@@ -1001,6 +1001,9 @@
     for (int n = 0; n < TN; ++n) acc_hi[m][n] += acc_lo[m][n];
   __syncthreads();
   gemm_epilogue<TM, TN>(g, acc_hi, reinterpret_cast<float*>(lds_raw), g.C, m0, n0, M, N, 0);
+  static_assert(NS == 2, "tile loop: the first stage's wait must be vmcnt(0)");
+  __syncthreads();
+  }
 }
 
 static bool bx3_ok(const nnr_gemm_args& g) {
@@ -1011,7 +1014,19 @@
 int launch_bx3(const nnr_gemm_args& g, hipStream_t s) {
   constexpr int BM = 64 * TM, BN = 16 * TN;
   const int nbm = (g.M + BM - 1) / BM, nbn = (g.N + BN - 1) / BN;
-  hipLaunchKernelGGL((gemm_nt_bx3_kernel<TM, TN, NS>), dim3(nbm * nbn), dim3(256), 0, s, g);
+  static int resident[64] = {};
+  int dev = 0;
+  if (hipGetDevice(&dev) != hipSuccess || dev < 0 || dev >= 64) return NNR_ERR_LAUNCH;
+  int R = __atomic_load_n(&resident[dev], __ATOMIC_RELAXED);
+  if (R == 0) {
+    int cus = 0, occ = 0;
+    if (hipDeviceGetAttribute(&cus, hipDeviceAttributeMultiprocessorCount, dev) != hipSuccess ||
+        hipOccupancyMaxActiveBlocksPerMultiprocessor(&occ, gemm_nt_bx3_kernel<TM, TN, NS>, 256, 0) != hipSuccess || cus < 1 || occ < 1)
+      return NNR_ERR_LAUNCH;
+    R = max(8, (occ * cus) & ~7);
+    __atomic_store_n(&resident[dev], R, __ATOMIC_RELAXED);
+  }
+  hipLaunchKernelGGL((gemm_nt_bx3_kernel<TM, TN, NS>), dim3(min(nbm * nbn, R)), dim3(256), 0, s, g);
   NNR_CHECK_LAUNCH();
   return NNR_OK;
 }
diff --git a/nnr_amd/csrc/misc.hip b/nnr_amd/csrc/misc.hip
--- a/nnr_amd/csrc/misc.hip
+++ b/nnr_amd/csrc/misc.hip
@@ -347,6 +347,63 @@
   }
 }
 
+__global__ __launch_bounds__(256) void sue_x0_vec4_kernel(const float* __restrict__ hist, const float* __restrict__ proxy, float* __restrict__ x0,
+                                                          int B, int Hn, int Kc, int D, const float* __restrict__ dx0,
+                                                          const float* __restrict__ dx0_add, int add_rows, float* __restrict__ dhist,
+                                                          float* __restrict__ dproxy, uint8_t* __restrict__ cmask_fix, uint32_t seed,
+                                                          uint32_t thr, float scale) {
+  const int G = Hn + Kc, D4 = D >> 2, tid = threadIdx.x;
+  const long gtid = blockIdx.x * 256L + tid, gthreads = gridDim.x * 256L;
+  if (cmask_fix)
+    for (long b = gtid; b < B; b += gthreads) cmask_fix[b * (Kc + 1) + Kc] = 1;
+  for (long row = blockIdx.x; row < (long)B * G; row += gridDim.x) {
+    const int b = (int)(row / G), j = (int)(row - (long)b * G);
+    if (j < Hn) {
+      const long hrow = (long)b * Hn + j;
+      for (int c4 = tid; c4 < D4; c4 += 256) {
+        if (x0) reinterpret_cast<f32x4*>(x0)[row * D4 + c4] = reinterpret_cast<const f32x4*>(hist)[hrow * D4 + c4];
+        if (dhist) {
+          f32x4 up = reinterpret_cast<const f32x4*>(dx0)[row * D4 + c4];
+          if (dx0_add) up += reinterpret_cast<const f32x4*>(dx0_add)[(add_rows == G ? row : hrow) * D4 + c4];
+          reinterpret_cast<f32x4*>(dhist)[hrow * D4 + c4] = up;
+        }
+      }
+    } else if (x0) {
+      const int k = j - Hn;
+      for (int c4 = tid; c4 < D4; c4 += 256) {
+        bool kp[4];
+        nnr_keep4(seed, (uint64_t)((long)b * Kc + k) * D + 4 * c4, thr, kp);
+        f32x4 v = reinterpret_cast<const f32x4*>(proxy)[(long)k * D4 + c4];
+#pragma unroll
+        for (int e = 0; e < 4; ++e) v[e] = v[e] * (kp[e] ? scale : 0.f);
+        reinterpret_cast<f32x4*>(x0)[row * D4 + c4] = v;
+      }
+    }
+  }
+  if (dproxy) {
+    for (long t = gtid; t < (long)Kc * D4; t += gthreads) {
+      const int k = (int)(t / D4), c4 = (int)(t - (long)k * D4);
+      float acc[4] = {0.f, 0.f, 0.f, 0.f};
+      for (int b = 0; b < B; ++b) {
+        const long i4 = ((long)b * G + Hn + k) * D4 + c4;
+        const f32x4 a = reinterpret_cast<const f32x4*>(dx0)[i4];
+        f32x4 z = {0.f, 0.f, 0.f, 0.f};
+        if (dx0_add && add_rows == G) z = reinterpret_cast<const f32x4*>(dx0_add)[i4];
+        bool kp[4];
+        nnr_keep4(seed, (uint64_t)((long)b * Kc + k) * D + 4 * c4, thr, kp);
+#pragma unroll
+        for (int e = 0; e < 4; ++e) {
+          const float up = dx0_add ? a[e] + z[e] : a[e];
+          const float m = kp[e] ? scale : 0.f;
+          acc[e] += up * m;
+        }
+      }
+#pragma unroll
+      for (int e = 0; e < 4; ++e) atomicAdd(&dproxy[4 * t + e], acc[e]);
+    }
+  }
+}
+
 __global__ void sue_slice_kernel(const float* __restrict__ gcn, const float* __restrict__ x0, float* __restrict__ gfeat,
                                  const float* __restrict__ dgfeat, float* __restrict__ dpad, int B, int Hn, int G, int D) {
   const long total = (long)B * G * D;
@@ -842,6 +899,11 @@
 
 extern "C" int nnr_version(void) { return 1; }
 
+static bool sue_x0_vec4_ok(int D, const void* a, const void* b, const void* c, const void* d, const void* e) {
+  return (D & 3) == 0 && (((uintptr_t)a | (uintptr_t)b | (uintptr_t)c | (uintptr_t)d | (uintptr_t)e) & 15) == 0;
+}
+static unsigned sue_x0_grid(int B, int G) { return (unsigned)((long)B * G < 16384 ? (long)B * G : 16384); }
+
 extern "C" int nnr_gate_bwd(const float* dHt, const float* H, const float* G, float* dH, float* dpre, const int* rows_dev,
                             int rows, int cols, hipStream_t stream) {
   if (cols & 3) return NNR_ERR_UNSUPPORTED;
@@ -971,14 +1033,36 @@
 extern "C" int nnr_sue_x0_fwd(const float* hist, const float* proxy, float* x0, int B, int Hn, int Kc, int D, float p, uint32_t seed,
                               uint8_t* cmask_fix, hipStream_t stream) {
   const float sc = p > 0.f ? 1.f / (1.f - p) : 1.f;
+  if (sue_x0_vec4_ok(D, hist, proxy, x0, nullptr, nullptr) && B > 0 && Hn + Kc > 0) {
+    hipLaunchKernelGGL(sue_x0_vec4_kernel, dim3(sue_x0_grid(B, Hn + Kc)), dim3(256), 0, stream, hist, proxy, x0, B, Hn, Kc, D, (const float*)nullptr,
+                       (const float*)nullptr, 0, (float*)nullptr, (float*)nullptr, cmask_fix, seed, nnr_drop_thresh(p), sc);
+    NNR_CHECK_LAUNCH();
+    return NNR_OK;
+  }
   EW_LAUNCH(sue_x0_kernel, (long)B * (Hn + Kc) * D, hist, proxy, x0, B, Hn, Kc, D, (const float*)nullptr, (const float*)nullptr, (float*)nullptr,
             (float*)nullptr, cmask_fix, seed, nnr_drop_thresh(p), sc);
 }
 extern "C" int nnr_sue_x0_bwd(const float* dx0, const float* dx0_add, float* dhist, float* dproxy, int B, int Hn, int Kc, int D, float p,
                               uint32_t seed, hipStream_t stream) {
   const float sc = p > 0.f ? 1.f / (1.f - p) : 1.f;
+  if (sue_x0_vec4_ok(D, dx0, dx0_add, dhist, dproxy, nullptr) && B > 0 && Hn + Kc > 0) {
+    hipLaunchKernelGGL(sue_x0_vec4_kernel, dim3(sue_x0_grid(B, Hn + Kc)), dim3(256), 0, stream, (const float*)nullptr, (const float*)nullptr,
+                       (float*)nullptr, B, Hn, Kc, D, dx0, dx0_add, Hn + Kc, dhist, dproxy, (uint8_t*)nullptr, seed, nnr_drop_thresh(p), sc);
+    NNR_CHECK_LAUNCH();
+    return NNR_OK;
+  }
   EW_LAUNCH(sue_x0_kernel, (long)B * (Hn + Kc) * D, (const float*)nullptr, (const float*)nullptr, (float*)nullptr, B, Hn, Kc, D, dx0, dx0_add,
             dhist, dproxy, (uint8_t*)nullptr, seed, nnr_drop_thresh(p), sc);
+}
+extern "C" int nnr_sue_x0_bwd_compact(const float* dx0, const float* dgfeat, float* dhist, float* dproxy, int B, int Hn, int Kc, int D, float p,
+                                      uint32_t seed, hipStream_t stream) {
+  if (!dx0 || !dgfeat || B <= 0 || Hn <= 0 || Kc < 0 || D <= 0) return NNR_ERR_ARG;
+  if (!sue_x0_vec4_ok(D, dx0, dgfeat, dhist, dproxy, nullptr)) return NNR_ERR_UNSUPPORTED;
+  const float sc = p > 0.f ? 1.f / (1.f - p) : 1.f;
+  hipLaunchKernelGGL(sue_x0_vec4_kernel, dim3(sue_x0_grid(B, Hn + Kc)), dim3(256), 0, stream, (const float*)nullptr, (const float*)nullptr,
+                     (float*)nullptr, B, Hn, Kc, D, dx0, dgfeat, Hn, dhist, dproxy, (uint8_t*)nullptr, seed, nnr_drop_thresh(p), sc);
+  NNR_CHECK_LAUNCH();
+  return NNR_OK;
 }
 extern "C" int nnr_sue_slice_fwd(const float* gcn, const float* x0, float* gfeat, int B, int Hn, int G, int D, hipStream_t stream) {
   EW_LAUNCH(sue_slice_kernel, (long)B * G * D, gcn, x0, gfeat, (const float*)nullptr, (float*)nullptr, B, Hn, G, D);
diff --git a/nnr_amd/csrc/pool.hip b/nnr_amd/csrc/pool.hip
--- a/nnr_amd/csrc/pool.hip
+++ b/nnr_amd/csrc/pool.hip
@@ -21,13 +21,14 @@
   float* dv; int lddv;
   const float* th; int ldth; int A; const float* w2;
   const float* alpha_b; const float* dout_b; int lddo_b; const float* dscore_b; const float* v_b; int ldv_b; float scale_b;
+  const float* relu_r; float* drelu; uint32_t drop_seed, drop_thr; float drop_scale;
 };
 
 __device__ __forceinline__ long item_row(const PoolArgs& a, int s, int t) {
   return a.packed ? (long)a.off[t] + s : (long)s * a.L + t;
 }
 
-template <bool BWD, int NV, int UR>
+template <bool BWD, int NV, int UR, bool FUSE = false>
 __device__ __forceinline__ void pool_stream_body(const PoolArgs& a, const int s, float* __restrict__ tok, f32x4 (*__restrict__ part)[64 * NV]) {
   constexpr int MAXV = NV;
   constexpr int NWV = 4;
@@ -274,6 +275,19 @@
               g += dst * q[j];
               dvacc[j] += dst * xv[u][j];
             }
+            if constexpr (FUSE) {
+              const long idx = rows[u] * a.lddx + 4 * c;
+              bool kp[4];
+              nnr_keep4(a.drop_seed, (uint64_t)idx, a.drop_thr, kp);
+              const f32x4 rv = *reinterpret_cast<const f32x4*>(a.relu_r + idx);
+              f32x4 gs;
+#pragma unroll
+              for (int e = 0; e < 4; ++e) {
+                g[e] = g[e] * (kp[e] ? a.drop_scale : 0.f);
+                gs[e] = rv[e] > 0.f ? g[e] : 0.f;
+              }
+              *reinterpret_cast<f32x4*>(a.drelu + idx) = gs;
+            }
             if (a.dx) *reinterpret_cast<f32x4*>(a.dx + rows[u] * a.lddx + 4 * c) = g;
           }
         }
@@ -292,11 +306,11 @@
   }
 }
 
-template <bool BWD, int NV, int UR>
+template <bool BWD, int NV, int UR, bool FUSE = false>
 __global__ __launch_bounds__(256) void pool_kernel(PoolArgs a) {
   __shared__ float tok[64 * MAXT];
   __shared__ f32x4 part[4][64 * NV];
-  pool_stream_body<BWD, NV, UR>(a, blockIdx.x, tok, part);
+  pool_stream_body<BWD, NV, UR, FUSE>(a, blockIdx.x, tok, part);
 }
 
 __device__ __forceinline__ float lane_get(float v, int i) { return __builtin_bit_cast(float, __builtin_amdgcn_readlane(__builtin_bit_cast(int, v), i)); }
@@ -524,6 +538,8 @@
   a.dx = p->dx; a.lddx = p->lddx; a.dx_accumulate = p->dx_accumulate; a.dscore = p->dscore; a.dv = p->dv; a.lddv = p->lddv;
   a.th = p->th; a.ldth = p->ldth; a.A = p->A; a.w2 = p->w2;
   a.alpha_b = p->alpha_b; a.dout_b = p->dout_b; a.lddo_b = p->lddo_b; a.dscore_b = p->dscore_b; a.v_b = p->v_b; a.ldv_b = p->ldv_b; a.scale_b = p->scale_b;
+  a.relu_r = p->relu_r; a.drelu = p->drelu; a.drop_seed = p->drop_seed; a.drop_thr = nnr_drop_thresh(p->drop_p);
+  a.drop_scale = p->drop_p > 0.f ? 1.f / (1.f - p->drop_p) : 1.f;
   return a;
 }
 
@@ -538,6 +554,16 @@
     NNR_CHECK_LAUNCH();
     return NNR_OK;
   }
+  if constexpr (BWD) {
+    if (p->relu_r) {
+      if (nv <= 64) hipLaunchKernelGGL((pool_kernel<true, 1, 4, true>), grid, block, 0, stream, a);
+      else if (nv <= 128) hipLaunchKernelGGL((pool_kernel<true, 2, 4, true>), grid, block, 0, stream, a);
+      else if (nv <= 256) hipLaunchKernelGGL((pool_kernel<true, 4, 2, true>), grid, block, 0, stream, a);
+      else hipLaunchKernelGGL((pool_kernel<true, 5, 2, true>), grid, block, 0, stream, a);
+      NNR_CHECK_LAUNCH();
+      return NNR_OK;
+    }
+  }
   if (nv <= 64) hipLaunchKernelGGL((pool_kernel<BWD, 1, 4>), grid, block, 0, stream, a);
   else if (nv <= 128) hipLaunchKernelGGL((pool_kernel<BWD, 2, 4>), grid, block, 0, stream, a);
   else if (nv <= 256) hipLaunchKernelGGL((pool_kernel<BWD, 4, 2>), grid, block, 0, stream, a);
@@ -558,5 +584,6 @@
   if (rc != NNR_OK) return rc;
   if (!p->dout || !p->alpha) return NNR_ERR_ARG;
   if (p->alpha_b && (!p->dout_b || !p->dscore_b || !p->v_b || !p->dx || p->dx_accumulate || (p->lddo_b & 3) || (p->ldv_b & 3))) return NNR_ERR_ARG;
+  if (p->relu_r && (!p->drelu || !p->dx || p->packed || p->dx_accumulate || p->lddx != p->D)) return NNR_ERR_ARG;
   return pool_launch<true>(p, stream);
 }
diff --git a/nnr_amd/csrc/tape.hip b/nnr_amd/csrc/tape.hip
--- a/nnr_amd/csrc/tape.hip
+++ b/nnr_amd/csrc/tape.hip
@@ -29,8 +29,8 @@
   R(nnr_lstm_fwd), R(nnr_lstm_bwd), R(nnr_attn_pool_fwd), R(nnr_attn_pool_bwd), R(nnr_gate_bwd), R(nnr_packed_seq_sum),
   R(nnr_tanh_score_bwd), R(nnr_colsum), R(nnr_rowdot), R(nnr_small_embed_fwd), R(nnr_small_embed_bwd), R(nnr_embed_gather),
   R(nnr_embed_scatter), R(nnr_embed_scatter_dyn), R(nnr_transpose2d), R(nnr_transpose_batch), R(nnr_add), R(nnr_add_atomic), R(nnr_add2d), R(nnr_expand_rows_fwd), R(nnr_expand_rows_bwd),
-  R(nnr_dropout), R(nnr_relu_bwd), R(nnr_gcn_aggregate_fwd), R(nnr_gcn_aggregate_bwd), R(nnr_relu_drop_bwd), R(nnr_mhsa_fwd), R(nnr_mhsa_bwd),
-  R(nnr_sue_x0_fwd), R(nnr_sue_x0_bwd), R(nnr_sue_slice_fwd), R(nnr_sue_slice_bwd), R(nnr_sue_intra_fwd), R(nnr_sue_intra_bwd),
+  R(nnr_dropout), R(nnr_relu_bwd), R(nnr_gcn_aggregate_fwd), R(nnr_gcn_aggregate_bwd), R(nnr_gcn_aggregate_fwd_slice), R(nnr_gcn_aggregate_bwd_compact), R(nnr_relu_drop_bwd), R(nnr_mhsa_fwd), R(nnr_mhsa_bwd),
+  R(nnr_sue_x0_fwd), R(nnr_sue_x0_bwd), R(nnr_sue_x0_bwd_compact), R(nnr_sue_slice_fwd), R(nnr_sue_slice_bwd), R(nnr_sue_intra_fwd), R(nnr_sue_intra_bwd),
   R(nnr_corpus_batch), R(nnr_history_graph), R(nnr_logits_loss_fwd), R(nnr_logits_fwd), R(nnr_nls_loss), R(nnr_logits_bwd),
   R(nnr_layernorm_fwd), R(nnr_layernorm_bwd), R(nnr_sumsq), R(nnr_sumsq_part), R(nnr_clip_adam), R(nnr_dp_allreduce), R(nnr_dp_broadcast), R(nnr_dp_busy), R(nnr_split_bf16x3), R(nnr_mhsa_fwd_packed), R(nnr_mhsa_bwd_packed), R(nnr_mhsa_pair_map), R(nnr_mhsa_fwd_paired), R(nnr_mhsa_bwd_paired), R(nnr_mask_cover), R(nnr_seq_rowmap),
   R(nnr_fill_zero), R(nnr_copy_bytes), R(nnr_fill_column_u8), R(nnr_fusion_rows_fwd), R(nnr_fusion_rows_bwd), R(nnr_click_loss), R(nnr_rank_metrics),
diff --git a/nnr_amd/ops.py b/nnr_amd/ops.py
--- a/nnr_amd/ops.py
+++ b/nnr_amd/ops.py
@@ -764,7 +764,8 @@
 
 def _pool_args(x, ldx, D, n, Lx, plan=None, mask=None, mask_div=1, score=None, v=None, ldv=0, scale=1.0, alpha=None, out=None,
                ldo=0, add_in=None, ldadd=0, dout=None, lddo=0, dout2=None, lddo2=0, dx=None, lddx=0, dx_accumulate=False,
-               dscore=None, dv=None, lddv=0, th=None, w2=None, alpha_b=None, dout_b=None, lddo_b=0, dscore_b=None, v_b=None, ldv_b=0, scale_b=1.0):
+               dscore=None, dv=None, lddv=0, th=None, w2=None, alpha_b=None, dout_b=None, lddo_b=0, dscore_b=None, v_b=None, ldv_b=0, scale_b=1.0,
+               relu_r=None, drelu=None, drop_p=0.0, drop_seed=0):
     a = L.PoolArgs()
     a.x, a.ldx, a.D, a.n, a.L = _p(x), ldx, D, n, Lx
     a.packed = int(plan is not None)
@@ -781,6 +782,8 @@
         a.th, a.ldth, a.A, a.w2 = _p(th), th.stride(0), th.shape[1], _p(w2)
     if alpha_b is not None:
         a.alpha_b, a.dout_b, a.lddo_b, a.dscore_b, a.v_b, a.ldv_b, a.scale_b = _p(alpha_b), _p(dout_b), lddo_b, _p(dscore_b), _p(v_b), ldv_b, float(scale_b)
+    if relu_r is not None:
+        a.relu_r, a.drelu, a.drop_p, a.drop_seed = _p(relu_r), _p(drelu), float(drop_p), int(drop_seed) & 0xFFFFFFFF
     return a
 
 
@@ -891,16 +894,24 @@
     L.check(L.lib().nnr_relu_drop_bwd(_p(dy), _p(r), _p(ds), _p(dx), dy.numel(), p, seed, _s()), 'nnr_relu_drop_bwd')
 
 
-def gcn_aggregate_fwd(graph, z, bias, resid, r_out, y, B, G, D, relu, p, seed):
+def gcn_aggregate_fwd(graph, z, bias, resid, r_out, y, B, G, D, relu, p, seed, x0=None, gfeat=None, Hn=0):
     arrays = 3 + (1 if resid is not None else 0)
-    with _hbm_span('gcn_aggregate_fwd', 4.0 * (G * D * arrays + G * G), B):
+    with _hbm_span('gcn_aggregate_fwd', 4.0 * (G * D * arrays + G * G + (2 * Hn * D if gfeat is not None else 0)), B):
+        if gfeat is not None:
+            L.check(L.lib().nnr_gcn_aggregate_fwd_slice(_p(graph), _p(z), _p(bias), _p(resid), _p(r_out), _p(y), _p(x0), _p(gfeat), B, G, Hn, D, relu,
+                                                        p, seed, _s()), 'nnr_gcn_aggregate_fwd_slice')
+            return
         L.check(L.lib().nnr_gcn_aggregate_fwd(_p(graph), _p(z), _p(bias), _p(resid), _p(r_out), _p(y), B, G, D, relu, p, seed, _s()),
                                               'nnr_gcn_aggregate_fwd')
 
 
-def gcn_aggregate_bwd(graph, dy, r, ds, dx0, dz, B, G, D, p, seed):
+def gcn_aggregate_bwd(graph, dy, r, ds, dx0, dz, B, G, D, p, seed, in_rows=None):
     arrays = 4 + (1 if dx0 is not None else 0)
     with _hbm_span('gcn_aggregate_bwd', 4.0 * (G * D * arrays + G * G), B):
+        if in_rows is not None:
+            L.check(L.lib().nnr_gcn_aggregate_bwd_compact(_p(graph), _p(dy), _p(r), _p(ds), _p(dx0), _p(dz), B, G, in_rows, D, p, seed, _s()),
+                    'nnr_gcn_aggregate_bwd_compact')
+            return
         L.check(L.lib().nnr_gcn_aggregate_bwd(_p(graph), _p(dy), _p(r), _p(ds), _p(dx0), _p(dz), B, G, D, p, seed, _s()), 'nnr_gcn_aggregate_bwd')
 
 
@@ -912,6 +923,10 @@
 
 def sue_x0_bwd(dx0, dhist, dproxy, B, Hn, Kc, D, p, seed, dx0_add=None):
     L.check(L.lib().nnr_sue_x0_bwd(_p(dx0), _p(dx0_add), _p(dhist), _p(dproxy), B, Hn, Kc, D, p, seed, _s()), 'nnr_sue_x0_bwd')
+
+
+def sue_x0_bwd_compact(dx0, dgfeat, dhist, dproxy, B, Hn, Kc, D, p, seed):
+    L.check(L.lib().nnr_sue_x0_bwd_compact(_p(dx0), _p(dgfeat), _p(dhist), _p(dproxy), B, Hn, Kc, D, p, seed, _s()), 'nnr_sue_x0_bwd_compact')
 
 
 def sue_slice_fwd(gcn, x0, gfeat, B, Hn, G, D):
diff --git a/nnr_amd/user_encoders.py b/nnr_amd/user_encoders.py
--- a/nnr_amd/user_encoders.py
+++ b/nnr_amd/user_encoders.py
@@ -55,10 +55,15 @@
     return _SIDE[key]
 
 
-def gcn_forward(gcn, x0, graph, seed0, training):
+def _gcn_row_moves_fold(gcn, G, D):
+    return gcn.num_layers >= 1 and G <= 128 and D % 4 == 0 and not getattr(gcn.gcn_layers[gcn.num_layers - 1], 'layer_norm', False)
+
+
+def gcn_forward(gcn, x0, graph, seed0, training, gfeat=None):
     B, G, D = x0.shape
     f32 = dict(device=x0.device, dtype=torch.float32)
     Lg = gcn.num_layers
+    assert gfeat is None or _gcn_row_moves_fold(gcn, G, D)
     xs, rs, lns = [x0], [], []
     x = x0
     for l, layer in enumerate(gcn.gcn_layers):
@@ -76,7 +81,9 @@
             ops.layernorm_fwd(u, ln.weight, ln.bias, ln.eps, xhat, rstd, r, x if gcn.residual else None, y, pl, seed0 + l)
             lns.append((xhat, rstd))
         elif G <= 128 and D % 4 == 0:
-            ops.gcn_aggregate_fwd(graph, z, layer.W.bias, x if gcn.residual else None, r, y, B, G, D, True, pl, seed0 + l)
+            last = gfeat if l + 1 == Lg else None
+            ops.gcn_aggregate_fwd(graph, z, layer.W.bias, x if gcn.residual else None, r, y, B, G, D, True, pl, seed0 + l,
+                                  x0=x0 if last is not None else None, gfeat=last, Hn=gfeat.shape[1] if last is not None else 0)
             lns.append(None)
         else:
             ops.gemm(graph, z, y, M=G, N=D, K=G, lda=G, ldb=D, ldc=D, trans_b=True, bias=layer.W.bias, act=ops.ACT_RELU, aux_out=r,
@@ -89,10 +96,11 @@
     return x, dict(xs=xs, rs=rs, lns=lns, seed0=seed0, training=training)
 
 
-def gcn_backward(gcn, gsv, dy, graph, leaf):
-    B, G, D = dy.shape
+def gcn_backward(gcn, gsv, dy, graph, leaf, in_rows=None):
+    B, G, D = gsv['xs'][0].shape
     f32 = dict(device=dy.device, dtype=torch.float32)
     Lg = gcn.num_layers
+    assert in_rows is None or _gcn_row_moves_fold(gcn, G, D)
     for l in range(Lg - 1, -1, -1):
         layer = gcn.gcn_layers[l]
         pl = (gcn.dropout_rate if gsv['training'] else 0.0) if l + 1 < Lg else 0.0
@@ -100,7 +108,8 @@
         dx = torch.empty((B, G, D), **f32)
         if G <= 128 and D % 4 == 0 and gsv['lns'][l] is None:
             dz = torch.empty((B, G, D), **f32)
-            ops.gcn_aggregate_bwd(graph, dy, gsv['rs'][l], dS, dx if gcn.residual else None, dz, B, G, D, pl, gsv['seed0'] + l)
+            ops.gcn_aggregate_bwd(graph, dy, gsv['rs'][l], dS, dx if gcn.residual else None, dz, B, G, D, pl, gsv['seed0'] + l,
+                                  in_rows=in_rows if l + 1 == Lg else None)
             ops.linear_bwd_data(dz.view(B * G, D), layer.W.weight, out=dx.view(B * G, D), accumulate=bool(gcn.residual))
             leaf(lambda dS=dS, dz=dz, l=l, layer=layer: (ops.bias_grad(dS.view(B * G, D), grad_of(layer.W.bias)),
                                                          ops.linear_bwd_weight(dz.view(B * G, D), gsv['xs'][l].view(B * G, D), grad_of(layer.W.weight))), dS, dz)
@@ -183,10 +192,12 @@
         else:
             cmask[:, -1] = 1
     ops.sue_x0_fwd(hist, mod.proxy_node_embedding, x0, B, Hn, Kc, D, p, seed + 1, cmask_fix=fix)
-    x, gsv = gcn_forward(mod.gcn, x0, graph, seed + 10, mod.training)
+    gfeat = torch.empty((B, Hn, D), **f32)
+    fold = _gcn_row_moves_fold(mod.gcn, G, D)
+    x, gsv = gcn_forward(mod.gcn, x0, graph, seed + 10, mod.training, gfeat=gfeat if fold else None)
     sv['gcn'] = gsv
-    gfeat = torch.empty((B, Hn, D), **f32)
-    ops.sue_slice_fwd(x, x0, gfeat, B, Hn, G, D)
+    if not fold:
+        ops.sue_slice_fwd(x, x0, gfeat, B, Hn, G, D)
     kf = ops.linear_fwd(gfeat.view(B * Hn, D), mod.intraCluster_K.weight)
     if side is None:
         cand_side()
@@ -227,10 +238,11 @@
 
 
 def _sue_backward_body(mod, sv, dout, leaf, B, Hn, D, N, Kc, G, Cn, A, p, seed, dev, f32, cand2, ia, dhist_out=None, dcand_accum=None):
-    df2 = torch.empty((B * N * Cn, D), **f32)
+    dS = torch.empty((B * N * Cn, D), **f32)
+    dfeat = torch.empty((B * N * Cn, D), **f32)
     dv = torch.empty((B * N, D), **f32)
     ops.pool_bwd(x=sv['f2'], ldx=D, D=D, n=B * N, Lx=Cn, mask=sv['cmask'], mask_div=N, v=sv['v'], ldv=D, scale=1.0 / math.sqrt(A),
-                 alpha=sv['alpha_o'], dout=dout, lddo=D, dx=df2, lddx=D, dv=dv, lddv=D)
+                 alpha=sv['alpha_o'], dout=dout, lddo=D, dx=dfeat, lddx=D, dv=dv, lddv=D, relu_r=sv['rc'], drelu=dS, drop_p=p, drop_seed=seed + 2)
     dqv = torch.empty((B * N, A), **f32)
     dcand = dcand_accum if dcand_accum is not None else torch.empty((B * N, D), **f32)
     main = torch.cuda.current_stream(dev)
@@ -249,9 +261,6 @@
                       ops.linear_bwd_weight(dqv, cand2, grad_of(ia.Q.weight), db=grad_of(ia.Q.bias))), dv, dqv)
         ops.linear_bwd_data(dqv, ia.Q.weight, out=dcand, accumulate=dcand_accum is not None)
     on_side(inter_q)
-    dS = torch.empty((B * N * Cn, D), **f32)
-    dfeat = torch.empty((B * N * Cn, D), **f32)
-    ops.relu_drop_bwd(df2, sv['rc'], dS, dfeat, p, seed + 2)
     ops.linear_bwd_data(dS, mod.clusterFeatureAffine.weight, out=dfeat, accumulate=True)
     dS_aff = dS
     leaf(lambda: ops.linear_bwd_weight(dS_aff, sv['feat'], grad_of(mod.clusterFeatureAffine.weight), db=grad_of(mod.clusterFeatureAffine.bias)), dS_aff)
@@ -263,11 +272,15 @@
     on_side(lambda: ops.linear_bwd_data(dqc, mod.intraCluster_Q.weight, out=dcand, accumulate=True))
     leaf(lambda: (ops.linear_bwd_weight(dkf, sv['gfeat'].view(B * Hn, D), grad_of(mod.intraCluster_K.weight)),
                   ops.linear_bwd_weight(dqc, cand2, grad_of(mod.intraCluster_Q.weight), db=grad_of(mod.intraCluster_Q.bias))), dkf, dqc)
-    dpad = torch.empty((B, G, D), **f32)
-    ops.sue_slice_bwd(dg, dpad, B, Hn, G, D)
-    dy = gcn_backward(mod.gcn, sv['gcn'], dpad, sv['graph'], leaf)
     dhist = torch.empty((B, Hn, D), **f32) if dhist_out is None else dhist_out
-    ops.sue_x0_bwd(dy, dhist, grad_of(mod.proxy_node_embedding), B, Hn, Kc, D, p, seed + 1, dx0_add=dpad)
+    if _gcn_row_moves_fold(mod.gcn, G, D):
+        dy = gcn_backward(mod.gcn, sv['gcn'], dg, sv['graph'], leaf, in_rows=Hn)
+        ops.sue_x0_bwd_compact(dy, dg, dhist, grad_of(mod.proxy_node_embedding), B, Hn, Kc, D, p, seed + 1)
+    else:
+        dpad = torch.empty((B, G, D), **f32)
+        ops.sue_slice_bwd(dg, dpad, B, Hn, G, D)
+        dy = gcn_backward(mod.gcn, sv['gcn'], dpad, sv['graph'], leaf)
+        ops.sue_x0_bwd(dy, dhist, grad_of(mod.proxy_node_embedding), B, Hn, Kc, D, p, seed + 1, dx0_add=dpad)
     if side is not None:
         main.wait_stream(side)
     return dhist, dcand.view(B, N, D)
```

Measured after the change: 6789, median of 6. No clear change (+0.7%).
